# nuclia/nucliadb

Hardware: NVIDIA H100
Metric: k-NN QPS @ recall@10 (higher is better)
Workload: dtype f32

## Files before the change

### include/nidx_b200.h

```cpp
#ifndef NIDX_B200_H
#define NIDX_B200_H

#include <stdint.h>

#ifdef __cplusplus
extern "C" {
#endif

#define NIDX_OK 0
#define NIDX_EINVAL (-1)
#define NIDX_ENODEVICE (-2)
#define NIDX_ECUDA (-3)
#define NIDX_EIO (-4)
#define NIDX_ESTATE (-5)
#define NIDX_EOVERFLOW (-6)

#define NIDX_MEM_HOST 0
#define NIDX_MEM_DEVICE 1

#define NIDX_SIM_DOT 0
#define NIDX_SIM_COSINE 1
#define NIDX_SIM_L2 2

#define NIDX_METHOD_AUTO 0
#define NIDX_METHOD_HNSW 1
#define NIDX_METHOD_BRUTE 2
#define NIDX_METHOD_BRUTE_RABITQ 3
#define NIDX_METHOD_HNSW_RABITQ 4

#define NIDX_NIL 0xFFFFFFFFu

const char* nidx_last_error(void);
int nidx_device_count(void);
uint64_t nidx_launch_count(void);

typedef struct nidx_vec_segment nidx_vec_segment;

typedef struct nidx_vec_config {
    int32_t dimension;
    int32_t similarity;
    int32_t multi_vector;
    int32_t m;
    int32_t m0;
    int32_t ef_construction;
    int32_t ef_search;
    int32_t device;
} nidx_vec_config;

int nidx_vec_create(const nidx_vec_config* cfg, const float* vectors, uint64_t n, int32_t ld, int mem, const uint32_t* paragraph_of,
                    nidx_vec_segment** out);

int nidx_vec_open(const nidx_vec_config* cfg, const char* dir, nidx_vec_segment** out);
int nidx_vec_save(nidx_vec_segment* seg, const char* dir);
void nidx_vec_close(nidx_vec_segment* seg);

uint64_t nidx_vec_len(const nidx_vec_segment* seg);
const float* nidx_vec_device_vectors(const nidx_vec_segment* seg, int32_t* ld_out);

int nidx_vec_build_hnsw(nidx_vec_segment* seg, uint64_t seed, int32_t max_batch, void* stream);

int nidx_hnsw_levels(uint64_t n, int32_t m, uint64_t seed, uint8_t* out_level);

int nidx_normalize_vectors(int32_t device, float* vectors, uint64_t n, int32_t d, int32_t ld, int mem, void* stream);

int nidx_use_hnsw(uint64_t total_nodes, uint64_t matching_nodes, uint64_t top_k, int has_rabitq, int m);

int nidx_vec_extend_hnsw(nidx_vec_segment* seg, uint64_t n_existing, const uint8_t* level_existing, const uint32_t* adj0, const float* w0,
                         const uint32_t* adjU, const float* wU, uint32_t entry_node, uint32_t entry_layer, uint64_t seed, int32_t max_batch,
                         void* stream);

int nidx_vec_graph_dims(const nidx_vec_segment* seg, int32_t* s0, int32_t* su, uint64_t* upper_rows, uint32_t* entry_node,
                        uint32_t* entry_layer);
int nidx_vec_set_graph(nidx_vec_segment* seg, const uint8_t* level, const uint32_t* adj0, const float* w0, const uint32_t* adjU,
                       const float* wU);
int nidx_vec_get_graph(const nidx_vec_segment* seg, uint8_t* level, uint32_t* adj0, float* w0, uint32_t* adjU, float* wU);

int nidx_vec_set_alive(nidx_vec_segment* seg, const uint64_t* alive_bits, int mem);

typedef struct nidx_vec_search_params {
    int32_t k;
    int32_t ef;
    float min_score;
    int32_t with_duplicates;
    int32_t method;
    const uint64_t* filter_bits;
    uint64_t filter_matching;
} nidx_vec_search_params;

int nidx_vec_search(nidx_vec_segment* seg, const float* queries, int32_t nq, int32_t ldq, int mem, const nidx_vec_search_params* p,
                    uint32_t* out_ids, float* out_scores, int32_t* out_counts, void* stream);

#define NIDX_INV_LABELS 0
#define NIDX_INV_FIELDS 1
int nidx_vec_set_inverted_index(nidx_vec_segment* seg, int32_t which, uint32_t n_keys, const uint8_t* key_bytes, const uint64_t* key_off,
                                const uint64_t* post_off, const uint32_t* postings);

#define NIDX_F_LABEL 0
#define NIDX_F_KEYS 1
#define NIDX_F_AND 2
#define NIDX_F_OR 3
#define NIDX_F_NOT 4
typedef struct nidx_filter_node {
    int32_t kind;
    int32_t n;
    const uint8_t* const* keys;
    const uint32_t* key_len;
} nidx_filter_node;

int nidx_vec_filter(nidx_vec_segment* seg, const nidx_filter_node* nodes, int32_t n_nodes, uint64_t* out_bits, int mem, uint64_t* out_matching, void* stream);

int nidx_vec_search_formula(nidx_vec_segment* seg, const float* queries, int32_t nq, int32_t ldq, int mem, const nidx_vec_search_params* p,
                            const nidx_filter_node* nodes, int32_t n_nodes, uint32_t* out_ids, float* out_scores, int32_t* out_counts, void* stream);

int nidx_merge_topk(int32_t device, const uint32_t* ids, const float* scores, int32_t n_parts, int64_t part_stride, int32_t nq, int32_t k,
                    uint32_t* out_ids, float* out_scores, int32_t* out_part, void* stream);
int nidx_merge_vector_parts(int32_t device, const uint32_t* ids, const float* scores, int32_t n_parts, int64_t part_stride, int32_t nq, int32_t k,
                            uint32_t* out_ids, float* out_scores, int32_t* out_part, void* stream);

int nidx_vec_counters(nidx_vec_segment* seg, uint64_t out[3]);
int nidx_vec_counters_ex(nidx_vec_segment* seg, uint64_t out[6]);
int nidx_vec_exact_rows(nidx_vec_segment* seg, uint64_t* out);
int nidx_vec_scan_counters(nidx_vec_segment* seg, uint64_t out[2]);

int nidx_vec_rabitq_encode(nidx_vec_segment* seg, void* stream);
int nidx_vec_rabitq_codes(const nidx_vec_segment* seg, uint8_t* out_codes);
int nidx_vec_rabitq_estimate(nidx_vec_segment* seg, const float* queries, int32_t nq, int32_t ldq, int mem, float* out_estimate, float* out_error,
                             void* stream);

int nidx_vec_last_kernel_ms(nidx_vec_segment* seg, float* ms);

typedef struct nidx_txt_segment nidx_txt_segment;

#define NIDX_BM25_OR 0
#define NIDX_BM25_AND 1

int nidx_txt_create(int32_t device, uint32_t n_docs, uint32_t n_terms, const uint64_t* term_off, const uint32_t* post_doc,
                    const uint32_t* post_tf, const uint8_t* fieldnorm_id, nidx_txt_segment** out);
int nidx_txt_set_stats(nidx_txt_segment* seg, uint64_t total_docs, uint64_t total_tokens, const uint64_t* doc_freq);
int nidx_txt_set_alive(nidx_txt_segment* seg, const uint64_t* alive_bits);
void nidx_txt_close(nidx_txt_segment* seg);

typedef struct nidx_txt_search_params {
    int32_t k;
    int32_t mode;
    int32_t use_tf;
    float min_score;
    int32_t after_mode;
    float after_score;
    uint64_t after_docaddr;
    uint64_t docaddr_base;
} nidx_txt_search_params;

int nidx_txt_search(nidx_txt_segment* seg, const uint32_t* query_terms, const uint32_t* query_off, int32_t nq, int mem,
                    const nidx_txt_search_params* p, uint32_t* out_docs, float* out_scores, int32_t* out_counts, uint64_t* out_total,
                    void* stream);

int nidx_txt_last_kernel_ms(nidx_txt_segment* seg, float* ms);


int nidx_txt_set_facets(nidx_txt_segment* seg, uint32_t n_facets, const uint8_t* key_bytes, const uint64_t* key_off, const uint64_t* doc_off,
                        const uint32_t* doc_ords);

typedef struct nidx_txt_facet_request {
    int32_t n;
    const uint8_t* key_bytes;
    const uint64_t* key_off;
} nidx_txt_facet_request;

int nidx_txt_facet_buckets(nidx_txt_segment* seg, const nidx_txt_facet_request* facets, uint32_t* out_bucket_req, uint32_t* out_bucket_ord,
                           uint32_t cap, uint32_t* out_n_buckets);

int nidx_txt_search_faceted(nidx_txt_segment* seg, const uint32_t* query_terms, const uint32_t* query_off, int32_t nq, int mem,
                            const nidx_txt_search_params* p, const nidx_txt_facet_request* facets, uint32_t* out_docs, float* out_scores,
                            int32_t* out_counts, uint64_t* out_total, uint32_t* out_facet_counts, void* stream);

int nidx_txt_facet_count_all(nidx_txt_segment* seg, const nidx_txt_facet_request* facets, int mem, uint32_t* out_facet_counts, void* stream);

#define NIDX_DATE_NONE INT64_MIN
#define NIDX_ORDER_CREATED 0
#define NIDX_ORDER_MODIFIED 1
#define NIDX_ORDER_DESC 0
#define NIDX_ORDER_ASC 1

typedef struct nidx_txt_order {
    int32_t field;
    int32_t type;
} nidx_txt_order;

int nidx_txt_set_dates(nidx_txt_segment* seg, const int64_t* created, const int64_t* modified);

int nidx_txt_search_ordered(nidx_txt_segment* seg, const uint32_t* query_terms, const uint32_t* query_off, int32_t nq, int mem,
                            const nidx_txt_search_params* p, const nidx_txt_order* order, const nidx_txt_facet_request* facets, uint32_t* out_docs,
                            int64_t* out_dates, int32_t* out_counts, uint64_t* out_total, uint32_t* out_facet_counts, void* stream);


int nidx_txt_set_positions(nidx_txt_segment* seg, const uint32_t* positions, uint64_t n_positions);

typedef struct nidx_txt_phrases {
    const uint32_t* terms;
    const uint32_t* off;
    const uint32_t* query;
    int32_t n;
} nidx_txt_phrases;

int nidx_txt_search_phrases(nidx_txt_segment* seg, const uint32_t* query_terms, const uint32_t* query_off, int32_t nq, int mem,
                            const nidx_txt_search_params* p, const nidx_txt_phrases* phrases, const nidx_txt_order* order,
                            const nidx_txt_facet_request* facets, uint32_t* out_docs, float* out_scores, int64_t* out_dates, int32_t* out_counts,
                            uint64_t* out_total, uint32_t* out_facet_counts, void* stream);

int nidx_txt_list_ordered(nidx_txt_segment* seg, const nidx_txt_order* order, int32_t k, int mem, uint32_t* out_docs, int64_t* out_dates,
                          int32_t* out_count, uint64_t* out_total, void* stream);


int nidx_txt_set_doc_columns(nidx_txt_segment* seg, const uint32_t* resource_ord, const uint32_t* field_ord);

#define NIDX_P_FACET 0
#define NIDX_P_FIELD 1
#define NIDX_P_RESOURCE 2
#define NIDX_P_DATE 3
#define NIDX_P_KEYWORD 4
#define NIDX_P_ALL 5
#define NIDX_P_AND 6
#define NIDX_P_OR 7
#define NIDX_P_NOT 8
#define NIDX_PREFILTER_MAX_DEPTH 64
typedef struct nidx_prefilter_node {
    int32_t kind;
    int32_t n;
    int64_t lo, hi;
    const uint32_t* terms;
} nidx_prefilter_node;

int nidx_txt_prefilter(nidx_txt_segment* seg, const nidx_prefilter_node* nodes, int32_t n_nodes, uint64_t* out_bits, int mem, uint64_t* out_matching,
                       void* stream);

int nidx_vec_prefilter_bits(nidx_vec_segment* seg, const uint64_t* doc_bits, uint64_t n_docs, const uint32_t* join, const nidx_filter_node* nodes,
                            int32_t n_nodes, int32_t op, uint64_t* out_bits, int mem, uint64_t* out_matching, void* stream);

typedef struct nidx_shard_comm nidx_shard_comm;

int nidx_shard_unique_id(uint8_t out_id[128]);
int nidx_shard_init(const uint8_t unique_id[128], int32_t rank, int32_t world, int32_t device, nidx_shard_comm** out);
void nidx_shard_destroy(nidx_shard_comm* comm);

int nidx_vec_set_paragraph_keys(nidx_vec_segment* seg, const uint64_t* keys);

int nidx_vec_search_sharded(nidx_shard_comm* comm, nidx_vec_segment* seg, const float* queries, int32_t nq, int32_t ldq, int mem,
                            const nidx_vec_search_params* p, int32_t dedup, uint32_t* out_ids, float* out_scores, int32_t* out_part, int32_t* out_counts,
                            void* stream);

int nidx_vec_shard_record(nidx_vec_segment* seg, const float* queries, int32_t nq, int32_t ldq, int mem, const nidx_vec_search_params* p, int32_t rank,
                          int32_t dedup, uint32_t* out_record, void* stream);
int nidx_shard_merge(int32_t device, const uint32_t* records, int32_t n_parts, int32_t nq, int32_t k, int32_t dedup, int32_t with_duplicates, int mem,
                     uint32_t* out_ids, float* out_scores, int32_t* out_part, int32_t* out_counts, void* stream);
int nidx_txt_search_sharded(nidx_shard_comm* comm, nidx_txt_segment* seg, const uint32_t* query_terms, const uint32_t* query_off, int32_t nq, int mem,
                            const nidx_txt_search_params* p, uint32_t* out_docs, float* out_scores, int32_t* out_part, int32_t* out_counts, uint64_t* out_total,
                            void* stream);

int nidx_txt_set_doc_keys(nidx_txt_segment* seg, const uint64_t* keys);

typedef struct nidx_rrf_source {
    const uint64_t* keys;
    const float* scores;
    const int32_t* counts;
    int32_t k;
    double weight;
} nidx_rrf_source;

int nidx_rank_fusion_rrf(int32_t device, const nidx_rrf_source* sources, int32_t n_sources, int32_t nq, double k, int mem, uint64_t* out_keys,
                         double* out_scores, uint32_t* out_refs, int32_t* out_counts, void* stream);

typedef struct nidx_shard_search_request {
    int32_t nq;
    nidx_vec_segment* vec; const float* queries; int32_t ldq; const nidx_vec_search_params* vec_params;
    const nidx_filter_node* formula; int32_t n_formula;
    nidx_txt_segment* par; const uint32_t* par_terms; const uint32_t* par_off; const nidx_txt_search_params* par_params;
    nidx_txt_segment* doc; const uint32_t* doc_terms; const uint32_t* doc_off; const nidx_txt_search_params* doc_params;
    double rrf_k, weight_keyword, weight_semantic;
    int32_t semantic_first;
} nidx_shard_search_request;

typedef struct nidx_shard_search_response {
    uint32_t* vec_ids; float* vec_scores; int32_t* vec_counts;
    uint32_t* par_docs; float* par_scores; int32_t* par_counts; uint64_t* par_total;
    uint32_t* doc_docs; float* doc_scores; int32_t* doc_counts; uint64_t* doc_total;
    uint64_t* fused_keys; double* fused_scores; uint32_t* fused_refs; int32_t* fused_counts;
} nidx_shard_search_response;

int nidx_shard_search(const nidx_shard_search_request* req, nidx_shard_search_response* resp, int mem, void* stream);

#ifdef __cplusplus
}
#endif
#endif
```

### nucliadb_b200/_lib.py

```python
from __future__ import annotations

import ctypes as C
import os

_HERE = os.path.dirname(os.path.abspath(__file__))
LIB_PATH = os.path.join(_HERE, os.path.basename(os.environ.get("NIDX_B200_LIB", "libnidx_b200.so")))

NIDX_MEM_HOST, NIDX_MEM_DEVICE = 0, 1
NIDX_SIM_DOT, NIDX_SIM_COSINE, NIDX_SIM_L2 = 0, 1, 2
NIDX_METHOD_AUTO, NIDX_METHOD_HNSW, NIDX_METHOD_BRUTE, NIDX_METHOD_BRUTE_RABITQ, NIDX_METHOD_HNSW_RABITQ = 0, 1, 2, 3, 4
NIDX_BM25_OR, NIDX_BM25_AND = 0, 1
NIDX_ORDER_CREATED, NIDX_ORDER_MODIFIED = 0, 1
NIDX_ORDER_DESC, NIDX_ORDER_ASC = 0, 1
NIDX_DATE_NONE = -(1 << 63)
NIL = 0xFFFFFFFF


class NidxError(RuntimeError):

    def __init__(self, code: int, message: str):
        super().__init__(f"nidx_b200 error {code}: {message}")
        self.code = code


class VecConfig(C.Structure):
    _fields_ = [("dimension", C.c_int32), ("similarity", C.c_int32), ("multi_vector", C.c_int32), ("m", C.c_int32), ("m0", C.c_int32),
                ("ef_construction", C.c_int32), ("ef_search", C.c_int32), ("device", C.c_int32)]


class VecSearchParams(C.Structure):
    _fields_ = [("k", C.c_int32), ("ef", C.c_int32), ("min_score", C.c_float), ("with_duplicates", C.c_int32), ("method", C.c_int32),
                ("filter_bits", C.c_void_p), ("filter_matching", C.c_uint64)]


class FilterNode(C.Structure):
    _fields_ = [("kind", C.c_int32), ("n", C.c_int32), ("keys", C.POINTER(C.c_void_p)), ("key_len", C.POINTER(C.c_uint32))]


NIDX_INV_LABELS, NIDX_INV_FIELDS = 0, 1
NIDX_F_LABEL, NIDX_F_KEYS, NIDX_F_AND, NIDX_F_OR, NIDX_F_NOT = 0, 1, 2, 3, 4


class PrefilterNode(C.Structure):
    _fields_ = [("kind", C.c_int32), ("n", C.c_int32), ("lo", C.c_int64), ("hi", C.c_int64), ("terms", C.c_void_p)]


NIDX_P_FACET, NIDX_P_FIELD, NIDX_P_RESOURCE, NIDX_P_DATE, NIDX_P_KEYWORD, NIDX_P_ALL, NIDX_P_AND, NIDX_P_OR, NIDX_P_NOT = range(9)
NIDX_PREFILTER_MAX_DEPTH = 64


class TxtSearchParams(C.Structure):
    _fields_ = [("k", C.c_int32), ("mode", C.c_int32), ("use_tf", C.c_int32), ("min_score", C.c_float), ("after_mode", C.c_int32),
                ("after_score", C.c_float), ("after_docaddr", C.c_uint64), ("docaddr_base", C.c_uint64)]


class TxtFacetRequest(C.Structure):
    _fields_ = [("n", C.c_int32), ("key_bytes", C.c_void_p), ("key_off", C.c_void_p)]


class TxtOrder(C.Structure):
    _fields_ = [("field", C.c_int32), ("type", C.c_int32)]


class TxtPhrases(C.Structure):
    _fields_ = [("terms", C.c_void_p), ("off", C.c_void_p), ("query", C.c_void_p), ("n", C.c_int32)]


class RrfSource(C.Structure):
    _fields_ = [("keys", C.c_void_p), ("scores", C.c_void_p), ("counts", C.c_void_p), ("k", C.c_int32), ("weight", C.c_double)]


class ShardSearchRequest(C.Structure):
    _fields_ = [("nq", C.c_int32),
                ("vec", C.c_void_p), ("queries", C.c_void_p), ("ldq", C.c_int32), ("vec_params", C.POINTER(VecSearchParams)),
                ("formula", C.POINTER(FilterNode)), ("n_formula", C.c_int32),
                ("par", C.c_void_p), ("par_terms", C.c_void_p), ("par_off", C.c_void_p), ("par_params", C.POINTER(TxtSearchParams)),
                ("doc", C.c_void_p), ("doc_terms", C.c_void_p), ("doc_off", C.c_void_p), ("doc_params", C.POINTER(TxtSearchParams)),
                ("rrf_k", C.c_double), ("weight_keyword", C.c_double), ("weight_semantic", C.c_double), ("semantic_first", C.c_int32)]


class ShardSearchResponse(C.Structure):
    _fields_ = [(n, C.c_void_p) for n in ("vec_ids", "vec_scores", "vec_counts", "par_docs", "par_scores", "par_counts", "par_total",
                                           "doc_docs", "doc_scores", "doc_counts", "doc_total", "fused_keys", "fused_scores", "fused_refs", "fused_counts")]


i32, u32, i64, u64, f64, P = C.c_int32, C.c_uint32, C.c_int64, C.c_uint64, C.c_double, C.c_void_p
CFG, VSP, NODES, TSP = C.POINTER(VecConfig), C.POINTER(VecSearchParams), C.POINTER(FilterNode), C.POINTER(TxtSearchParams)
REQ, ORDER, RRF = C.POINTER(TxtFacetRequest), C.POINTER(TxtOrder), C.POINTER(RrfSource)
SIGNATURES = {
    "nidx_last_error": (C.c_char_p, []),
    "nidx_device_count": (i32, []),
    "nidx_launch_count": (u64, []),
    "nidx_vec_create": (i32, [CFG, P, u64, i32, i32, P, P]),
    "nidx_vec_open": (i32, [CFG, C.c_char_p, P]),
    "nidx_vec_save": (i32, [P, C.c_char_p]),
    "nidx_vec_close": (None, [P]),
    "nidx_vec_len": (u64, [P]),
    "nidx_vec_device_vectors": (P, [P, P]),
    "nidx_vec_build_hnsw": (i32, [P, u64, i32, P]),
    "nidx_hnsw_levels": (i32, [u64, i32, u64, P]),
    "nidx_normalize_vectors": (i32, [i32, P, u64, i32, i32, i32, P]),
    "nidx_use_hnsw": (i32, [u64, u64, u64, i32, i32]),
    "nidx_vec_extend_hnsw": (i32, [P, u64, P, P, P, P, P, u32, u32, u64, i32, P]),
    "nidx_vec_graph_dims": (i32, [P, P, P, P, P, P]),
    "nidx_vec_set_graph": (i32, [P, P, P, P, P, P]),
    "nidx_vec_get_graph": (i32, [P, P, P, P, P, P]),
    "nidx_vec_set_alive": (i32, [P, P, i32]),
    "nidx_vec_search": (i32, [P, P, i32, i32, i32, VSP, P, P, P, P]),
    "nidx_vec_set_inverted_index": (i32, [P, i32, u32, P, P, P, P]),
    "nidx_vec_filter": (i32, [P, NODES, i32, P, i32, P, P]),
    "nidx_vec_search_formula": (i32, [P, P, i32, i32, i32, VSP, NODES, i32, P, P, P, P]),
    "nidx_merge_topk": (i32, [i32, P, P, i32, i64, i32, i32, P, P, P, P]),
    "nidx_merge_vector_parts": (i32, [i32, P, P, i32, i64, i32, i32, P, P, P, P]),
    "nidx_vec_counters": (i32, [P, P]),
    "nidx_vec_counters_ex": (i32, [P, P]),
    "nidx_vec_exact_rows": (i32, [P, P]),
    "nidx_vec_scan_counters": (i32, [P, P]),
    "nidx_vec_rabitq_encode": (i32, [P, P]),
    "nidx_vec_rabitq_codes": (i32, [P, P]),
    "nidx_vec_rabitq_estimate": (i32, [P, P, i32, i32, i32, P, P, P]),
    "nidx_vec_last_kernel_ms": (i32, [P, P]),
    "nidx_txt_create": (i32, [i32, u32, u32, P, P, P, P, P]),
    "nidx_txt_set_stats": (i32, [P, u64, u64, P]),
    "nidx_txt_set_alive": (i32, [P, P]),
    "nidx_txt_close": (None, [P]),
    "nidx_txt_search": (i32, [P, P, P, i32, i32, TSP, P, P, P, P, P]),
    "nidx_txt_last_kernel_ms": (i32, [P, P]),
    "nidx_txt_set_facets": (i32, [P, u32, P, P, P, P]),
    "nidx_txt_facet_buckets": (i32, [P, REQ, P, P, u32, P]),
    "nidx_txt_search_faceted": (i32, [P, P, P, i32, i32, TSP, REQ, P, P, P, P, P, P]),
    "nidx_txt_facet_count_all": (i32, [P, REQ, i32, P, P]),
    "nidx_txt_set_dates": (i32, [P, P, P]),
    "nidx_txt_search_ordered": (i32, [P, P, P, i32, i32, TSP, ORDER, REQ, P, P, P, P, P, P]),
    "nidx_txt_list_ordered": (i32, [P, ORDER, i32, i32, P, P, P, P, P]),
    "nidx_txt_set_positions": (i32, [P, P, u64]),
    "nidx_txt_search_phrases": (i32, [P, P, P, i32, i32, TSP, P, ORDER, REQ, P, P, P, P, P, P, P]),
    "nidx_txt_set_doc_columns": (i32, [P, P, P]),
    "nidx_txt_prefilter": (i32, [P, P, i32, P, i32, P, P]),
    "nidx_vec_prefilter_bits": (i32, [P, P, u64, P, NODES, i32, i32, P, i32, P, P]),
    "nidx_shard_unique_id": (i32, [P]),
    "nidx_shard_init": (i32, [P, i32, i32, i32, P]),
    "nidx_shard_destroy": (None, [P]),
    "nidx_vec_set_paragraph_keys": (i32, [P, P]),
    "nidx_vec_search_sharded": (i32, [P, P, P, i32, i32, i32, VSP, i32, P, P, P, P, P]),
    "nidx_vec_shard_record": (i32, [P, P, i32, i32, i32, VSP, i32, i32, P, P]),
    "nidx_shard_merge": (i32, [i32, P, i32, i32, i32, i32, i32, i32, P, P, P, P, P]),
    "nidx_txt_search_sharded": (i32, [P, P, P, P, i32, i32, TSP, P, P, P, P, P, P]),
    "nidx_txt_set_doc_keys": (i32, [P, P]),
    "nidx_rank_fusion_rrf": (i32, [i32, RRF, i32, i32, f64, i32, P, P, P, P, P]),
    "nidx_shard_search": (i32, [C.POINTER(ShardSearchRequest), C.POINTER(ShardSearchResponse), i32, P]),
}
SYMBOLS = list(SIGNATURES)

_lib = None


def load():
    global _lib
    if _lib is not None:
        return _lib
    if not os.path.exists(LIB_PATH):
        raise ImportError(f"{LIB_PATH} is missing: build it with `python -c 'import __graft_entry__ as g; g.build()'` "
                          "(nvcc, sm_90a). nucliadb_b200 has no CPU fallback.")
    L = C.CDLL(LIB_PATH)
    for name, (restype, argtypes) in SIGNATURES.items():
        fn = getattr(L, name)
        fn.restype, fn.argtypes = restype, argtypes
    _lib = L
    return L


def check(rc: int):
    if rc != 0:
        raise NidxError(rc, load().nidx_last_error().decode("utf-8", "replace"))


def require_device():
    L = load()
    if L.nidx_device_count() <= 0:
        raise NidxError(-2, "no CUDA device available; nucliadb_b200 has no CPU fallback")
    return L


def ptr(a):
    if a is None:
        return None
    if isinstance(a, int):
        return C.c_void_p(a)
    if hasattr(a, "data_ptr"):
        return C.c_void_p(a.data_ptr())
    return a.ctypes.data_as(C.c_void_p)
```

### nucliadb_b200/csrc/api.cu

```cuda
#include <cub/device/device_radix_sort.cuh>
#include <cub/device/device_scan.cuh>

#include <algorithm>
#include <atomic>
#include <cmath>
#include <cfloat>
#include <cstdarg>
#include <cstdio>
#include <cstring>
#include <memory>
#include <mutex>
#include <string>
#include <vector>

#include "../../include/nidx_b200.h"
#include "bm25.cuh"
#include "phrase.cuh"
#include "prefilter.cuh"
#include "common.cuh"
#include "hnsw_build.cuh"
#include "hnsw_search.cuh"
#include "hnsw_rabitq.cuh"
#include "rabitq.cuh"
#include "rank_fusion.cuh"
#include "scan.cu"
#include "scan_tc2.cuh"
#include "segment_io.hpp"
#include "shard.cuh"
#include "topk.cuh"

using namespace nidx;

static thread_local std::string g_err;
static std::atomic<uint64_t> g_launches{0};

static int fail(int code, const char* fmt, ...) {
    char buf[512];
    va_list ap;
    va_start(ap, fmt);
    vsnprintf(buf, sizeof(buf), fmt, ap);
    va_end(ap);
    g_err = buf;
    return code;
}
#define CU(expr)                                                                                              \
    do {                                                                                                      \
        cudaError_t e__ = (expr);                                                                             \
        if (e__ != cudaSuccess) return fail(NIDX_ECUDA, "%s failed: %s (%s:%d)", #expr, cudaGetErrorString(e__), __FILE__, __LINE__); \
    } while (0)
#define LAUNCHED() (g_launches.fetch_add(1, std::memory_order_relaxed))

static int next_pow2(int x) { int p = 1; while (p < x) p <<= 1; return p; }
static int ilog2(int x) { int b = 0; while ((1 << b) < x) ++b; return b; }

template <class T>
struct DevArray {
    T* p = nullptr;
    size_t cap = 0;
    DevArray() = default;
    DevArray(DevArray&& o) noexcept : p(o.p), cap(o.cap) { o.p = nullptr; o.cap = 0; }
    DevArray& operator=(DevArray&& o) noexcept {
        if (this != &o) { release(); p = o.p; cap = o.cap; o.p = nullptr; o.cap = 0; }
        return *this;
    }
    ~DevArray() { release(); }
    operator T*() const { return p; }
    template <class U> U* as() const { return reinterpret_cast<U*>(p); }
    void release() { if (p) cudaFree(p); p = nullptr; cap = 0; }
    cudaError_t try_alloc(size_t bytes) {
        release();
        cudaError_t e = cudaMalloc(&p, bytes);
        if (e == cudaSuccess) cap = bytes;
        else { p = nullptr; (void)cudaGetLastError(); }
        return e;
    }
    int alloc(size_t bytes) {
        cudaError_t e = try_alloc(bytes);
        return e == cudaSuccess ? 0 : fail(NIDX_ECUDA, "cudaMalloc(%zu) failed: %s", bytes, cudaGetErrorString(e));
    }
    int ensure(size_t bytes) {
        if (bytes <= cap || try_alloc(bytes + bytes / 4 + 256) == cudaSuccess) return 0;
        return alloc(bytes);
    }
};
using DevBuf = DevArray<unsigned char>;
#define ENSURE(buf, bytes) do { int r__ = (buf).ensure(bytes); if (r__) return r__; } while (0)
#define ALLOC(buf, bytes) do { int r__ = (buf).alloc(bytes); if (r__) return r__; } while (0)

struct Workspace {
    DevBuf queries, qnorms, stage, scores, partial, filter, misc, sched, facets, phrases, prefilter;
    cudaEvent_t done = nullptr;
    cudaStream_t last_stream = nullptr;
    bool busy = false;
    ~Workspace() { if (done) cudaEventDestroy(done); }
};

struct WorkspacePool {
    std::mutex mu;
    std::vector<Workspace*> all;
    static constexpr size_t MAX_POOL = 8;
    Workspace* acquire(cudaStream_t stream) {
        std::lock_guard<std::mutex> g(mu);
        Workspace* pick = nullptr;
        for (Workspace* w : all)
            if (!w->busy && w->last_stream == stream) { pick = w; break; }
        if (!pick) {
            for (Workspace* w : all)
                if (!w->busy && (!w->done || cudaEventQuery(w->done) == cudaSuccess)) { pick = w; break; }
            (void)cudaGetLastError();
        }
        if (!pick && all.size() >= MAX_POOL)
            for (Workspace* w : all)
                if (!w->busy) { cudaEventSynchronize(w->done); pick = w; break; }
        if (!pick) {
            pick = new Workspace();
            cudaEventCreateWithFlags(&pick->done, cudaEventDisableTiming);
            all.push_back(pick);
        }
        pick->busy = true;
        return pick;
    }
    void release(Workspace* w, cudaStream_t stream) {
        cudaEventRecord(w->done, stream);
        std::lock_guard<std::mutex> g(mu);
        w->last_stream = stream;
        w->busy = false;
    }
    ~WorkspacePool() { for (Workspace* w : all) delete w; }
};
struct WsGuard {
    WorkspacePool& pool; Workspace* w; cudaStream_t s;
    WsGuard(WorkspacePool& p, cudaStream_t st) : pool(p), w(p.acquire(st)), s(st) {}
    ~WsGuard() { pool.release(w, s); }
};

static WorkspacePool* plan_pool(int device) {
    static std::mutex mu;
    static WorkspacePool* pools[64] = {nullptr};
    std::lock_guard<std::mutex> g(mu);
    if (device < 0 || device >= 64) return nullptr;
    if (!pools[device]) pools[device] = new WorkspacePool();
    return pools[device];
}

struct Stage {
    cudaStream_t stream;
    bool qhost, ohost;
    struct Slot { void* var; const void* in; void* out; size_t bytes; void* dev; };
    std::vector<Slot> slots;
    size_t total = 0;
    Stage(cudaStream_t s, bool qh, bool oh) : stream(s), qhost(qh), ohost(oh) {}
    void add(void* var, const void* in, void* out, size_t bytes) {
        slots.push_back({var, in, out, bytes, nullptr});
        total += (bytes + 15) / 16 * 16;
    }
    template <class T> void in(const T* src, size_t n, const T** dev) {
        *dev = src;
        if (qhost && src) add(dev, src, nullptr, n * sizeof(T));
    }
    template <class T> void out(T* dst, size_t n, T** dev) {
        *dev = dst;
        if (ohost || !dst) add(dev, nullptr, ohost ? dst : nullptr, n * sizeof(T));
    }
    int place(DevBuf& buf) {
        ENSURE(buf, total);
        unsigned char* p = buf.as<unsigned char>();
        for (Slot& s : slots) {
            s.dev = p;
            p += (s.bytes + 15) / 16 * 16;
            memcpy(s.var, &s.dev, sizeof(void*));
            if (s.in && s.bytes) CU(cudaMemcpyAsync(s.dev, s.in, s.bytes, cudaMemcpyHostToDevice, stream));
        }
        return 0;
    }
    int finish(bool sync = false) {
        if (ohost)
            for (const Slot& s : slots)
                if (s.out && s.bytes) CU(cudaMemcpyAsync(s.out, s.dev, s.bytes, cudaMemcpyDeviceToHost, stream));
        if (ohost || sync) CU(cudaStreamSynchronize(stream));
        return 0;
    }
};

struct nidx_vec_segment {
    nidx_vec_config cfg;
    uint64_t n = 0;
    int d = 0, ld = 0;
    int sm_count = 0;
    DevArray<float> d_vecs;
    DevArray<float> d_norms;
    DevArray<uint32_t> d_par_of;
    DevArray<uint32_t> d_par_first;
    uint32_t n_par = 0;
    DevArray<uint64_t> d_alive;
    uint64_t alive_count = 0;
    DevArray<uint64_t> d_par_keys;
    struct InvIndex {
        std::vector<unsigned char> key_bytes;
        std::vector<uint64_t> key_off, post_off;
        DevArray<uint32_t> d_post;
        DevArray<uint64_t> d_post_off;
        uint32_t n_keys = 0;
    } inv[2];
    bool has_graph = false;
    std::vector<uint8_t> h_level;
    DevArray<uint8_t> d_level;
    uint32_t entry_node = 0, entry_layer = 0;
    int s0 = 0, su = 0;
    uint64_t upper_rows = 0;
    DevArray<uint32_t> d_adj0; DevArray<float> d_w0;
    DevArray<uint64_t> d_upper_off;
    DevArray<uint32_t> d_adjU; DevArray<float> d_wU;
    float max_norm = 0.0f;
    bool tc_rows_ok = false;
    CUtensorMap map_v;
    bool map_v_ready = false;
    std::mutex map_mu;
    DevArray<unsigned char> d_quant;
    int quant_stride = 0;
    DevArray<unsigned long long> d_counters;
    std::atomic<unsigned long long*> last_counters{nullptr};
    DevArray<unsigned int> d_work_counter;
    cudaEvent_t ev_k0 = nullptr, ev_k1 = nullptr;
    WorkspacePool pool;
    DevArray<__half> d_hvecs;
    DevArray<float4> d_hrec;
    int ldh = 0;
    bool half_decided = false;
    std::mutex half_mu;

    ~nidx_vec_segment() {
        if (ev_k0) cudaEventDestroy(ev_k0);
        if (ev_k1) cudaEventDestroy(ev_k1);
    }

    VecDev vdev() const {
        VecDev v;
        v.vecs = d_vecs; v.norms = d_norms; v.paragraph_of = d_par_of; v.n = (uint32_t)n; v.d = d; v.ld = ld; v.sim = cfg.similarity;
        v.hvecs = nullptr; v.hrec = nullptr; v.ldh = 0;
        return v;
    }
    GraphDev gdev() const {
        GraphDev g;
        g.n = (uint32_t)n; g.M = cfg.m; g.M0 = cfg.m0; g.s0 = s0; g.su = su; g.level = d_level;
        g.entry_node = entry_node; g.entry_layer = entry_layer;
        g.adj0 = d_adj0; g.w0 = d_w0; g.upper_off = d_upper_off; g.adjU = d_adjU; g.wU = d_wU;
        return g;
    }
};

static int stride0_for(int M0) { return (M0 + 31) / 32 * 32; }
static int strideU_for(int M) { return (M + 15) / 16 * 16; }

static void free_graph(nidx_vec_segment* s) {
    s->d_level.release(); s->d_adj0.release(); s->d_w0.release(); s->d_upper_off.release(); s->d_adjU.release(); s->d_wU.release();
    s->has_graph = false;
}

static int alloc_graph(nidx_vec_segment* s, const uint8_t* level) {
    free_graph(s);
    uint64_t n = s->n;
    s->h_level.assign(level, level + n);
    std::vector<uint64_t> off(n ? n : 1);
    uint64_t rows = 0;
    uint32_t top = 0;
    for (uint64_t i = 0; i < n; ++i) { off[i] = rows; rows += level[i]; top = std::max<uint32_t>(top, level[i]); }
    s->upper_rows = rows;
    s->entry_layer = top;
    s->entry_node = 0;
    for (uint64_t i = 0; i < n; ++i) if (level[i] == top) { s->entry_node = (uint32_t)i; break; }
    s->s0 = stride0_for(s->cfg.m0);
    s->su = strideU_for(s->cfg.m);
    size_t n0 = (size_t)n * s->s0, nu = (size_t)std::max<uint64_t>(rows, 1) * s->su;
    ALLOC(s->d_level, std::max<uint64_t>(n, 1));
    ALLOC(s->d_adj0, n0 * 4 + 16);
    ALLOC(s->d_w0, n0 * 4 + 16);
    ALLOC(s->d_upper_off, std::max<uint64_t>(n, 1) * 8);
    ALLOC(s->d_adjU, nu * 4);
    ALLOC(s->d_wU, nu * 4);
    CU(cudaMemcpy(s->d_level, level, n, cudaMemcpyHostToDevice));
    CU(cudaMemcpy(s->d_upper_off, off.data(), n * 8, cudaMemcpyHostToDevice));
    CU(cudaMemset(s->d_adj0, 0xFF, n0 * 4));
    CU(cudaMemset(s->d_w0, 0, n0 * 4));
    CU(cudaMemset(s->d_adjU, 0xFF, nu * 4));
    CU(cudaMemset(s->d_wU, 0, nu * 4));
    return 0;
}

__global__ void max_norm_kernel(VecDev V, uint64_t n, unsigned int* __restrict__ out) {
    float m = 0.0f;
    bool bad = false;
    for (uint64_t i = blockIdx.x * (uint64_t)blockDim.x + threadIdx.x; i < n; i += (uint64_t)gridDim.x * blockDim.x) {
        const float nv = V.norms[i];
        m = fmaxf(m, nv);
        if (!(nv <= FLT_MAX)) bad = true;
        else if (V.sim == SIM_COSINE && nv < TC2_MIN_NORM)
            for (int j = 0; j < V.ld && !bad; ++j) bad = V.vecs[i * V.ld + j] != 0.0f;
    }
    for (int off = 16; off >= 1; off >>= 1) m = fmaxf(m, __shfl_xor_sync(0xFFFFFFFFu, m, off));
    if ((threadIdx.x & 31) == 0) atomicMax(out, __float_as_uint(m));
    if (__any_sync(0xFFFFFFFFu, bad) && (threadIdx.x & 31) == 0) atomicOr(out + 1, 1u);
}

__global__ void hs_half_kernel(VecDev V, uint64_t n, int ldh, __half* __restrict__ hv, float4* __restrict__ rec) {
    const int lane = threadIdx.x & 31;
    const double slack = 1.0 + 0x1p-20, mu = dot_depth(V.ld) * 0x1p-24, gm = mu / (1.0 - mu);
    for (uint64_t i = (blockIdx.x * (uint64_t)blockDim.x + threadIdx.x) >> 5; i < n; i += ((uint64_t)gridDim.x * blockDim.x) >> 5) {
        const float* v = V.vecs + i * V.ld;
        float m = 0.0f;
        bool finite = true;
        for (int k = lane; k < V.ld; k += 32) { float x = v[k]; finite = finite && isfinite(x); m = fmaxf(m, fabsf(x)); }
        for (int off = 16; off >= 1; off >>= 1) m = fmaxf(m, __shfl_xor_sync(0xFFFFFFFFu, m, off));
        finite = __all_sync(0xFFFFFFFFu, finite);
        int e = 0;
        if (finite && m > 0.0f) { int ex; frexpf(m, &ex); e = min(15 - ex, 126); }
        const float up = ldexpf(1.0f, e), down = ldexpf(1.0f, -e);
        double r2 = 0.0, v2 = 0.0;
        for (int k = lane; k < ldh; k += 32) {
            float x = k < V.ld ? v[k] : 0.0f;
            __half h = __float2half_rn(__fmul_rn(x, up));
            hv[i * ldh + k] = h;
            double dd = (double)__half2float(h) * (double)down - (double)x;
            r2 = fma(dd, dd, r2);
            v2 = fma((double)x, (double)x, v2);
        }
        for (int off = 16; off >= 1; off >>= 1) { r2 += __shfl_xor_sync(0xFFFFFFFFu, r2, off); v2 += __shfl_xor_sync(0xFFFFFFFFu, v2, off); }
        if (lane == 0) {
            double rho = sqrt(r2 * slack), vn = sqrt(v2 * slack);
            double eq = (rho + gm * (2.0 * vn + rho)) * slack;
            double ea = 0x1p-149 * ((double)V.ld * (1.0 + (double)down) + 1.0) * slack;
            rec[i] = make_float4(V.norms[i], down, finite ? __double2float_ru(eq) : INFINITY, __double2float_ru(ea));
        }
    }
}

constexpr size_t HS_HALF_MARGIN = (size_t)4 << 30;
static int attach_half_copy(nidx_vec_segment* s, VecDev* V) {
    const char* e = getenv("NIDX_B200_HS_F16");
    if (e && !strcmp(e, "0")) return 0;
    std::lock_guard<std::mutex> g(s->half_mu);
    if (!s->half_decided && s->n) {
        s->half_decided = true;
        const int ldh = (s->ld + 7) / 8 * 8;
        const size_t hbytes = (size_t)s->n * ldh * 2, rbytes = (size_t)s->n * 16;
        size_t free_b = 0, total_b = 0;
        CU(cudaMemGetInfo(&free_b, &total_b));
        if (free_b < hbytes + rbytes + HS_HALF_MARGIN) return 0;
        if (s->d_hvecs.try_alloc(hbytes) != cudaSuccess || s->d_hrec.try_alloc(rbytes) != cudaSuccess) {
            s->d_hvecs.release();
            return 0;
        }
        hs_half_kernel<<<s->sm_count * 8, 256>>>(s->vdev(), s->n, ldh, s->d_hvecs, s->d_hrec);
        LAUNCHED();
        CU(cudaGetLastError());
        CU(cudaDeviceSynchronize());
        s->ldh = ldh;
    }
    if (s->ldh) { V->hvecs = s->d_hvecs; V->hrec = s->d_hrec; V->ldh = s->ldh; }
    return 0;
}

typedef CUresult (*tmap_encode_fn)(CUtensorMap*, CUtensorMapDataType, cuuint32_t, void*, const cuuint64_t*, const cuuint64_t*, const cuuint32_t*, const cuuint32_t*,
                                   CUtensorMapInterleave, CUtensorMapSwizzle, CUtensorMapL2promotion, CUtensorMapFloatOOBfill);
static int make_row_tensor_map(CUtensorMap* map, const float* base, uint64_t rows, int ld, int box_rows) {
    static tmap_encode_fn encode = nullptr;
    static std::once_flag once;
    std::call_once(once, [] {
        void* fn = nullptr;
        cudaDriverEntryPointQueryResult qres;
        if (cudaGetDriverEntryPoint("cuTensorMapEncodeTiled", &fn, cudaEnableDefault, &qres) == cudaSuccess && qres == cudaDriverEntryPointSuccess)
            encode = reinterpret_cast<tmap_encode_fn>(fn);
    });
    if (!encode) return fail(NIDX_ECUDA, "cuTensorMapEncodeTiled is not available from this driver");
    cuuint64_t dims[2] = {(cuuint64_t)ld, (cuuint64_t)rows};
    cuuint64_t strides[1] = {(cuuint64_t)ld * 4};
    cuuint32_t box[2] = {(cuuint32_t)TC2_KB, (cuuint32_t)box_rows};
    cuuint32_t estr[2] = {1, 1};
    CUresult r = encode(map, CU_TENSOR_MAP_DATA_TYPE_FLOAT32, 2, const_cast<float*>(base), dims, strides, box, estr, CU_TENSOR_MAP_INTERLEAVE_NONE,
                        CU_TENSOR_MAP_SWIZZLE_128B, CU_TENSOR_MAP_L2_PROMOTION_L2_256B, CU_TENSOR_MAP_FLOAT_OOB_FILL_NONE);
    if (r != CUDA_SUCCESS) return fail(NIDX_ECUDA, "cuTensorMapEncodeTiled failed (%d)", (int)r);
    return 0;
}

template <class T>
static int set_rows(int device, DevArray<T>& dev, const T* host, size_t n) {
    CU(cudaSetDevice(device));
    if (!host) { dev.release(); return 0; }
    if (!dev) ALLOC(dev, std::max<size_t>(n, 1) * sizeof(T));
    CU(cudaMemcpy(dev, host, n * sizeof(T), cudaMemcpyHostToDevice));
    return 0;
}

extern "C" {

const char* nidx_last_error(void) { return g_err.c_str(); }
int nidx_device_count(void) {
    int n = 0;
    if (cudaGetDeviceCount(&n) != cudaSuccess) { cudaGetLastError(); return 0; }
    return n;
}
uint64_t nidx_launch_count(void) { return g_launches.load(); }

static int check_device(int device) {
    int n = nidx_device_count();
    if (n <= 0) return fail(NIDX_ENODEVICE, "no CUDA device available (nidx_b200 has no CPU fallback)");
    if (device < 0 || device >= n) return fail(NIDX_EINVAL, "device %d out of range (have %d)", device, n);
    CU(cudaSetDevice(device));
    return 0;
}

static int fill_defaults(nidx_vec_config* c) {
    if (c->dimension <= 0) return fail(NIDX_EINVAL, "dimension must be positive");
    if (c->similarity != NIDX_SIM_DOT && c->similarity != NIDX_SIM_COSINE && c->similarity != NIDX_SIM_L2) return fail(NIDX_EINVAL, "unknown similarity %d", c->similarity);
    if (c->m <= 0) c->m = 30;
    if (c->m0 <= 0) c->m0 = 60;
    if (c->ef_construction <= 0) c->ef_construction = 100;
    if (c->ef_search <= 0) c->ef_search = 30;
    if (c->m0 > HS_MAX_ROW || c->m > HS_MAX_ROW) return fail(NIDX_EINVAL, "M / M0 above %d not supported", HS_MAX_ROW);
    if (c->ef_construction > HB_MAX_CAND) return fail(NIDX_EINVAL, "ef_construction above %d not supported", HB_MAX_CAND);
    return 0;
}

static int finish_create(nidx_vec_segment* s, const uint32_t* paragraph_of_host) {
    uint64_t n = s->n;
    ALLOC(s->d_norms, std::max<uint64_t>(n, 1) * 4);
    if (n) {
        int blocks = (int)std::min<uint64_t>((n + 7) / 8, (uint64_t)s->sm_count * 16);
        row_norms_kernel<<<blocks, 256>>>(s->d_vecs, s->ld, n, s->d_norms);
        LAUNCHED();
        CU(cudaGetLastError());
    }
    s->n_par = (uint32_t)n;
    if (paragraph_of_host) {
        std::vector<uint32_t> first;
        uint32_t prev = NIDX_NIL;
        for (uint64_t i = 0; i < n; ++i) {
            uint32_t p = paragraph_of_host[i];
            if (i == 0 || p != prev) {
                if (p != (uint32_t)first.size()) return fail(NIDX_EINVAL, "paragraph_of must be contiguous and ascending from 0 (vector %llu -> %u)", (unsigned long long)i, p);
                first.push_back((uint32_t)i);
                prev = p;
            }
        }
        first.push_back((uint32_t)n);
        s->n_par = (uint32_t)first.size() - 1;
        if (s->n_par != n) {
            ALLOC(s->d_par_of, n * 4);
            CU(cudaMemcpy(s->d_par_of, paragraph_of_host, n * 4, cudaMemcpyHostToDevice));
            ALLOC(s->d_par_first, first.size() * 4);
            CU(cudaMemcpy(s->d_par_first, first.data(), first.size() * 4, cudaMemcpyHostToDevice));
        }
    }
    if (n) {
        DevArray<unsigned int> d_bits;
        ALLOC(d_bits, 8);
        CU(cudaMemset(d_bits, 0, 8));
        max_norm_kernel<<<std::min<uint64_t>((n + 255) / 256, (uint64_t)s->sm_count * 8), 256>>>(s->vdev(), n, d_bits);
        LAUNCHED();
        unsigned int hb[2] = {0, 0};
        CU(cudaMemcpy(hb, d_bits, 8, cudaMemcpyDeviceToHost));
        memcpy(&s->max_norm, &hb[0], 4);
        s->tc_rows_ok = hb[1] == 0;
    }
    ALLOC(s->d_counters, 8 * sizeof(unsigned long long));
    CU(cudaMemset(s->d_counters, 0, 8 * sizeof(unsigned long long)));
    ALLOC(s->d_work_counter, 64);
    CU(cudaEventCreate(&s->ev_k0));
    CU(cudaEventCreate(&s->ev_k1));
    CU(cudaDeviceSynchronize());
    return 0;
}

static int new_segment(const nidx_vec_config* cfg, std::unique_ptr<nidx_vec_segment>& out) {
    if (!cfg) return fail(NIDX_EINVAL, "null argument");
    nidx_vec_config c = *cfg;
    int r = fill_defaults(&c);
    if (r) return r;
    r = check_device(c.device);
    if (r) return r;
    out.reset(new nidx_vec_segment());
    nidx_vec_segment* s = out.get();
    s->cfg = c;
    s->d = c.dimension;
    s->ld = (c.dimension + 3) / 4 * 4;
    cudaDeviceProp prop;
    cudaGetDeviceProperties(&prop, c.device);
    s->sm_count = prop.multiProcessorCount;
    return 0;
}

static int upload_rows(nidx_vec_segment* s, const void* rows, size_t row_bytes, bool host, bool whole) {
    const uint64_t n = s->n;
    ALLOC(s->d_vecs, std::max<size_t>((size_t)n * s->ld * 4, 16));
    if (n == 0) return 0;
    if (whole) {
        CU(cudaMemcpy(s->d_vecs, rows, (size_t)n * row_bytes, host ? cudaMemcpyHostToDevice : cudaMemcpyDeviceToDevice));
        return 0;
    }
    const unsigned char* src = static_cast<const unsigned char*>(rows);
    DevBuf staged;
    if (host) {
        ALLOC(staged, (size_t)n * row_bytes);
        CU(cudaMemcpy(staged, rows, (size_t)n * row_bytes, cudaMemcpyHostToDevice));
        src = staged;
    }
    pad_rows_kernel<<<s->sm_count * 8, 256>>>(src, row_bytes, s->d, s->d_vecs, s->ld, n);
    LAUNCHED();
    CU(cudaGetLastError());
    CU(cudaDeviceSynchronize());
    return 0;
}

int nidx_vec_create(const nidx_vec_config* cfg, const float* vectors, uint64_t n, int32_t ld, int mem, const uint32_t* paragraph_of,
                    nidx_vec_segment** out) {
    if (!out) return fail(NIDX_EINVAL, "null argument");
    std::unique_ptr<nidx_vec_segment> s;
    int r = new_segment(cfg, s);
    if (r) return r;
    if (n >= (1ull << 31)) return fail(NIDX_EINVAL, "at most 2^31-1 vectors per segment");
    if (ld < s->d) return fail(NIDX_EINVAL, "ld %d < dimension %d (VectorErr::InconsistentDimensions)", ld, s->d);
    s->n = n;
    r = upload_rows(s.get(), vectors, (size_t)ld * 4, mem == NIDX_MEM_HOST, ld == s->ld);
    if (!r) r = finish_create(s.get(), paragraph_of);
    if (r) return r;
    *out = s.release();
    return 0;
}

constexpr int NRM_WARPS = 4;
__global__ void __launch_bounds__(NRM_WARPS * 32) normalize_rows_kernel(float* __restrict__ v, uint64_t n, int d, int ld) {
    extern __shared__ float nrm_row[];
    const int lane = threadIdx.x & 31, warp = threadIdx.x >> 5;
    float* row = nrm_row + (size_t)warp * d;
    for (uint64_t i = (uint64_t)blockIdx.x * NRM_WARPS + warp; i < n; i += (uint64_t)gridDim.x * NRM_WARPS) {
        float* src = v + i * (uint64_t)ld;
        for (int j = lane; j < d; j += 32) row[j] = src[j];
        __syncwarp();
        float acc = 0.0f;
        if (lane == 0)
            for (int j = 0; j < d; ++j) acc = __fadd_rn(acc, __fmul_rn(row[j], row[j]));
        float mag = __fsqrt_rn(__shfl_sync(0xFFFFFFFFu, acc, 0));
        for (int j = lane; j < d; j += 32) src[j] = __fdiv_rn(row[j], mag);
        __syncwarp();
    }
}

int nidx_normalize_vectors(int32_t device, float* vectors, uint64_t n, int32_t d, int32_t ld, int mem, void* stream_) {
    int r = check_device(device);
    if (r) return r;
    if (d <= 0 || ld < d || !vectors) return fail(NIDX_EINVAL, "normalize: d %d, ld %d", d, ld);
    if ((size_t)d * 4 * NRM_WARPS > 200 * 1024) return fail(NIDX_EINVAL, "normalize: dimension %d too large", d);
    if (n == 0) return 0;
    cudaStream_t st = static_cast<cudaStream_t>(stream_);
    float* dv = vectors;
    DevArray<float> staged;
    size_t bytes = (size_t)n * ld * 4;
    if (mem == NIDX_MEM_HOST) {
        ALLOC(staged, bytes);
        dv = staged;
        cudaError_t e = cudaMemcpyAsync(dv, vectors, bytes, cudaMemcpyHostToDevice, st);
        if (e != cudaSuccess) return fail(NIDX_ECUDA, "normalize: H2D failed: %s", cudaGetErrorString(e));
    }
    int sm = 0;
    cudaDeviceGetAttribute(&sm, cudaDevAttrMultiProcessorCount, device);
    size_t smem = (size_t)d * 4 * NRM_WARPS;
    cudaFuncSetAttribute(normalize_rows_kernel, cudaFuncAttributeMaxDynamicSharedMemorySize, (int)smem);
    uint64_t want = (n + NRM_WARPS - 1) / NRM_WARPS;
    int grid = (int)std::min<uint64_t>(want, (uint64_t)sm * 16);
    normalize_rows_kernel<<<grid, NRM_WARPS * 32, smem, st>>>(dv, n, d, ld);
    LAUNCHED();
    cudaError_t e = cudaGetLastError();
    if (e == cudaSuccess && staged) e = cudaMemcpyAsync(vectors, dv, bytes, cudaMemcpyDeviceToHost, st);
    if (e == cudaSuccess && staged) e = cudaStreamSynchronize(st);
    if (e != cudaSuccess) return fail(NIDX_ECUDA, "normalize failed: %s", cudaGetErrorString(e));
    return 0;
}

void nidx_vec_close(nidx_vec_segment* s) {
    if (!s) return;
    cudaSetDevice(s->cfg.device);
    cudaDeviceSynchronize();
    delete s;
}

uint64_t nidx_vec_len(const nidx_vec_segment* s) { return s ? s->n : 0; }
const float* nidx_vec_device_vectors(const nidx_vec_segment* s, int32_t* ld_out) {
    if (!s) return nullptr;
    if (ld_out) *ld_out = s->ld;
    return s->d_vecs;
}

int nidx_vec_set_alive(nidx_vec_segment* s, const uint64_t* alive_bits, int mem) {
    if (!s) return fail(NIDX_EINVAL, "null segment");
    CU(cudaSetDevice(s->cfg.device));
    if (!alive_bits) { s->d_alive.release(); return 0; }
    size_t words = ((size_t)s->n_par + 63) / 64;
    if (!s->d_alive) ALLOC(s->d_alive, std::max<size_t>(words, 1) * 8 + 8);
    CU(cudaMemcpy(s->d_alive, alive_bits, words * 8, mem == NIDX_MEM_DEVICE ? cudaMemcpyDeviceToDevice : cudaMemcpyHostToDevice));
    std::vector<uint64_t> h(words);
    if (words) CU(cudaMemcpy(h.data(), s->d_alive, words * 8, cudaMemcpyDeviceToHost));
    uint64_t cnt = 0;
    for (size_t i = 0; i < words; ++i) {
        uint64_t v = h[i];
        if ((i + 1) * 64 > s->n_par) v &= s->n_par > i * 64 ? (~0ull >> (64 - (s->n_par - i * 64))) : 0ull;
        cnt += (uint64_t)__builtin_popcountll(v);
    }
    s->alive_count = cnt;
    return 0;
}

static bool use_hnsw_cost(size_t total_nodes, size_t matching_nodes, size_t top_k, size_t M, bool has_rabitq);
int nidx_use_hnsw(uint64_t total_nodes, uint64_t matching_nodes, uint64_t top_k, int has_rabitq, int m) {
    if (matching_nodes == 0 || top_k == 0 || m <= 0) return 0;
    return use_hnsw_cost((size_t)total_nodes, (size_t)matching_nodes, (size_t)top_k, (size_t)m, has_rabitq != 0) ? 1 : 0;
}

int nidx_vec_graph_dims(const nidx_vec_segment* s, int32_t* s0, int32_t* su, uint64_t* upper_rows, uint32_t* entry_node, uint32_t* entry_layer) {
    if (!s) return fail(NIDX_EINVAL, "null segment");
    if (!s->has_graph) return fail(NIDX_ESTATE, "segment has no HNSW graph");
    if (s0) *s0 = s->s0;
    if (su) *su = s->su;
    if (upper_rows) *upper_rows = s->upper_rows;
    if (entry_node) *entry_node = s->entry_node;
    if (entry_layer) *entry_layer = s->entry_layer;
    return 0;
}

int nidx_vec_set_graph(nidx_vec_segment* s, const uint8_t* level, const uint32_t* adj0, const float* w0, const uint32_t* adjU, const float* wU) {
    if (!s || !level || !adj0) return fail(NIDX_EINVAL, "null argument");
    CU(cudaSetDevice(s->cfg.device));
    for (uint64_t i = 0; i < s->n; ++i)
        if (level[i] >= HS_MAX_LAYERS) return fail(NIDX_EINVAL, "node %llu has level %d >= %d", (unsigned long long)i, level[i], HS_MAX_LAYERS);
    int r = alloc_graph(s, level);
    if (r) return r;
    size_t n0 = (size_t)s->n * s->s0, nu = (size_t)s->upper_rows * s->su;
    CU(cudaMemcpy(s->d_adj0, adj0, n0 * 4, cudaMemcpyHostToDevice));
    if (w0) CU(cudaMemcpy(s->d_w0, w0, n0 * 4, cudaMemcpyHostToDevice));
    if (nu && adjU) CU(cudaMemcpy(s->d_adjU, adjU, nu * 4, cudaMemcpyHostToDevice));
    if (nu && wU) CU(cudaMemcpy(s->d_wU, wU, nu * 4, cudaMemcpyHostToDevice));
    s->has_graph = true;
    return 0;
}

int nidx_vec_get_graph(const nidx_vec_segment* s, uint8_t* level, uint32_t* adj0, float* w0, uint32_t* adjU, float* wU) {
    if (!s) return fail(NIDX_EINVAL, "null segment");
    if (!s->has_graph) return fail(NIDX_ESTATE, "segment has no HNSW graph");
    CU(cudaSetDevice(s->cfg.device));
    CU(cudaDeviceSynchronize());
    size_t n0 = (size_t)s->n * s->s0, nu = (size_t)s->upper_rows * s->su;
    if (level) memcpy(level, s->h_level.data(), s->n);
    if (adj0) CU(cudaMemcpy(adj0, s->d_adj0, n0 * 4, cudaMemcpyDeviceToHost));
    if (w0) CU(cudaMemcpy(w0, s->d_w0, n0 * 4, cudaMemcpyDeviceToHost));
    if (adjU && nu) CU(cudaMemcpy(adjU, s->d_adjU, nu * 4, cudaMemcpyDeviceToHost));
    if (wU && nu) CU(cudaMemcpy(wU, s->d_wU, nu * 4, cudaMemcpyDeviceToHost));
    return 0;
}

static int read_counters(nidx_vec_segment* s, uint64_t* out, std::initializer_list<int> pick) {
    if (!s || !out) return fail(NIDX_EINVAL, "null argument");
    CU(cudaSetDevice(s->cfg.device));
    unsigned long long h[8];
    unsigned long long* src = s->last_counters.load();
    CU(cudaMemcpy(h, src ? src : s->d_counters, sizeof(h), cudaMemcpyDeviceToHost));
    for (int i : pick) *out++ = i < 0 ? h[2] + h[3] : h[i];
    return 0;
}
int nidx_vec_counters_ex(nidx_vec_segment* s, uint64_t out[6]) { return read_counters(s, out, {0, 1, 2, 3, 4, 5}); }
int nidx_vec_counters(nidx_vec_segment* s, uint64_t out[3]) { return read_counters(s, out, {0, 1, -1}); }
int nidx_vec_exact_rows(nidx_vec_segment* s, uint64_t* out) { return read_counters(s, out, {6}); }
int nidx_vec_scan_counters(nidx_vec_segment* s, uint64_t out[2]) { return read_counters(s, out, {6, 7}); }

static int rabitq_check(const nidx_vec_segment* s) {
    if (s->cfg.similarity != NIDX_SIM_DOT || s->d % 64 != 0) return fail(NIDX_EINVAL, "RaBitQ needs Dot similarity and dimension %% 64 == 0 (config.rs:170-173)");
    if (s->d / 32 > RQ_MAX_WORDS32) return fail(NIDX_EINVAL, "RaBitQ: dimension above %d not supported", RQ_MAX_WORDS32 * 32);
    return 0;
}

int nidx_vec_rabitq_encode(nidx_vec_segment* s, void* stream_) {
    if (!s) return fail(NIDX_EINVAL, "null segment");
    int r = rabitq_check(s);
    if (r) return r;
    CU(cudaSetDevice(s->cfg.device));
    cudaStream_t stream = reinterpret_cast<cudaStream_t>(stream_);
    s->quant_stride = rabitq_stride(s->d);
    if (!s->d_quant) ALLOC(s->d_quant, std::max<size_t>((size_t)s->n * s->quant_stride, 16));
    if (s->n) {
        rabitq_encode_kernel<<<(unsigned)((s->n + 7) / 8), 256, 0, stream>>>(s->vdev(), s->d_quant, s->quant_stride);
        LAUNCHED();
        CU(cudaGetLastError());
    }
    CU(cudaStreamSynchronize(stream));
    return 0;
}

int nidx_vec_rabitq_codes(const nidx_vec_segment* s, uint8_t* out) {
    if (!s || !out) return fail(NIDX_EINVAL, "null argument");
    if (!s->d_quant) return fail(NIDX_ESTATE, "segment has no RaBitQ codes (call nidx_vec_rabitq_encode)");
    CU(cudaSetDevice(s->cfg.device));
    size_t rec = (size_t)s->d / 8 + 8;
    CU(cudaMemcpy2D(out, rec, s->d_quant, (size_t)s->quant_stride, rec, (size_t)s->n, cudaMemcpyDeviceToHost));
    return 0;
}

static int rabitq_ready(const nidx_vec_segment* s) {
    int r = rabitq_check(s);
    if (r) return r;
    if (!s->d_quant) return fail(NIDX_ESTATE, "segment has no RaBitQ codes (call nidx_vec_rabitq_encode)");
    return 0;
}

static int upload_queries(nidx_vec_segment* s, Workspace& w, const float* queries, int nq, int ldq, bool staged, cudaStream_t stream, const float** dq) {
    *dq = queries;
    if (ldq == s->ld && staged) return 0;
    ENSURE(w.queries, (size_t)nq * s->ld * 4);
    *dq = w.queries.as<float>();
    if (ldq == s->ld) {
        CU(cudaMemcpyAsync(w.queries.p, queries, (size_t)nq * ldq * 4, cudaMemcpyDeviceToDevice, stream));
    } else {
        pad_rows_kernel<<<std::min(nq, 1024), 256, 0, stream>>>(reinterpret_cast<const unsigned char*>(queries), (size_t)ldq * 4, s->d, w.queries.as<float>(),
                                                               s->ld, (uint64_t)nq);
        LAUNCHED();
    }
    return 0;
}

static int rabitq_query_planes(nidx_vec_segment* s, Workspace& w, const float* dq, int nq, cudaStream_t stream, uint32_t** planes, RabitqQueryParams** params) {
    size_t plane_bytes = ((size_t)nq * 4 * (s->d / 32) * 4 + 15) / 16 * 16;
    ENSURE(w.misc, plane_bytes + (size_t)nq * sizeof(RabitqQueryParams) + 64);
    *planes = w.misc.as<uint32_t>();
    *params = reinterpret_cast<RabitqQueryParams*>(w.misc.as<unsigned char>() + plane_bytes);
    rabitq_query_kernel<<<(nq + 7) / 8, 256, 0, stream>>>(dq, s->ld, s->d, nq, *planes, *params);
    LAUNCHED();
    return 0;
}

int nidx_vec_rabitq_estimate(nidx_vec_segment* s, const float* queries, int32_t nq, int32_t ldq, int mem, float* out_est, float* out_err, void* stream_) {
    if (!s || !queries || !out_est || !out_err || nq <= 0) return fail(NIDX_EINVAL, "bad argument");
    if (!s->d_quant) return fail(NIDX_ESTATE, "segment has no RaBitQ codes (call nidx_vec_rabitq_encode)");
    if (ldq < s->d) return fail(NIDX_EINVAL, "query dimension %d != index dimension %d", ldq, s->d);
    CU(cudaSetDevice(s->cfg.device));
    cudaStream_t stream = reinterpret_cast<cudaStream_t>(stream_);
    WsGuard g(s->pool, stream);
    Workspace& w = *g.w;
    const bool host = mem == NIDX_MEM_HOST;
    Stage st(stream, host, host);
    const float* d_q;
    float *d_est, *d_err;
    st.in(queries, (size_t)nq * ldq, &d_q);
    st.out(out_est, (size_t)nq * s->n, &d_est);
    st.out(out_err, (size_t)nq * s->n, &d_err);
    int r = st.place(w.stage);
    const float* dq;
    if (!r) r = upload_queries(s, w, d_q, nq, ldq, host, stream, &dq);
    uint32_t* planes; RabitqQueryParams* params;
    if (!r) r = rabitq_query_planes(s, w, dq, nq, stream, &planes, &params);
    if (r) return r;
    if (s->n) {
        rabitq_estimate_kernel<<<dim3((unsigned)((s->n + 255) / 256), nq), 256, 0, stream>>>(s->d_quant, s->quant_stride, (uint32_t)s->n, s->d, planes, params, d_est, d_err);
        LAUNCHED();
        CU(cudaGetLastError());
    }
    return st.finish();
}

int nidx_vec_last_kernel_ms(nidx_vec_segment* s, float* ms) {
    if (!s || !ms) return fail(NIDX_EINVAL, "null argument");
    CU(cudaSetDevice(s->cfg.device));
    CU(cudaEventSynchronize(s->ev_k1));
    CU(cudaEventElapsedTime(ms, s->ev_k0, s->ev_k1));
    return 0;
}

static bool use_hnsw_cost(size_t total_nodes, size_t matching_nodes, size_t top_k, size_t M, bool has_rabitq) {
    const size_t RERANKING_FACTOR = 100;
    size_t full_cost = has_rabitq ? 16 : 1, search_mult = has_rabitq ? RERANKING_FACTOR * 3 / 4 : 1, rerank_mult = has_rabitq ? RERANKING_FACTOR / 2 : 0;
    float l = logf((float)total_nodes) - 2.0f;
    float hnsw_rq = l * l * logf((float)top_k) * (float)search_mult;
    size_t hnsw_full = top_k * rerank_mult + top_k * M * total_nodes / std::max<size_t>(matching_nodes, 1);
    size_t hnsw_cost = (size_t)(hnsw_rq < 0 ? 0 : hnsw_rq) + hnsw_full * full_cost;
    size_t bf_cost = matching_nodes + top_k * rerank_mult * full_cost;
    return hnsw_cost < bf_cost;
}

__global__ void and_bits_kernel(const uint64_t* a, const uint64_t* b, uint64_t* out, size_t words, unsigned long long* count) {
    unsigned long long local = 0;
    for (size_t i = blockIdx.x * (size_t)blockDim.x + threadIdx.x; i < words; i += (size_t)gridDim.x * blockDim.x) {
        uint64_t v = a[i] & (b ? b[i] : ~0ull);
        out[i] = v;
        local += __popcll(v);
    }
    for (int off = 16; off >= 1; off >>= 1) local += __shfl_xor_sync(0xFFFFFFFFu, local, off);
    if ((threadIdx.x & 31) == 0 && local) atomicAdd(count, local);
}

static bool hnsw_search_smem(const nidx_vec_segment* s, int ef0, int k, int* list_cap, int* cu_cap, int* hash_bits, size_t* bytes) {
    int cu = std::min(std::max(ef0 + k * s->s0, 2 * ef0), 4096);
    int lc = std::max(ef0, cu);
    int slots = next_pow2(std::max(4096, (ef0 * s->s0 * 3) / 2));
    slots = std::max(slots, next_pow2(4 * lc));
    *list_cap = lc; *cu_cap = cu; *hash_bits = ilog2(slots);
    *bytes = hs_smem_bytes(s->ld, lc, *hash_bits);
    return *bytes <= 200 * 1024;
}

static bool rq_walk_smem(const nidx_vec_segment* s, int k, int* last_k, int* cu_cap, int* list_cap, int* hash_bits, size_t* bytes) {
    *last_k = (int)std::min<size_t>((size_t)k * 100, 2000);
    *cu_cap = std::min(std::max(k + k * s->s0, 2 * k), 4096);
    *list_cap = std::max(*last_k, *cu_cap);
    *hash_bits = ilog2(next_pow2(std::max(2048, 4 * *cu_cap)));
    *bytes = rq_smem_bytes(s->ld, s->d, *list_cap, *hash_bits, k);
    return *bytes <= 200 * 1024;
}

}

template <int... NGs, typename F>
static auto pick_ng(int ld, F inst) {
    auto k = inst(std::integral_constant<int, 0>());
    auto match = [&](auto ng) { if (ld == ng * 128) k = inst(ng); };
    (match(std::integral_constant<int, NGs>()), ...);
    return k;
}

typedef void (*hs_kernel_t)(VecDev, GraphDev, SearchArgs);
static hs_kernel_t pick_search_kernel(int ld) {
    return pick_ng<1, 2, 3, 4, 6, 8>(ld, [](auto ng) -> hs_kernel_t { return hnsw_search_kernel<ng>; });
}

static hs_kernel_t pick_rabitq_walk_kernel(int ld, bool w4) {
    return pick_ng<2, 3, 4, 6, 8>(ld, [w4](auto ng) -> hs_kernel_t { return w4 ? hnsw_rabitq_kernel<ng, 4> : hnsw_rabitq_kernel<ng>; });
}

typedef void (*scan_kernel_t)(VecDev, const float*, const float*, int, int, float*);
static scan_kernel_t pick_scan_kernel(int ld) {
    return pick_ng<1, 2, 3, 4, 6, 8>(ld, [](auto ng) -> scan_kernel_t {
        if constexpr (ng == 0) return scan_scores_kernel;
        else return scan_scores_kernel_t<ng, ng <= 3 ? 4 : 2>;
    });
}

__global__ void bits_scatter_kernel(const uint32_t* __restrict__ postings, const uint64_t* __restrict__ ranges, uint64_t* __restrict__ out) {
    uint64_t b = ranges[2 * blockIdx.x], e = ranges[2 * blockIdx.x + 1];
    for (uint64_t i = b + threadIdx.x; i < e; i += blockDim.x) {
        uint32_t p = postings[i];
        atomicOr(reinterpret_cast<unsigned long long*>(out) + (p >> 6), 1ull << (p & 63));
    }
}
__global__ void bits_combine_kernel(uint64_t* __restrict__ a, const uint64_t* __restrict__ b, size_t words, uint64_t n_bits, int op) {
    for (size_t i = blockIdx.x * (size_t)blockDim.x + threadIdx.x; i < words; i += (size_t)gridDim.x * blockDim.x) {
        uint64_t v = a[i];
        if (op == 0) v &= b[i];
        else if (op == 1) v |= b[i];
        else {
            v = ~v;
            if ((i + 1) * 64 > n_bits) v &= n_bits > i * 64 ? (~0ull >> (64 - (n_bits - i * 64))) : 0ull;
        }
        a[i] = v;
    }
}

struct FilterEval {
    nidx_vec_segment* s;
    const nidx_filter_node* nodes;
    int n_nodes;
    uint64_t* bufs;
    size_t words;
    cudaStream_t stream;
    std::vector<uint64_t> ranges;
    std::vector<std::pair<size_t, size_t>> atom_ranges;
    uint64_t* d_ranges = nullptr;
    int next_buf = 0;

    static int cmp_key(const unsigned char* a, size_t la, const unsigned char* b, size_t lb) {
        int c = memcmp(a, b, std::min(la, lb));
        return c ? c : (la < lb ? -1 : (la > lb ? 1 : 0));
    }
    static uint32_t lower_bound(const nidx_vec_segment::InvIndex& ix, const unsigned char* q, size_t lq) {
        uint32_t lo = 0, hi = ix.n_keys;
        while (lo < hi) {
            uint32_t mid = (lo + hi) / 2;
            if (cmp_key(ix.key_bytes.data() + ix.key_off[mid], ix.key_off[mid + 1] - ix.key_off[mid], q, lq) < 0) lo = mid + 1; else hi = mid;
        }
        return lo;
    }
    int collect(int i) {
        const nidx_filter_node& nd = nodes[i];
        if (nd.kind == NIDX_F_LABEL || nd.kind == NIDX_F_KEYS) {
            const nidx_vec_segment::InvIndex& ix = s->inv[nd.kind == NIDX_F_LABEL ? NIDX_INV_LABELS : NIDX_INV_FIELDS];
            size_t first = ranges.size() / 2;
            for (int j = 0; j < nd.n; ++j) {
                const unsigned char* q = nd.keys[j];
                size_t lq = nd.key_len[j];
                uint32_t lo = lower_bound(ix, q, lq), hi = lo;
                if (nd.kind == NIDX_F_LABEL) {
                    uint32_t a = lo, b = ix.n_keys;
                    while (a < b) {
                        uint32_t mid = (a + b) / 2;
                        size_t lk = ix.key_off[mid + 1] - ix.key_off[mid];
                        bool starts = lk >= lq && memcmp(ix.key_bytes.data() + ix.key_off[mid], q, lq) == 0;
                        if (starts) a = mid + 1; else b = mid;
                    }
                    hi = a;
                } else if (lo < ix.n_keys && cmp_key(ix.key_bytes.data() + ix.key_off[lo], ix.key_off[lo + 1] - ix.key_off[lo], q, lq) == 0) {
                    hi = lo + 1;
                }
                if (hi > lo && ix.post_off[hi] > ix.post_off[lo]) { ranges.push_back(ix.post_off[lo]); ranges.push_back(ix.post_off[hi]); }
            }
            atom_ranges[i] = {first, ranges.size() / 2 - first};
            return i + 1;
        }
        int j = i + 1;
        for (int c = 0; c < nd.n; ++c) { if (j >= n_nodes) return -1; j = collect(j); if (j < 0) return -1; }
        return j;
    }
    uint64_t* eval(int i, int* next) {
        const nidx_filter_node& nd = nodes[i];
        uint64_t* out = bufs + (size_t)(next_buf++) * words;
        if (nd.kind == NIDX_F_LABEL || nd.kind == NIDX_F_KEYS) {
            cudaMemsetAsync(out, 0, words * 8, stream);
            auto ar = atom_ranges[i];
            if (ar.second) {
                const nidx_vec_segment::InvIndex& ix = s->inv[nd.kind == NIDX_F_LABEL ? NIDX_INV_LABELS : NIDX_INV_FIELDS];
                bits_scatter_kernel<<<(unsigned)ar.second, 128, 0, stream>>>(ix.d_post, d_ranges + 2 * ar.first, out);
                LAUNCHED();
            }
            *next = i + 1;
            return out;
        }
        int j = i + 1;
        uint64_t* acc = nullptr;
        unsigned blocks = (unsigned)std::min<size_t>((words + 255) / 256, 1024);
        for (int c = 0; c < nd.n; ++c) {
            int nx;
            uint64_t* child = eval(j, &nx);
            j = nx;
            if (!acc) { cudaMemcpyAsync(out, child, words * 8, cudaMemcpyDeviceToDevice, stream); acc = out; }
            else {
                bits_combine_kernel<<<blocks, 256, 0, stream>>>(acc, child, words, s->n_par, nd.kind == NIDX_F_OR ? 1 : 0);
                LAUNCHED();
            }
        }
        if (nd.kind == NIDX_F_NOT) { bits_combine_kernel<<<blocks, 256, 0, stream>>>(acc, nullptr, words, s->n_par, 2); LAUNCHED(); }
        *next = j;
        return acc;
    }
};

struct FilterBufs {
    size_t words;
    uint64_t* bits;
    unsigned long long* count;
    uint64_t* nodes;
    uint64_t* ranges;
};
static int filter_bufs(const nidx_vec_segment* s, Workspace& w, int n_nodes, size_t range_bytes, FilterBufs& f) {
    f.words = ((size_t)s->n_par + 63) / 64;
    const size_t node_words = n_nodes ? ((size_t)n_nodes + 1) * f.words : 0;
    ENSURE(w.filter, (f.words + 8 + node_words) * 8 + range_bytes);
    f.bits = w.filter.as<uint64_t>();
    f.count = reinterpret_cast<unsigned long long*>(f.bits + f.words);
    f.nodes = f.bits + f.words + 8;
    f.ranges = f.nodes + node_words;
    return 0;
}

static int filter_and_alive(nidx_vec_segment* s, Workspace& w, const uint64_t* filter, uint64_t* out, unsigned long long* h_count, cudaStream_t stream,
                            const uint64_t** bits) {
    FilterBufs f;
    int r = filter_bufs(s, w, 0, 0, f);
    if (r) return r;
    if (!out) out = f.bits;
    CU(cudaMemsetAsync(f.count, 0, 8, stream));
    and_bits_kernel<<<std::min<size_t>((f.words + 255) / 256, 1024), 256, 0, stream>>>(filter, s->d_alive, out, f.words, f.count);
    LAUNCHED();
    if (h_count) CU(cudaMemcpyAsync(h_count, f.count, 8, cudaMemcpyDeviceToHost, stream));
    *bits = out;
    return 0;
}

static int filter_formula_device(nidx_vec_segment* s, Workspace& w, const nidx_filter_node* nodes, int n_nodes, cudaStream_t stream, uint64_t** out) {
    if (!nodes || n_nodes <= 0) return fail(NIDX_EINVAL, "empty filter formula");
    size_t words = ((size_t)s->n_par + 63) / 64;
    for (int i = 0; i < n_nodes; ++i) {
        int kd = nodes[i].kind;
        if (kd < NIDX_F_LABEL || kd > NIDX_F_NOT || nodes[i].n < 0) return fail(NIDX_EINVAL, "filter node %d: bad kind / count", i);
        if ((kd == NIDX_F_LABEL || kd == NIDX_F_KEYS) && nodes[i].n > 0 && (!nodes[i].keys || !nodes[i].key_len)) return fail(NIDX_EINVAL, "filter node %d: null keys", i);
        if ((kd == NIDX_F_AND || kd == NIDX_F_OR || kd == NIDX_F_NOT) && nodes[i].n < 1) return fail(NIDX_EINVAL, "filter node %d: a compound clause needs operands", i);
    }
    FilterEval ev;
    ev.s = s; ev.nodes = nodes; ev.n_nodes = n_nodes; ev.words = words; ev.stream = stream;
    ev.atom_ranges.assign(n_nodes, {0, 0});
    if (ev.collect(0) != n_nodes) return fail(NIDX_EINVAL, "malformed filter formula (operand counts do not add up to %d nodes)", n_nodes);
    size_t range_bytes = ev.ranges.size() * 8;
    FilterBufs f;
    int r = filter_bufs(s, w, n_nodes, range_bytes, f);
    if (r) return r;
    ev.bufs = f.nodes;
    ev.d_ranges = f.ranges;
    if (range_bytes) CU(cudaMemcpyAsync(ev.d_ranges, ev.ranges.data(), range_bytes, cudaMemcpyHostToDevice, stream));
    int next = 0;
    uint64_t* res = ev.eval(0, &next);
    CU(cudaGetLastError());
    if (range_bytes) CU(cudaStreamSynchronize(stream));
    *out = res;
    return 0;
}

static bool use_tc_filter(const nidx_vec_segment* s, int nq, int k) {
    if (k > TC2_KMAX || s->ld % TC2_KB != 0 || s->d_par_first || s->n < (uint64_t)TC2_N || s->cfg.similarity == NIDX_SIM_L2 || !s->tc_rows_ok) return false;
    const char* e = getenv("NIDX_B200_SCAN");
    if (e && !strcmp(e, "exact")) return false;
    if (e && !strcmp(e, "tensor")) return true;
    return nq >= 64;
}

struct VecCall {
    nidx_vec_segment* s;
    Workspace& w;
    cudaStream_t stream;
    const nidx_vec_search_params* p;
    VecDev V;
    int nq, k;
    const float* dq;
    float* qnorms;
    const uint64_t* bits;
    uint32_t* ids;
    float* scores;
    int* counts;
    unsigned long long* counters;

    int write_empty() const {
        CU(cudaMemsetAsync(ids, 0xFF, (size_t)nq * k * 4, stream));
        CU(cudaMemsetAsync(scores, 0, (size_t)nq * k * 4, stream));
        CU(cudaMemsetAsync(counts, 0, (size_t)nq * 4, stream));
        return 0;
    }

    int rabitq_scan() {
        int r = rabitq_ready(s);
        if (r) return r;
        if (s->d_par_first) return fail(NIDX_EINVAL, "RaBitQ scan of multi-vector paragraphs is not implemented");
        if (k > 1024) return fail(NIDX_EINVAL, "k above 1024 not supported");
        uint32_t* planes; RabitqQueryParams* params;
        r = rabitq_query_planes(s, w, dq, nq, stream, &planes, &params);
        if (r) return r;
        int qgroup = (int)std::max<size_t>(1, std::min<size_t>((size_t)nq, ((size_t)4 << 30) / ((size_t)s->n * 8)));
        ENSURE(w.scores, (size_t)qgroup * s->n * 8);
        size_t smem_rr = rr_smem_bytes(s->ld, k);
        CU(cudaFuncSetAttribute(rabitq_rerank_kernel, cudaFuncAttributeMaxDynamicSharedMemorySize, (int)smem_rr));
        for (int q0 = 0; q0 < nq; q0 += qgroup) {
            int nqg = std::min(qgroup, nq - q0);
            float* d_est = w.scores.as<float>();
            float* d_err = d_est + (size_t)nqg * s->n;
            if (q0 == 0) CU(cudaEventRecord(s->ev_k0, stream));
            const uint32_t* qplanes = planes + (size_t)q0 * 4 * (s->d / 32);
            rabitq_estimate_kernel<<<dim3((unsigned)((s->n + 255) / 256), nqg), 256, 0, stream>>>(s->d_quant, s->quant_stride, (uint32_t)s->n, s->d, qplanes,
                                                                                                     params + q0, d_est, d_err);
            if (q0 == 0) CU(cudaEventRecord(s->ev_k1, stream));
            LAUNCHED();
            rabitq_rerank_kernel<<<nqg, RR_THREADS, smem_rr, stream>>>(V, dq + (size_t)q0 * s->ld, d_est, d_err, bits, p->min_score, k,
                                                                         ids + (size_t)q0 * k, scores + (size_t)q0 * k, counts + q0, nullptr);
            LAUNCHED();
        }
        CU(cudaGetLastError());
        return 0;
    }

    int tc_filter_scan() {
        int n_chunks = (int)((s->n + TC2_CHUNK - 1) / TC2_CHUNK), n_qblocks = (nq + TC2_M - 1) / TC2_M;
        {
            std::lock_guard<std::mutex> lk(s->map_mu);
            if (!s->map_v_ready) {
                int mr = make_row_tensor_map(&s->map_v, s->d_vecs, s->n, s->ld, TC2_N);
                if (mr) return mr;
                s->map_v_ready = true;
            }
        }
        CUtensorMap map_q;
        int mr = make_row_tensor_map(&map_q, dq, (uint64_t)nq, s->ld, TC2_M);
        if (mr) return mr;
        int grid = std::min(n_chunks * n_qblocks, s->sm_count);
        int slots = std::max(1, std::min(grid / n_qblocks, n_chunks));
        size_t cand_n = (size_t)nq * slots * TC2_LISTS * TC2_L;
        ENSURE(w.scores, cand_n * 8 + 64);
        Tc2Args ta;
        ta.nq = nq; ta.n_qblocks = n_qblocks; ta.n_chunks = n_chunks; ta.slots = slots; ta.qnorms = qnorms; ta.bits = bits;
        ta.cand_score = w.scores.as<float>(); ta.cand_id = reinterpret_cast<uint32_t*>(w.scores.as<float>() + cand_n);
        ta.work_counter = w.sched.as<unsigned int>();
        CU(cudaFuncSetAttribute(scan_tc_filter_kernel, cudaFuncAttributeMaxDynamicSharedMemorySize, (int)TC2_SMEM_BYTES));
        grid = n_qblocks <= grid ? n_qblocks * slots : grid;
        CU(cudaEventRecord(s->ev_k0, stream));
        scan_tc_filter_kernel<<<grid, TC2_THREADS, TC2_SMEM_BYTES, stream>>>(map_q, s->map_v, V, ta);
        CU(cudaEventRecord(s->ev_k1, stream));
        LAUNCHED();
        int cap = topk_cap(k, 256);
        size_t smem_rf = tc2_refine_smem(s->ld, cap);
        if (smem_rf > 48 * 1024) CU(cudaFuncSetAttribute(scan_tc_refine_kernel, cudaFuncAttributeMaxDynamicSharedMemorySize, (int)smem_rf));
        scan_tc_refine_kernel<<<nq, 256, smem_rf, stream>>>(V, dq, qnorms, slots * TC2_LISTS, ta.cand_score, ta.cand_id, bits, s->max_norm,
                                                              p->min_score, k, cap, ids, scores, counts, counters + 6);
        LAUNCHED();
        CU(cudaGetLastError());
        return 0;
    }

    int exact_scan() {
        if (k > 1024) return fail(NIDX_EINVAL, "brute-force k above 1024 not supported");
        int cap = topk_cap(k, 256);
        int n_chunks = (int)std::min<uint64_t>(std::max<uint64_t>(1, ((uint64_t)s->sm_count * 4 + nq - 1) / nq), (s->n_par + 4095) / 4096);
        n_chunks = std::max(n_chunks, 1);
        size_t max_score_bytes = (size_t)4 << 30;
        int qgroup = (int)std::max<size_t>(1, std::min<size_t>((size_t)nq, max_score_bytes / ((size_t)s->n * 4)));
        qgroup = std::max(SCAN_QT, qgroup / SCAN_QT * SCAN_QT);
        qgroup = std::min(qgroup, (nq + SCAN_QT - 1) / SCAN_QT * SCAN_QT);
        ENSURE(w.scores, (size_t)qgroup * s->n * 4);
        ENSURE(w.partial, (size_t)qgroup * n_chunks * k * 8);
        size_t smem_scan = (size_t)SCAN_QT * s->ld * 4;
        scan_kernel_t scan_kern = pick_scan_kernel(s->ld);
        if (smem_scan > 48 * 1024) CU(cudaFuncSetAttribute(scan_kern, cudaFuncAttributeMaxDynamicSharedMemorySize, (int)smem_scan));
        if ((size_t)cap * 8 > 48 * 1024) {
            CU(cudaFuncSetAttribute(scan_select_kernel, cudaFuncAttributeMaxDynamicSharedMemorySize, cap * 8));
            CU(cudaFuncSetAttribute(topk_merge_kernel, cudaFuncAttributeMaxDynamicSharedMemorySize, cap * 8));
        }
        for (int q0 = 0; q0 < nq; q0 += qgroup) {
            int nqg = std::min(qgroup, nq - q0);
            int n_qtiles = (nqg + SCAN_QT - 1) / SCAN_QT;
            uint64_t n_vchunks = (s->n + SCAN_WARPS * SCAN_VPW - 1) / (SCAN_WARPS * SCAN_VPW);
            uint64_t grid = n_vchunks * n_qtiles;
            if (grid > 0x7FFFFFFFull) return fail(NIDX_EINVAL, "scan grid too large");
            if (q0 == 0) CU(cudaEventRecord(s->ev_k0, stream));
            scan_kern<<<(unsigned)grid, SCAN_WARPS * 32, smem_scan, stream>>>(V, dq + (size_t)q0 * s->ld, qnorms + q0, nqg, n_qtiles, w.scores.as<float>());
            if (q0 == 0) CU(cudaEventRecord(s->ev_k1, stream));
            LAUNCHED();
            scan_select_kernel<<<dim3(n_chunks, nqg), 256, (size_t)cap * 8, stream>>>(w.scores.as<float>(), (uint32_t)s->n, s->n_par, s->d_par_first, nullptr,
                                                                                        bits, p->min_score, k, cap, n_chunks, w.partial.as<uint64_t>());
            LAUNCHED();
            topk_merge_kernel<<<nqg, 256, (size_t)cap * 8, stream>>>(w.partial.as<uint64_t>(), n_chunks * k, k, cap, ids + (size_t)q0 * k,
                                                                       scores + (size_t)q0 * k, counts + q0);
            LAUNCHED();
        }
        CU(cudaGetLastError());
        return 0;
    }

    SearchArgs walk_args(int ef0, int list_cap, int cu_cap, int hash_bits) const {
        SearchArgs a;
        memset(&a, 0, sizeof(a));
        a.mode = 0; a.nq = nq; a.queries = dq; a.qnorms = qnorms; a.k = k; a.ef0 = ef0; a.min_score = p->min_score;
        a.with_duplicates = p->with_duplicates; a.multi_vector = s->cfg.multi_vector; a.filter = bits;
        a.out_ids = ids; a.out_scores = scores; a.out_counts = counts;
        a.hash_bits = hash_bits; a.list_cap = list_cap; a.cu_cap = cu_cap;
        a.work_counter = w.sched.as<unsigned int>();
        a.counters = counters;
        return a;
    }

    int walk_grid(hs_kernel_t kern, int threads, size_t smem, int* grid) const {
        CU(cudaFuncSetAttribute(kern, cudaFuncAttributeMaxDynamicSharedMemorySize, (int)smem));
        int occ = 0;
        CU(cudaOccupancyMaxActiveBlocksPerMultiprocessor(&occ, kern, threads, smem));
        *grid = std::min(nq, std::max(1, occ) * s->sm_count);
        return 0;
    }

    int launch_walk(hs_kernel_t kern, int grid, int threads, size_t smem, const VecDev& Vw, const SearchArgs& a) const {
        CU(cudaEventRecord(s->ev_k0, stream));
        kern<<<grid, threads, smem, stream>>>(Vw, s->gdev(), a);
        CU(cudaEventRecord(s->ev_k1, stream));
        LAUNCHED();
        CU(cudaGetLastError());
        return 0;
    }

    int quantised_walk() {
        int r = rabitq_ready(s);
        if (r) return r;
        uint32_t* planes; RabitqQueryParams* params;
        r = rabitq_query_planes(s, w, dq, nq, stream, &planes, &params);
        if (r) return r;
        int last_k, cu_cap, list_cap, hash_bits;
        size_t smem;
        if (!rq_walk_smem(s, k, &last_k, &cu_cap, &list_cap, &hash_bits, &smem))
            return fail(NIDX_EINVAL, "quantised HNSW search needs %zu bytes of shared memory (k=%d, dim=%d): too large", smem, k, s->d);
        int gv_bits = 16;
        while ((1 << gv_bits) < 24 * last_k) ++gv_bits;
        hs_kernel_t kern = pick_rabitq_walk_kernel(s->ld, false);
        int threads = HS_THREADS, grid = 0;
        r = walk_grid(kern, threads, smem, &grid);
        const char* ew = getenv("NIDX_B200_RQ_W");
        const int force = ew ? atoi(ew) : 0;
        if (!r && (force == 4 || (force != 8 && nq > grid))) {
            kern = pick_rabitq_walk_kernel(s->ld, true);
            threads = 128;
            r = walk_grid(kern, threads, smem, &grid);
        }
        if (r) return r;
        ENSURE(w.scores, ((size_t)grid << gv_bits) * 4);
        SearchArgs a = walk_args(last_k, list_cap, cu_cap, hash_bits);
        a.codes = s->d_quant; a.code_stride = s->quant_stride; a.planes = planes; a.qparams = params;
        a.gvisited = w.scores.as<uint32_t>(); a.gv_bits = gv_bits; a.last_k = last_k;
        return launch_walk(kern, grid, threads, smem, V, a);
    }

    int dense_walk() {
        int ef = p->ef > 0 ? p->ef : s->cfg.ef_search;
        int ef0 = std::max(k, ef);
        int list_cap, cu_cap, hash_bits;
        size_t smem;
        if (!hnsw_search_smem(s, ef0, k, &list_cap, &cu_cap, &hash_bits, &smem))
            return fail(NIDX_EINVAL, "HNSW search needs %zu bytes of shared memory (ef=%d, k=%d, dim=%d): too large", smem, ef0, k, s->d);
        VecDev Vh = V;
        int r = attach_half_copy(s, &Vh);
        hs_kernel_t kern = pick_search_kernel(s->ld);
        int grid = 0;
        if (!r) r = walk_grid(kern, HS_THREADS, smem, &grid);
        if (r) return r;
        return launch_walk(kern, grid, HS_THREADS, smem, Vh, walk_args(ef0, list_cap, cu_cap, hash_bits));
    }
};

static int choose_method(const nidx_vec_segment* s, uint64_t matching, int k, int ef) {
    if (!s->has_graph) return NIDX_METHOD_BRUTE;
    bool walk_ok = s->d_quant && s->cfg.similarity == NIDX_SIM_DOT;
    bool scan_ok = walk_ok && !s->d_par_first && k <= 1024;
    if (!use_hnsw_cost(s->n_par, matching, (size_t)k, (size_t)s->cfg.m, walk_ok)) return scan_ok ? NIDX_METHOD_BRUTE_RABITQ : NIDX_METHOD_BRUTE;
    int last_k, list_cap, cu_cap, hash_bits;
    size_t bytes;
    bool fits = walk_ok ? rq_walk_smem(s, k, &last_k, &cu_cap, &list_cap, &hash_bits, &bytes)
                        : hnsw_search_smem(s, std::max(k, ef > 0 ? ef : s->cfg.ef_search), k, &list_cap, &cu_cap, &hash_bits, &bytes);
    if (!fits && k <= 1024) return NIDX_METHOD_BRUTE;
    return walk_ok ? NIDX_METHOD_HNSW_RABITQ : NIDX_METHOD_HNSW;
}

static int vec_search_impl(nidx_vec_segment* s, const float* queries, int32_t nq, int32_t ldq, bool qhost, bool ohost, const nidx_vec_search_params* p,
                           uint32_t* out_ids, float* out_scores, int32_t* out_counts, cudaStream_t stream, const nidx_filter_node* formula = nullptr,
                           int32_t n_formula = 0) {
    if (!s || !p || (!queries && nq > 0) || !out_ids || !out_scores) return fail(NIDX_EINVAL, "null argument");
    if (nq <= 0) return 0;
    if (ldq < s->d) return fail(NIDX_EINVAL, "query dimension %d != index dimension %d (VectorErr::InconsistentDimensions)", ldq, s->d);
    const int k = p->k;
    if (k <= 0) return fail(NIDX_EINVAL, "k must be positive");
    CU(cudaSetDevice(s->cfg.device));
    WsGuard g(s->pool, stream);
    Workspace& w = *g.w;
    VecCall c{s, w, stream, p, s->vdev(), nq, k};
    Stage st(stream, qhost, ohost);
    const float* d_q;
    const uint64_t* d_filter;
    st.in(queries, (size_t)nq * ldq, &d_q);
    st.in(formula ? nullptr : p->filter_bits, ((size_t)s->n_par + 63) / 64, &d_filter);
    st.out(out_ids, (size_t)nq * k, &c.ids);
    st.out(out_scores, (size_t)nq * k, &c.scores);
    st.out(out_counts, (size_t)nq, &c.counts);
    int r = st.place(w.stage);
    if (r) return r;
    ENSURE(w.sched, 128);
    CU(cudaMemsetAsync(w.sched.p, 0, 128, stream));
    c.counters = reinterpret_cast<unsigned long long*>(w.sched.as<unsigned char>() + 64);
    s->last_counters.store(c.counters);

    r = upload_queries(s, w, d_q, nq, ldq, qhost, stream, &c.dq);
    if (r) return r;
    ENSURE(w.qnorms, (size_t)nq * 4);
    c.qnorms = w.qnorms.as<float>();
    if (s->cfg.similarity != NIDX_SIM_DOT) {
        row_norms_kernel<<<(nq + 7) / 8, 256, 0, stream>>>(c.dq, s->ld, (uint64_t)nq, c.qnorms);
        LAUNCHED();
    }

    c.bits = s->d_alive;
    uint64_t matching = s->d_alive ? s->alive_count : s->n_par;
    if (d_filter || formula) {
        if (formula) {
            uint64_t* fdev = nullptr;
            r = filter_formula_device(s, w, formula, n_formula, stream, &fdev);
            if (r) return r;
            d_filter = fdev;
        }
        matching = formula ? 0 : p->filter_matching;
        unsigned long long h = 0;
        r = filter_and_alive(s, w, d_filter, nullptr, matching ? nullptr : &h, stream, &c.bits);
        if (r) return r;
        if (matching == 0) {
            CU(cudaStreamSynchronize(stream));
            matching = h;
        }
    }

    const int method = p->method == NIDX_METHOD_AUTO ? choose_method(s, matching, k, p->ef) : p->method;
    const bool walk = method == NIDX_METHOD_HNSW || method == NIDX_METHOD_HNSW_RABITQ;
    if (matching == 0) r = c.write_empty();
    else if (walk && !s->has_graph) return fail(NIDX_ESTATE, "HNSW search requested but the segment has no graph");
    else if (s->n == 0) r = c.write_empty();
    else if (method == NIDX_METHOD_BRUTE_RABITQ) r = c.rabitq_scan();
    else if (method == NIDX_METHOD_BRUTE && use_tc_filter(s, nq, k)) r = c.tc_filter_scan();
    else if (method == NIDX_METHOD_BRUTE) r = c.exact_scan();
    else if (method == NIDX_METHOD_HNSW_RABITQ) r = c.quantised_walk();
    else r = c.dense_walk();
    if (r) return r;
    return st.finish();
}

extern "C" {

int nidx_vec_search(nidx_vec_segment* s, const float* queries, int32_t nq, int32_t ldq, int mem, const nidx_vec_search_params* p, uint32_t* out_ids,
                    float* out_scores, int32_t* out_counts, void* stream_) {
    bool host = mem == NIDX_MEM_HOST;
    return vec_search_impl(s, queries, nq, ldq, host, host, p, out_ids, out_scores, out_counts, reinterpret_cast<cudaStream_t>(stream_));
}

int nidx_vec_search_formula(nidx_vec_segment* s, const float* queries, int32_t nq, int32_t ldq, int mem, const nidx_vec_search_params* p,
                            const nidx_filter_node* nodes, int32_t n_nodes, uint32_t* out_ids, float* out_scores, int32_t* out_counts, void* stream_) {
    bool host = mem == NIDX_MEM_HOST;
    if (p && p->filter_bits) return fail(NIDX_EINVAL, "give either filter_bits or a formula");
    return vec_search_impl(s, queries, nq, ldq, host, host, p, out_ids, out_scores, out_counts, reinterpret_cast<cudaStream_t>(stream_), nodes, n_nodes);
}

int nidx_vec_set_inverted_index(nidx_vec_segment* s, int32_t which, uint32_t n_keys, const uint8_t* key_bytes, const uint64_t* key_off, const uint64_t* post_off,
                                const uint32_t* postings) {
    if (!s || (which != NIDX_INV_LABELS && which != NIDX_INV_FIELDS)) return fail(NIDX_EINVAL, "bad argument");
    if (n_keys && (!key_off || !post_off || (!key_bytes && key_off[n_keys]) || (!postings && post_off[n_keys]))) return fail(NIDX_EINVAL, "null argument");
    CU(cudaSetDevice(s->cfg.device));
    nidx_vec_segment::InvIndex ix;
    if (!n_keys) { ix.key_off.assign(1, 0); ix.post_off.assign(1, 0); s->inv[which] = std::move(ix); return 0; }
    for (uint32_t i = 0; i + 1 < n_keys; ++i)
        if (FilterEval::cmp_key(key_bytes + key_off[i], key_off[i + 1] - key_off[i], key_bytes + key_off[i + 1], key_off[i + 2] - key_off[i + 1]) >= 0)
            return fail(NIDX_EINVAL, "inverted index keys must be strictly ascending (key %u)", i + 1);
    uint64_t np = post_off[n_keys];
    for (uint64_t i = 0; i < np; ++i) if (postings[i] >= s->n_par) return fail(NIDX_EINVAL, "posting %llu: paragraph %u out of range", (unsigned long long)i, postings[i]);
    ix.key_bytes.assign(key_bytes, key_bytes + key_off[n_keys]);
    ix.key_off.assign(key_off, key_off + n_keys + 1);
    ix.post_off.assign(post_off, post_off + n_keys + 1);
    ALLOC(ix.d_post, std::max<uint64_t>(np, 1) * 4);
    if (np) CU(cudaMemcpy(ix.d_post, postings, np * 4, cudaMemcpyHostToDevice));
    ALLOC(ix.d_post_off, ((size_t)n_keys + 1) * 8);
    CU(cudaMemcpy(ix.d_post_off, post_off, ((size_t)n_keys + 1) * 8, cudaMemcpyHostToDevice));
    ix.n_keys = n_keys;
    s->inv[which] = std::move(ix);
    return 0;
}

int nidx_vec_filter(nidx_vec_segment* s, const nidx_filter_node* nodes, int32_t n_nodes, uint64_t* out_bits, int mem, uint64_t* out_matching, void* stream_) {
    if (!s) return fail(NIDX_EINVAL, "null segment");
    CU(cudaSetDevice(s->cfg.device));
    cudaStream_t stream = reinterpret_cast<cudaStream_t>(stream_);
    WsGuard g(s->pool, stream);
    Workspace& w = *g.w;
    const bool host = mem == NIDX_MEM_HOST;
    Stage st(stream, host, host);
    uint64_t* d_bits;
    st.out(out_bits, ((size_t)s->n_par + 63) / 64, &d_bits);
    int r = st.place(w.stage);
    uint64_t* fdev = nullptr;
    if (!r) r = filter_formula_device(s, w, nodes, n_nodes, stream, &fdev);
    unsigned long long h = 0;
    const uint64_t* bits;
    if (!r) r = filter_and_alive(s, w, fdev, d_bits, &h, stream, &bits);
    if (!r) r = st.finish(true);
    if (r) return r;
    if (out_matching) *out_matching = h;
    return 0;
}

static int launch_parts_merge(const uint32_t* ids, const float* scores, int n_parts, size_t part_stride, int nq, int k, uint32_t* out_ids, float* out_scores,
                              int* out_part, cudaStream_t stream) {
    if (k > 1024 || (long long)n_parts * k >= (1ll << 31)) return fail(NIDX_EINVAL, "k above 1024 not supported");
    int cap = topk_cap(k, 256);
    if ((size_t)cap * 8 > 48 * 1024) CU(cudaFuncSetAttribute(parts_merge_kernel, cudaFuncAttributeMaxDynamicSharedMemorySize, cap * 8));
    parts_merge_kernel<<<nq, 256, (size_t)cap * 8, stream>>>(ids, scores, n_parts, part_stride, nq, k, cap, out_ids, out_scores, out_part);
    LAUNCHED();
    return 0;
}

int nidx_merge_topk(int32_t device, const uint32_t* ids, const float* scores, int32_t n_parts, int64_t part_stride, int32_t nq, int32_t k,
                    uint32_t* out_ids, float* out_scores, int32_t* out_part, void* stream_) {
    int r = check_device(device);
    if (r) return r;
    if (!ids || !scores || !out_ids || !out_scores || n_parts <= 0 || nq <= 0 || k <= 0) return fail(NIDX_EINVAL, "bad argument");
    r = launch_parts_merge(ids, scores, n_parts, part_stride > 0 ? (size_t)part_stride : (size_t)nq * k, nq, k, out_ids, out_scores, out_part,
                           reinterpret_cast<cudaStream_t>(stream_));
    if (r) return r;
    CU(cudaGetLastError());
    return 0;
}

static int launch_kmerge(const uint32_t* ids, const float* scores, int n_parts, size_t part_stride, int nq, int k, uint32_t* out_ids, float* out_scores,
                         int* out_part, int* out_counts, cudaStream_t stream) {
    if ((long long)n_parts * k >= (1ll << 31)) return fail(NIDX_EINVAL, "n_parts * k must stay below 2^31");
    size_t per = (size_t)n_parts * 4;
    if (per > 96 * 1024) return fail(NIDX_EINVAL, "%d parts are too many for the vector merge", n_parts);
    int threads = (int)std::max<size_t>(1, std::min<size_t>(128, (size_t)(48 * 1024) / per));
    threads = std::min(threads, nq);
    size_t smem = per * threads;
    if (smem > 48 * 1024) CU(cudaFuncSetAttribute(kmerge_parts_kernel, cudaFuncAttributeMaxDynamicSharedMemorySize, (int)smem));
    kmerge_parts_kernel<<<(nq + threads - 1) / threads, threads, smem, stream>>>(ids, scores, n_parts, part_stride, nq, k, out_ids, out_scores, out_part,
                                                                                 out_counts);
    LAUNCHED();
    return 0;
}

int nidx_merge_vector_parts(int32_t device, const uint32_t* ids, const float* scores, int32_t n_parts, int64_t part_stride, int32_t nq, int32_t k,
                            uint32_t* out_ids, float* out_scores, int32_t* out_part, void* stream_) {
    int r = check_device(device);
    if (r) return r;
    if (!ids || !scores || !out_ids || !out_scores || n_parts <= 0 || nq <= 0 || k <= 0) return fail(NIDX_EINVAL, "bad argument");
    r = launch_kmerge(ids, scores, n_parts, part_stride > 0 ? (size_t)part_stride : (size_t)nq * k, nq, k, out_ids, out_scores, out_part, nullptr,
                      reinterpret_cast<cudaStream_t>(stream_));
    if (r) return r;
    CU(cudaGetLastError());
    return 0;
}

static void host_assign_levels(uint64_t n, int M, uint64_t seed, uint8_t* level) {
    uint64_t st[4], state = seed;
    for (int i = 0; i < 4; ++i) {
        state += 0x9e3779b97f4a7c15ull;
        uint64_t z = state;
        z = (z ^ (z >> 30)) * 0xbf58476d1ce4e5b9ull;
        z = (z ^ (z >> 27)) * 0x94d049bb133111ebull;
        st[i] = z ^ (z >> 31);
    }
    auto rotl = [](uint64_t x, int k) { return (x << k) | (x >> (64 - k)); };
    double level_factor = 1.0 / std::log((double)M);
    for (uint64_t i = 0; i < n; ++i) {
        uint64_t r = rotl(st[0] + st[3], 23) + st[0];
        uint64_t t = st[1] << 17;
        st[2] ^= st[0]; st[3] ^= st[1]; st[1] ^= st[2]; st[0] ^= st[3];
        st[2] ^= t;
        st[3] = rotl(st[3], 45);
        double u = (double)(r >> 12) * (1.0 / 4503599627370496.0);
        double lv = std::round(-std::log(u) * level_factor);
        if (!(lv < (double)(HS_MAX_LAYERS - 1))) lv = (double)(HS_MAX_LAYERS - 1);
        level[i] = (uint8_t)lv;
    }
}

}

static int insert_batches(nidx_vec_segment* s, const std::vector<uint8_t>& level, const std::vector<uint32_t>& order, const std::vector<uint32_t>& ends,
                          cudaStream_t stream, const uint32_t* entry_after_first) {
    uint64_t n = order.size();
    std::vector<uint64_t> wstart(n + 1);
    uint64_t W = 0;
    for (uint64_t i = 0; i < n; ++i) { wstart[i] = W; W += (uint64_t)level[order[i]] + 1; }
    wstart[n] = W;
    std::vector<uint32_t> w_pos(W);
    std::vector<unsigned char> w_layer(W);
    for (uint64_t i = 0; i < n; ++i)
        for (int l = 0; l <= level[order[i]]; ++l) { w_pos[wstart[i] + l] = (uint32_t)i; w_layer[wstart[i] + l] = (unsigned char)l; }
    uint64_t max_b = 0, max_w = 0;
    for (size_t b = 0, begin = 0; b < ends.size(); begin = ends[b], ++b) {
        max_b = std::max<uint64_t>(max_b, ends[b] - begin);
        max_w = std::max<uint64_t>(max_w, wstart[ends[b]] - wstart[begin]);
    }
    int efC = s->cfg.ef_construction, M = s->cfg.m;
    DevArray<uint32_t> d_order, d_wpos, d_rev_x, d_idx, d_idx_sorted, d_heads;
    DevArray<unsigned int> d_head_ctr;
    DevArray<unsigned char> d_wlayer;
    DevArray<uint64_t> d_found, d_rev_key, d_key_sorted;
    DevArray<int> d_found_count;
    DevArray<float> d_rev_sim;
    DevBuf d_cub;
    size_t cub_bytes = 0;
    size_t max_rev = (size_t)max_w * M;
    ALLOC(d_order, n * 4);
    ALLOC(d_wpos, W * 4);
    ALLOC(d_wlayer, W);
    ALLOC(d_found, (size_t)max_b * HS_MAX_LAYERS * efC * 8);
    ALLOC(d_found_count, (size_t)max_b * HS_MAX_LAYERS * 4);
    ALLOC(d_rev_key, max_rev * 8);
    ALLOC(d_key_sorted, max_rev * 8);
    ALLOC(d_rev_x, max_rev * 4);
    ALLOC(d_rev_sim, max_rev * 4);
    ALLOC(d_idx, max_rev * 4);
    ALLOC(d_idx_sorted, max_rev * 4);
    ALLOC(d_heads, max_rev * 4);
    ALLOC(d_head_ctr, 64);
    CU(cudaMemcpyAsync(d_order, order.data(), n * 4, cudaMemcpyHostToDevice, stream));
    CU(cudaMemcpyAsync(d_wpos, w_pos.data(), W * 4, cudaMemcpyHostToDevice, stream));
    CU(cudaMemcpyAsync(d_wlayer, w_layer.data(), W, cudaMemcpyHostToDevice, stream));
    {
        std::vector<uint32_t> iota(max_rev);
        for (size_t i = 0; i < max_rev; ++i) iota[i] = (uint32_t)i;
        CU(cudaMemcpyAsync(d_idx, iota.data(), max_rev * 4, cudaMemcpyHostToDevice, stream));
        CU(cudaStreamSynchronize(stream));
    }
    CU(cub::DeviceRadixSort::SortPairs(nullptr, cub_bytes, d_rev_key.p, d_key_sorted.p, d_idx.p, d_idx_sorted.p, (int)max_rev, 0, 40, stream));
    ALLOC(d_cub, cub_bytes);


    int list_cap = efC, hash_bits;
    int slots = next_pow2(std::max(2048, (efC * s->s0 * 3) / 2));
    slots = std::max(slots, next_pow2(4 * list_cap));
    hash_bits = ilog2(slots);
    size_t smem_search = hs_smem_bytes(s->ld, list_cap, hash_bits);
    if (smem_search > 200 * 1024) return fail(NIDX_EINVAL, "HNSW build search needs %zu bytes of shared memory", smem_search);
    hs_kernel_t kern = pick_search_kernel(s->ld);
    CU(cudaFuncSetAttribute(kern, cudaFuncAttributeMaxDynamicSharedMemorySize, (int)smem_search));
    int occ = 0;
    CU(cudaOccupancyMaxActiveBlocksPerMultiprocessor(&occ, kern, HS_THREADS, smem_search));
    size_t row_bytes = (size_t)s->ld * 4;
    size_t budget = 96 * 1024;
    int cache_sel = (int)std::min<size_t>(M, budget / row_bytes);
    int prune_max = std::max(s->cfg.m0, M) * 95 / 100;
    int cache_rev = (int)std::min<size_t>(prune_max, budget / row_bytes);
    size_t smem_sel = hb_smem_bytes(s->ld, cache_sel), smem_rev = hb_smem_bytes(s->ld, cache_rev);
    CU(cudaFuncSetAttribute(select_link_kernel, cudaFuncAttributeMaxDynamicSharedMemorySize, (int)smem_sel));
    CU(cudaFuncSetAttribute(reverse_link_kernel, cudaFuncAttributeMaxDynamicSharedMemorySize, (int)smem_rev));
    int occ_rev = 0;
    CU(cudaOccupancyMaxActiveBlocksPerMultiprocessor(&occ_rev, reverse_link_kernel, HB_THREADS, smem_rev));
    int rev_grid = std::max(1, occ_rev) * s->sm_count;
    CU(cudaMemsetAsync(s->d_counters, 0, 8 * sizeof(unsigned long long), stream));
    s->last_counters.store(nullptr);


    VecDev V = s->vdev();
    int hr = attach_half_copy(s, &V);
    if (hr) return hr;
    GraphDev G = s->gdev();
    uint32_t begin = 0;
    for (size_t b = 0; b < ends.size(); ++b) {
        uint32_t end = ends[b];
        int nb = (int)(end - begin);
        int nw = (int)(wstart[end] - wstart[begin]);
        SearchArgs a;
        memset(&a, 0, sizeof(a));
        a.mode = 1; a.nq = nb; a.nodes = d_order + begin; a.efC = efC; a.found = d_found; a.found_count = d_found_count;
        a.hash_bits = hash_bits; a.list_cap = list_cap; a.cu_cap = 0; a.work_counter = s->d_work_counter; a.counters = s->d_counters;
        CU(cudaMemsetAsync(s->d_work_counter, 0, 4, stream));
        int grid = std::min(nb, std::max(1, occ) * s->sm_count);
        kern<<<grid, HS_THREADS, smem_search, stream>>>(V, G, a);
        LAUNCHED();
        BuildArgs ba;
        ba.n_work = nw; ba.w_pos = d_wpos + wstart[begin]; ba.w_layer = d_wlayer + wstart[begin]; ba.order = d_order; ba.batch_begin = begin;
        ba.efC = efC; ba.M = M; ba.found = d_found; ba.found_count = d_found_count; ba.rev_key = d_rev_key; ba.rev_x = d_rev_x; ba.rev_sim = d_rev_sim;
        ba.cache_cap = cache_sel;
        select_link_kernel<<<nw, HB_THREADS, smem_sel, stream>>>(V, G, ba);
        LAUNCHED();
        int n_rev = nw * M;
        size_t tmp = cub_bytes;
        CU(cub::DeviceRadixSort::SortPairs(d_cub.p, tmp, d_rev_key.p, d_key_sorted.p, d_idx.p, d_idx_sorted.p, n_rev, 0, 40, stream));
        LAUNCHED();
        ReverseArgs ra;
        ra.n_rev = n_rev; ra.key_sorted = d_key_sorted; ra.idx_sorted = d_idx_sorted; ra.rev_x = d_rev_x; ra.rev_sim = d_rev_sim; ra.cache_cap = cache_rev;
        ra.heads = d_heads; ra.n_heads = d_head_ctr; ra.work_counter = d_head_ctr + 1;
        CU(cudaMemsetAsync(d_head_ctr, 0, 8, stream));
        collect_heads_kernel<<<(n_rev + 255) / 256, 256, 0, stream>>>(d_key_sorted, n_rev, d_heads, d_head_ctr);
        LAUNCHED();
        reverse_link_kernel<<<std::min(n_rev, rev_grid), HB_THREADS, smem_rev, stream>>>(V, G, ra);
        LAUNCHED();
        begin = end;
        if (b == 0 && entry_after_first) {
            s->entry_node = entry_after_first[0];
            s->entry_layer = entry_after_first[1];
            G = s->gdev();
        }
    }
    CU(cudaGetLastError());
    CU(cudaStreamSynchronize(stream));
    return 0;
}

static int run_insertions(nidx_vec_segment* s, const std::vector<uint8_t>& level, const std::vector<uint32_t>& order, const std::vector<uint32_t>& ends,
                          cudaStream_t stream, const uint32_t* entry_after_first = nullptr) {
    int r = insert_batches(s, level, order, ends, stream, entry_after_first);
    if (r) free_graph(s);
    return r;
}

static void batch_ends(uint64_t done, uint64_t n, uint64_t base, int max_batch, std::vector<uint32_t>& ends) {
    if (max_batch <= 0) max_batch = 4096;
    while (done < n) {
        done += std::min<uint64_t>({(uint64_t)max_batch, std::max<uint64_t>(1, done / 16), n - done});
        ends.push_back((uint32_t)(done - base));
    }
}

extern "C" {

int nidx_hnsw_levels(uint64_t n, int32_t m, uint64_t seed, uint8_t* out_level) {
    if (!out_level && n) return fail(NIDX_EINVAL, "null argument");
    if (m < 2) return fail(NIDX_EINVAL, "M must be at least 2");
    host_assign_levels(n, m, seed, out_level);
    return 0;
}

int nidx_vec_build_hnsw(nidx_vec_segment* s, uint64_t seed, int32_t max_batch, void* stream_) {
    if (!s) return fail(NIDX_EINVAL, "null segment");
    CU(cudaSetDevice(s->cfg.device));
    cudaStream_t stream = reinterpret_cast<cudaStream_t>(stream_);
    uint64_t n = s->n;
    std::vector<uint8_t> level(n ? n : 1);
    host_assign_levels(n, s->cfg.m, seed, level.data());
    int r = alloc_graph(s, level.data());
    if (r) return r;
    s->has_graph = true;
    if (n == 0) return 0;

    std::vector<uint32_t> order(n);
    order[0] = s->entry_node;
    for (uint64_t i = 0, j = 1; i < n; ++i) if (i != s->entry_node) order[j++] = (uint32_t)i;
    std::vector<uint32_t> ends;
    batch_ends(0, n, 0, max_batch, ends);
    return run_insertions(s, level, order, ends, stream);
}

int nidx_vec_extend_hnsw(nidx_vec_segment* s, uint64_t n_existing, const uint8_t* level_existing, const uint32_t* adj0, const float* w0,
                         const uint32_t* adjU, const float* wU, uint32_t entry_node, uint32_t entry_layer, uint64_t seed, int32_t max_batch, void* stream_) {
    if (!s || !level_existing || !adj0) return fail(NIDX_EINVAL, "null argument");
    if (!w0 || (adjU && !wU)) return fail(NIDX_EINVAL, "the existing edges' similarities are required (hnsw.edges): the reverse-link prune ranks by them");
    if (n_existing == 0 || n_existing > s->n) return fail(NIDX_EINVAL, "n_existing must be in 1..len");
    if (entry_node >= n_existing || level_existing[entry_node] < entry_layer) return fail(NIDX_EINVAL, "bad entry point");
    CU(cudaSetDevice(s->cfg.device));
    cudaStream_t stream = reinterpret_cast<cudaStream_t>(stream_);
    uint64_t n = s->n;
    std::vector<uint8_t> level(n);
    memcpy(level.data(), level_existing, n_existing);
    for (uint64_t i = 0; i < n_existing; ++i)
        if (level[i] >= HS_MAX_LAYERS) return fail(NIDX_EINVAL, "node %llu has level %d >= %d", (unsigned long long)i, level[i], HS_MAX_LAYERS);
    uint64_t rows_existing = 0;
    for (uint64_t i = 0; i < n_existing; ++i) rows_existing += level[i];
    if (rows_existing && !adjU) return fail(NIDX_EINVAL, "existing nodes have upper layers but adjU is null");
    host_assign_levels(n - n_existing, s->cfg.m, seed, level.data() + n_existing);
    int r = alloc_graph(s, level.data());
    if (r) return r;
    uint32_t raised[2] = {s->entry_node, s->entry_layer};
    bool raises = raised[1] > entry_layer && raised[0] >= n_existing;
    if (raised[1] > entry_layer && !raises) { entry_node = raised[0]; entry_layer = raised[1]; }
    s->entry_layer = entry_layer;
    s->entry_node = entry_node;
    CU(cudaMemcpy(s->d_adj0, adj0, (size_t)n_existing * s->s0 * 4, cudaMemcpyHostToDevice));
    CU(cudaMemcpy(s->d_w0, w0, (size_t)n_existing * s->s0 * 4, cudaMemcpyHostToDevice));
    if (rows_existing) {
        std::vector<uint32_t> fixed_adj;
        std::vector<float> fixed_w;
        uint64_t row = 0;
        for (uint64_t i = 0; i < n_existing; ++i)
            for (int layer = 1; layer <= level[i]; ++layer, ++row) {
                const uint32_t* r0 = adjU + row * s->su;
                bool broken = false;
                for (int j = 0; j < s->su && r0[j] != NIL; ++j)
                    if (r0[j] >= n_existing || level[r0[j]] < layer) { broken = true; break; }
                if (!broken) continue;
                if (fixed_adj.empty()) {
                    fixed_adj.assign(adjU, adjU + rows_existing * s->su);
                    if (wU) fixed_w.assign(wU, wU + rows_existing * s->su);
                }
                uint32_t* dst = fixed_adj.data() + row * s->su;
                float* dw = wU ? fixed_w.data() + row * s->su : nullptr;
                int kept = 0;
                for (int j = 0; j < s->su && r0[j] != NIL; ++j)
                    if (r0[j] < n_existing && level[r0[j]] >= layer) {
                        dst[kept] = r0[j];
                        if (dw) dw[kept] = wU[row * s->su + j];
                        ++kept;
                    }
                for (int j = kept; j < s->su; ++j) { dst[j] = NIL; if (dw) dw[j] = 0.0f; }
            }
        const uint32_t* srcA = fixed_adj.empty() ? adjU : fixed_adj.data();
        const float* srcW = fixed_adj.empty() ? wU : fixed_w.data();
        CU(cudaMemcpy(s->d_adjU, srcA, (size_t)rows_existing * s->su * 4, cudaMemcpyHostToDevice));
        if (wU) CU(cudaMemcpy(s->d_wU, srcW, (size_t)rows_existing * s->su * 4, cudaMemcpyHostToDevice));
    }
    s->has_graph = true;
    if (n == n_existing) return 0;
    std::vector<uint32_t> order;
    order.reserve(n - n_existing);
    if (raises) order.push_back(raised[0]);
    for (uint64_t i = n_existing; i < n; ++i)
        if (!raises || i != raised[0]) order.push_back((uint32_t)i);
    std::vector<uint32_t> ends;
    if (raises) ends.push_back(1);
    batch_ends(n_existing + (raises ? 1 : 0), n, n_existing, max_batch, ends);
    return run_insertions(s, level, order, ends, stream, raises ? raised : nullptr);
}

int nidx_vec_open(const nidx_vec_config* cfg, const char* dir, nidx_vec_segment** out) {
    if (!dir) return fail(NIDX_EINVAL, "null dir");
    if (!out) return fail(NIDX_EINVAL, "null argument");
    std::unique_ptr<nidx_vec_segment> s;
    int r = new_segment(cfg, s);
    if (r) return r;
    std::string err;
    std::vector<unsigned char> raw;
    if (!segio::read_file(std::string(dir) + "/vectors.bin", raw, err)) return fail(NIDX_EIO, "%s", err.c_str());
    size_t rec = (size_t)s->d * 4 + 4;
    if (raw.size() % rec) return fail(NIDX_EIO, "vectors.bin size %zu is not a multiple of the record length %zu", raw.size(), rec);
    uint64_t n = raw.size() / rec;
    s->n = n;
    std::vector<uint32_t> par(n);
    for (uint64_t i = 0; i < n; ++i) memcpy(&par[i], raw.data() + i * rec + (size_t)s->d * 4, 4);
    r = upload_rows(s.get(), raw.data(), rec, true, false);
    if (!r) r = finish_create(s.get(), n ? par.data() : nullptr);
    if (r) return r;
    std::vector<unsigned char> graph, edges;
    if (segio::read_file(std::string(dir) + "/hnsw.graph", graph, err) && !graph.empty()) {
        segio::read_file(std::string(dir) + "/hnsw.edges", edges, err);
        segio::FlatGraph fg;
        if (!segio::parse_graph_v2(graph, edges, n, stride0_for(s->cfg.m0), strideU_for(s->cfg.m), HS_MAX_LAYERS, fg, err))
            return fail(NIDX_EIO, "hnsw.graph: %s", err.c_str());
        r = nidx_vec_set_graph(s.get(), fg.level.data(), fg.adj0.data(), fg.w0.empty() ? nullptr : fg.w0.data(), fg.adjU.data(), fg.wU.empty() ? nullptr : fg.wU.data());
        if (r) return r;
        s->entry_node = fg.entry_node;
        s->entry_layer = fg.entry_layer;
    }
    std::vector<unsigned char> quant;
    if (s->cfg.similarity == NIDX_SIM_DOT && s->d % 64 == 0 && s->d / 32 <= RQ_MAX_WORDS32 && segio::read_file(std::string(dir) + "/vectors.quant", quant, err) && !quant.empty()) {
        size_t rec_q = (size_t)s->d / 8 + 8;
        if (quant.size() != rec_q * n) return fail(NIDX_EIO, "vectors.quant holds %zu bytes, expected %zu records of %zu", quant.size(), (size_t)n, rec_q);
        s->quant_stride = rabitq_stride(s->d);
        ALLOC(s->d_quant, std::max<size_t>((size_t)n * s->quant_stride, 16));
        CU(cudaMemset(s->d_quant, 0, std::max<size_t>((size_t)n * s->quant_stride, 16)));
        CU(cudaMemcpy2D(s->d_quant, (size_t)s->quant_stride, quant.data(), rec_q, rec_q, (size_t)n, cudaMemcpyHostToDevice));
    }
    *out = s.release();
    return 0;
}

int nidx_vec_save(nidx_vec_segment* s, const char* dir) {
    if (!s || !dir) return fail(NIDX_EINVAL, "null argument");
    CU(cudaSetDevice(s->cfg.device));
    CU(cudaDeviceSynchronize());
    uint64_t n = s->n;
    std::vector<float> vecs((size_t)n * s->ld);
    CU(cudaMemcpy(vecs.data(), s->d_vecs, vecs.size() * 4, cudaMemcpyDeviceToHost));
    std::vector<uint32_t> par(n);
    if (s->d_par_of) CU(cudaMemcpy(par.data(), s->d_par_of, n * 4, cudaMemcpyDeviceToHost));
    else for (uint64_t i = 0; i < n; ++i) par[i] = (uint32_t)i;
    std::string err;
    if (!segio::write_vectors_bin(std::string(dir) + "/vectors.bin", vecs.data(), n, s->d, s->ld, par.data(), err)) return fail(NIDX_EIO, "%s", err.c_str());
    if (s->has_graph) {
        segio::FlatGraph fg;
        fg.n = n; fg.s0 = s->s0; fg.su = s->su; fg.entry_node = s->entry_node; fg.entry_layer = s->entry_layer;
        fg.level = s->h_level;
        fg.upper_rows = s->upper_rows;
        fg.adj0.resize((size_t)n * s->s0); fg.w0.resize((size_t)n * s->s0);
        fg.adjU.resize((size_t)s->upper_rows * s->su); fg.wU.resize((size_t)s->upper_rows * s->su);
        int r = nidx_vec_get_graph(s, nullptr, fg.adj0.data(), fg.w0.data(), fg.adjU.data(), fg.wU.data());
        if (r) return r;
        if (!segio::write_graph_v2(std::string(dir) + "/hnsw.graph", std::string(dir) + "/hnsw.edges", fg, err)) return fail(NIDX_EIO, "%s", err.c_str());
    }
    if (s->d_quant) {
        size_t rec_q = (size_t)s->d / 8 + 8;
        std::vector<unsigned char> quant(rec_q * n);
        if (n) CU(cudaMemcpy2D(quant.data(), rec_q, s->d_quant, (size_t)s->quant_stride, rec_q, (size_t)n, cudaMemcpyDeviceToHost));
        FILE* f = fopen((std::string(dir) + "/vectors.quant").c_str(), "wb");
        if (!f) return fail(NIDX_EIO, "cannot write %s/vectors.quant", dir);
        size_t wr = quant.empty() ? 0 : fwrite(quant.data(), 1, quant.size(), f);
        fclose(f);
        if (wr != quant.size()) return fail(NIDX_EIO, "short write to %s/vectors.quant", dir);
    }
    return 0;
}

struct nidx_txt_segment {
    int device = 0, sm_count = 0;
    uint32_t n_docs = 0, n_terms = 0;
    uint64_t n_post = 0;
    DevArray<uint64_t> d_term_off;
    DevArray<uint2> d_post;
    DevArray<uint32_t> d_skip_row;
    DevArray<uint32_t> d_skip;
    uint32_t n_fine = 0;
    DevArray<uint64_t> d_alive;
    DevArray<float> d_weight;
    DevArray<float> d_norm_cache;
    DevArray<uint64_t> d_doc_keys;
    std::vector<uint64_t> own_df;
    uint64_t own_tokens = 0;
    cudaEvent_t ev_k0 = nullptr, ev_k1 = nullptr;
    std::vector<std::string> facet_keys;
    DevArray<uint32_t> d_fdoc_off;
    DevArray<uint32_t> d_ford;
    uint64_t n_facet_ords = 0;
    DevArray<int64_t> d_secs[2];
    DevArray<uint32_t> d_rank[2];
    uint32_t n_ranks[2] = {0, 0};
    DevArray<uint64_t> d_pos_off;
    DevArray<uint32_t> d_pos;
    std::vector<float> idf;
    DevArray<uint32_t> d_res_ord, d_field_ord;
    WorkspacePool pool;

    ~nidx_txt_segment() {
        if (ev_k0) cudaEventDestroy(ev_k0);
        if (ev_k1) cudaEventDestroy(ev_k1);
    }
};

static uint32_t fieldnorm_id_to_value(uint32_t id) {
    if (id < 24) return id;
    uint32_t j = id - 24, bits = j & 7, shift = j >> 3;
    return 24 + (shift == 0 ? bits : ((bits | 8u) << (shift - 1)));
}

static int txt_upload_stats(nidx_txt_segment* t, uint64_t total_docs, uint64_t total_tokens, const uint64_t* df) {
    const float K1 = 1.2f, B = 0.75f;
    float avg = (float)total_tokens / (float)total_docs;
    float cache[256];
    for (int i = 0; i < 256; ++i) cache[i] = K1 * (1.0f - B + B * (float)fieldnorm_id_to_value(i) / avg);
    std::vector<float> weight(t->n_terms), idf(t->n_terms);
    for (uint32_t i = 0; i < t->n_terms; ++i) {
        float x = ((float)(total_docs - df[i]) + 0.5f) / ((float)df[i] + 0.5f);
        idf[i] = logf(1.0f + x);
        weight[i] = idf[i] * (1.0f + K1);
    }
    CU(cudaMemcpy(t->d_norm_cache, cache, sizeof(cache), cudaMemcpyHostToDevice));
    if (t->n_terms) CU(cudaMemcpy(t->d_weight, weight.data(), (size_t)t->n_terms * 4, cudaMemcpyHostToDevice));
    t->idf = std::move(idf);
    return 0;
}

int nidx_txt_create(int32_t device, uint32_t n_docs, uint32_t n_terms, const uint64_t* term_off, const uint32_t* post_doc, const uint32_t* post_tf,
                    const uint8_t* fieldnorm_id, nidx_txt_segment** out) {
    if (!term_off || !fieldnorm_id || !out) return fail(NIDX_EINVAL, "null argument");
    int r = check_device(device);
    if (r) return r;
    if (n_docs >= (1u << 31)) return fail(NIDX_EINVAL, "at most 2^31-1 documents per segment");
    std::unique_ptr<nidx_txt_segment> t(new nidx_txt_segment());
    t->device = device; t->n_docs = n_docs; t->n_terms = n_terms; t->n_post = term_off[n_terms];
    cudaDeviceProp prop;
// ... 1173 lines not shown
```

### nucliadb_b200/csrc/common.cuh

```cuda
#pragma once
#include <cuda_fp16.h>
#include <cuda_runtime.h>
#include <stdint.h>

namespace nidx {

constexpr uint32_t NIL = 0xFFFFFFFFu;
constexpr int SIM_DOT = 0, SIM_COSINE = 1, SIM_L2 = 2;

struct VecDev {
    const float* vecs;
    const float* norms;
    const uint32_t* paragraph_of;
    uint32_t n;
    int d, ld, sim;
    const __half* hvecs;
    const float4* hrec;
    int ldh;
};

__host__ __device__ __forceinline__ int dot_depth(int ld) { return (ld / 4 + 31) / 32 + 7; }

struct GraphDev {
    uint32_t n;
    int M, M0, s0, su;
    const uint8_t* level;
    uint32_t entry_node, entry_layer;
    uint32_t* adj0; float* w0;
    const uint64_t* upper_off;
    uint32_t* adjU; float* wU;
    __device__ __forceinline__ uint32_t* row(uint32_t node, int layer) const {
        return layer == 0 ? adj0 + (size_t)node * s0 : adjU + (upper_off[node] + (uint64_t)(layer - 1)) * su;
    }
    __device__ __forceinline__ float* wrow(uint32_t node, int layer) const {
        return layer == 0 ? w0 + (size_t)node * s0 : wU + (upper_off[node] + (uint64_t)(layer - 1)) * su;
    }
    __device__ __forceinline__ int stride(int layer) const { return layer == 0 ? s0 : su; }
    __device__ __forceinline__ int mmax(int layer) const { return layer == 0 ? M0 : M; }
};

__device__ __forceinline__ uint32_t ordered_bits(float f) {
    uint32_t u = __float_as_uint(f);
    return (u & 0x80000000u) ? ~u : (u | 0x80000000u);
}
__device__ __forceinline__ float from_ordered_bits(uint32_t o) {
    uint32_t u = (o & 0x80000000u) ? (o & 0x7FFFFFFFu) : ~o;
    return __uint_as_float(u);
}
__device__ __forceinline__ uint64_t make_key(float score, uint32_t id, uint32_t flag) {
    return ((uint64_t)ordered_bits(score) << 32) | (uint64_t)(((0x7FFFFFFFu - id) << 1) | (flag & 1u));
}
__device__ __forceinline__ uint32_t key_id(uint64_t k) { return 0x7FFFFFFFu - ((uint32_t)k >> 1); }
__device__ __forceinline__ float key_score(uint64_t k) { return from_ordered_bits((uint32_t)(k >> 32)); }
__device__ __forceinline__ uint32_t key_flag(uint64_t k) { return (uint32_t)k & 1u; }

__device__ __forceinline__ float4 ldg_stream(const float4* p) {
    float4 r;
    asm volatile("ld.global.nc.L1::no_allocate.v4.f32 {%0, %1, %2, %3}, [%4];" : "=f"(r.x), "=f"(r.y), "=f"(r.z), "=f"(r.w) : "l"(p));
    return r;
}

__device__ __forceinline__ float butterfly_sum(float v) {
#pragma unroll
    for (int off = 16; off >= 1; off >>= 1) v = __fadd_rn(v, __shfl_xor_sync(0xFFFFFFFFu, v, off));
    return v;
}

__device__ __forceinline__ float warp_dot(const float4* __restrict__ a, const float4* __restrict__ b, int ngroups, int lane) {
    float ax = 0.f, ay = 0.f, az = 0.f, aw = 0.f;
    for (int base = 0; base < ngroups; base += 256) {
        float4 va[8];
#pragma unroll
        for (int j = 0; j < 8; ++j) {
            int g = base + j * 32 + lane;
            va[j] = g < ngroups ? ldg_stream(a + g) : make_float4(0.f, 0.f, 0.f, 0.f);
        }
#pragma unroll
        for (int j = 0; j < 8; ++j) {
            int g = base + j * 32 + lane;
            if (g < ngroups) {
                float4 vb = b[g];
                ax = __fmaf_rn(va[j].x, vb.x, ax);
                ay = __fmaf_rn(va[j].y, vb.y, ay);
                az = __fmaf_rn(va[j].z, vb.z, az);
                aw = __fmaf_rn(va[j].w, vb.w, aw);
            }
        }
    }
    return butterfly_sum(__fadd_rn(__fadd_rn(ax, ay), __fadd_rn(az, aw)));
}

template <int NG>
__device__ __forceinline__ float warp_dot_t(const float4* __restrict__ a, const float4* __restrict__ b, int ngroups, int lane) {
    if constexpr (NG == 0) {
        return warp_dot(a, b, ngroups, lane);
    } else {
        float4 va[NG];
#pragma unroll
        for (int j = 0; j < NG; ++j) va[j] = ldg_stream(a + j * 32 + lane);
        float ax = 0.f, ay = 0.f, az = 0.f, aw = 0.f;
#pragma unroll
        for (int j = 0; j < NG; ++j) {
            float4 vb = b[j * 32 + lane];
            ax = __fmaf_rn(va[j].x, vb.x, ax);
            ay = __fmaf_rn(va[j].y, vb.y, ay);
            az = __fmaf_rn(va[j].z, vb.z, az);
            aw = __fmaf_rn(va[j].w, vb.w, aw);
        }
        return butterfly_sum(__fadd_rn(__fadd_rn(ax, ay), __fadd_rn(az, aw)));
    }
}

__device__ __forceinline__ uint2 ldg_stream2(const uint2* p) {
    uint2 r;
    asm volatile("ld.global.nc.L1::no_allocate.v2.u32 {%0, %1}, [%2];" : "=r"(r.x), "=r"(r.y) : "l"(p));
    return r;
}

template <int NG>
__device__ __forceinline__ float warp_dot_h(const uint2* __restrict__ a, const float4* __restrict__ b, int ngroups, int lane) {
    float ax = 0.f, ay = 0.f, az = 0.f, aw = 0.f;
    auto acc = [&](uint2 h, float4 vb) {
        float2 lo = __half22float2(*reinterpret_cast<const __half2*>(&h.x)), hi = __half22float2(*reinterpret_cast<const __half2*>(&h.y));
        ax = __fmaf_rn(lo.x, vb.x, ax);
        ay = __fmaf_rn(lo.y, vb.y, ay);
        az = __fmaf_rn(hi.x, vb.z, az);
        aw = __fmaf_rn(hi.y, vb.w, aw);
    };
    if constexpr (NG == 0) {
        for (int g = lane; g < ngroups; g += 32) acc(ldg_stream2(a + g), b[g]);
    } else {
        uint2 va[NG];
#pragma unroll
        for (int j = 0; j < NG; ++j) va[j] = ldg_stream2(a + j * 32 + lane);
#pragma unroll
        for (int j = 0; j < NG; ++j) acc(va[j], b[j * 32 + lane]);
    }
    return butterfly_sum(__fadd_rn(__fadd_rn(ax, ay), __fadd_rn(az, aw)));
}

__device__ __forceinline__ void cp_async4(void* smem_dst, const void* gmem_src) {
    unsigned s = (unsigned)__cvta_generic_to_shared(smem_dst);
    asm volatile("cp.async.ca.shared.global [%0], [%1], 4;" ::"r"(s), "l"(gmem_src));
}
__device__ __forceinline__ void cp_async_commit_wait_all() {
    asm volatile("cp.async.commit_group;\n\tcp.async.wait_all;" ::: "memory");
}
__device__ __forceinline__ void prefetch_l2(const void* p) { asm volatile("prefetch.global.L2 [%0];" :: "l"(p)); }

__device__ __forceinline__ float cosine_from_parts(float ab, float na, float nb) {
    if (na == 0.0f && nb == 0.0f) return 1.0f;
    if (ab == 0.0f) return 0.0f;
    float c = __fdiv_rn(ab, __fmul_rn(na, nb));
    float dist = __fsub_rn(1.0f, c);
    if (!(dist > 0.0f)) dist = 0.0f;
    return __fsub_rn(1.0f, dist);
}

__device__ __forceinline__ float l2_from_parts(float ab, float na, float nb) {
    return __fsub_rn(__fmul_rn(2.0f, ab), __fadd_rn(__fmul_rn(na, na), __fmul_rn(nb, nb)));
}
__device__ __forceinline__ float sim_from_parts(int sim, float ab, float na, float nb) {
    return sim == SIM_COSINE ? cosine_from_parts(ab, na, nb) : (sim == SIM_L2 ? l2_from_parts(ab, na, nb) : ab);
}
__device__ __forceinline__ float finish_similarity(const VecDev& V, float ab, uint32_t x, float qnorm) {
    return V.sim == SIM_DOT ? ab : sim_from_parts(V.sim, ab, V.norms[x], qnorm);
}

}
```

### nucliadb_b200/csrc/hnsw_search.cuh

```cuda
#pragma once
#include <limits.h>

#include "common.cuh"

namespace nidx {

constexpr int HS_WARPS = 8;
constexpr int HS_THREADS = HS_WARPS * 32;
constexpr int HS_MAX_ROW = 64;
constexpr int HS_MAX_LAYERS = 8;

struct SearchArgs {
    int mode;
    int nq;
    const float* queries;
    const float* qnorms;
    int k, ef0;
    float min_score;
    int with_duplicates, multi_vector;
    const uint64_t* filter;
    uint32_t* out_ids; float* out_scores; int* out_counts;
    const uint32_t* nodes;
    int efC;
    uint64_t* found;
    int* found_count;
    int hash_bits;
    int list_cap;
    int cu_cap;
    unsigned int* work_counter;
    unsigned long long* counters;
    const unsigned char* codes;
    int code_stride;
    const uint32_t* planes;
    const void* qparams;
    uint32_t* gvisited;
    int gv_bits;
    int last_k;
};

struct VisitedSet {
    uint32_t* slots;
    uint32_t mask;
    int bits;
    int limit;

    __device__ void init(uint32_t* s, int b) {
        slots = s; bits = b; mask = (1u << b) - 1;
        limit = (int)((15u << b) >> 4) - HS_MAX_ROW;
    }
    __device__ uint32_t slot(uint32_t y) const { return (y * 2654435761u) >> (32 - bits); }
    __device__ void clear() const {
        const uint4 e4 = make_uint4(NIL, NIL, NIL, NIL);
        for (uint32_t i = threadIdx.x; i < (mask + 1) / 4; i += blockDim.x) reinterpret_cast<uint4*>(slots)[i] = e4;
    }
    __device__ bool insert(uint32_t y, int count, bool& overflow) const {
        if (count >= limit) { overflow = true; return false; }
        for (uint32_t h = slot(y);; h = (h + 1) & mask) {
            const uint32_t old = atomicCAS(&slots[h], NIL, y);
            if (old == NIL) return true;
            if (old == y) return false;
        }
    }
};

struct HopRec {
    unsigned long long maxtodo;
    int ntodo;
    int nadmit;
    int best_next;
    int pred;
    int nfresh;
    int overflow;

    __device__ void clear() { maxtodo = 0; nadmit = 0; best_next = INT_MAX; nfresh = 0; overflow = 0; }
};

struct SearchCtx {
    float* qvec;
    uint64_t *A, *B;
    VisitedSet vis;
    uint32_t* todo_id;
    uint64_t* todo_key;
    uint32_t* pref_row;
    uint32_t* pref_node;
    int *s_len, *s_best, *s_hash_count, *s_flag;
    HopRec* hops;
    unsigned hop;
    float qnorm;
    float qbound;
    unsigned long long n_dist, n_expand, n_overflow;
    unsigned long long n_skip;

    __device__ HopRec& last_hop() const { return hops[(hop & 1u) ^ 1u]; }
};

__device__ inline float hs_query_bound(const float* q, int ld) {
    double s = 0.0;
    for (int i = threadIdx.x & 31; i < ld; i += 32) s = fma((double)q[i], (double)q[i], s);
#pragma unroll
    for (int off = 16; off >= 1; off >>= 1) s += __shfl_xor_sync(0xFFFFFFFFu, s, off);
    return __double2float_ru(__dsqrt_ru(__dmul_ru(s, 1.0 + 0x1p-20)));
}

__device__ __forceinline__ bool hs_screened_out(const VecDev& V, const SearchCtx& c, uint32_t y, float ah, float4 r, uint64_t wkey) {
    float a = __fmul_rn(ah, r.y);
    float bnd = __fmaf_ru(c.qbound, r.z, r.w);
    if (!(fabsf(a) <= 0x1p120f && bnd <= 0x1p100f)) return false;
    float s_up = sim_from_parts(V.sim, __fadd_ru(a, bnd), r.x, c.qnorm);
    return make_key(s_up, y, 1) <= wkey;
}

__host__ __device__ __forceinline__ size_t hs_smem_bytes(int ld, int list_cap, int hash_bits) {
    return (size_t)ld * 4 + (size_t)list_cap * 16 + ((size_t)4 << hash_bits) + HS_MAX_ROW * 12 + HS_MAX_ROW * 8 + 16 + 64;
}

__device__ inline unsigned char* hs_setup(SearchCtx& c, const SearchArgs& a, unsigned char* p, int ld) {
    __shared__ int s_ints[4];
    __shared__ HopRec s_hops[2];
    c.qvec = reinterpret_cast<float*>(p); p += (size_t)ld * 4;
    c.A = reinterpret_cast<uint64_t*>(p); p += (size_t)a.list_cap * 8;
    c.B = reinterpret_cast<uint64_t*>(p); p += (size_t)a.list_cap * 8;
    c.todo_key = reinterpret_cast<uint64_t*>(p); p += HS_MAX_ROW * 8;
    c.vis.init(reinterpret_cast<uint32_t*>(p), a.hash_bits); p += (size_t)4 << a.hash_bits;
    c.todo_id = reinterpret_cast<uint32_t*>(p); p += HS_MAX_ROW * 4;
    c.pref_row = reinterpret_cast<uint32_t*>(p); p += 2 * HS_MAX_ROW * 4;
    c.pref_node = reinterpret_cast<uint32_t*>(p); p += 16;
    c.s_len = &s_ints[0]; c.s_best = &s_ints[1]; c.s_hash_count = &s_ints[2]; c.s_flag = &s_ints[3];
    c.hops = s_hops;
    c.hop = 0;
    c.qnorm = 0.0f;
    c.n_dist = c.n_expand = c.n_overflow = c.n_skip = 0;
    return p;
}

__device__ inline bool hs_next_query(const SearchArgs& a, unsigned* q) {
    __shared__ unsigned s_work;
    __syncthreads();
    if (threadIdx.x == 0) s_work = atomicAdd(a.work_counter, 1u);
    __syncthreads();
    *q = s_work;
    return *q < (unsigned)a.nq;
}

__device__ inline void hs_flush_counters(const SearchCtx& c, unsigned long long* counters) {
    if ((threadIdx.x & 31) == 0 && c.n_dist) atomicAdd(&counters[0], c.n_dist);
    if (threadIdx.x == 0) {
        if (c.n_expand) atomicAdd(&counters[1], c.n_expand);
        if (c.n_overflow & 0xFFFFFFFFull) atomicAdd(&counters[2], c.n_overflow & 0xFFFFFFFFull);
        if (c.n_overflow >> 32) atomicAdd(&counters[3], c.n_overflow >> 32);
    }
}

__device__ inline void hs_reseed(SearchCtx& c, const VisitedSet& vis) {
    __syncthreads();
    vis.clear();
    if (threadIdx.x == 0) {
        *c.s_hash_count = 0; *c.s_best = 0; c.pref_node[0] = NIL; c.pref_node[1] = NIL;
        c.hops[0].clear(); c.hops[1].clear();
    }
    __syncthreads();
    int len = *c.s_len;
    bool ov = false;
    for (int i = threadIdx.x; i < len; i += blockDim.x) {
        uint64_t key = c.A[i] | 1ull;
        c.A[i] = key;
        vis.insert(key_id(key), 0, ov);
    }
    __syncthreads();
    if (threadIdx.x == 0) *c.s_hash_count = len;
    __syncthreads();
}

template <bool CU>
__device__ inline int hs_prefetch_next(const GraphDev& G, SearchCtx& c, int layer, int best, int len) {
    const int lane = threadIdx.x & 31;
    const int stride = G.stride(layer);
    int pred = -1;
    if (CU) {
        pred = len > 1 ? 1 : -1;
    } else {
        for (int i0 = best + 1; i0 < len && pred < 0; i0 += 32) {
            int i = i0 + lane;
            unsigned m = __ballot_sync(0xFFFFFFFFu, i < len && (c.A[i] & 1ull));
            if (m) pred = i0 + __ffs(m) - 1;
        }
    }
    uint32_t pnode = NIL;
    if (pred >= 0) {
        pnode = key_id(c.A[pred]);
        const uint32_t* row = G.row(pnode, layer);
        uint32_t* dst = c.pref_row + ((c.hop & 1u) ^ 1u) * HS_MAX_ROW;
        for (int e = lane; e < stride; e += 32) cp_async4(dst + e, row + e);
    }
    if (lane == 0) c.pref_node[(c.hop & 1u) ^ 1u] = pnode;
    return pred;
}

template <bool CU, int NG, int W = HS_WARPS, bool LEAN = false>
__device__ inline void hs_expand(const VecDev& V, const GraphDev& G, SearchCtx& c, uint32_t node, int layer, int ef, float min_score, int best, int len_in = -1) {
    int lane = threadIdx.x & 31, warp = threadIdx.x >> 5;
    int stride = G.stride(layer);
    unsigned cur = c.hop & 1u;
    HopRec& h = c.hops[cur];
    if (warp == 0) {
        const uint32_t* prow = c.pref_row + cur * HS_MAX_ROW;
        bool hit = c.pref_node[cur] == node;
        const uint32_t* row = G.row(node, layer);
        const int visited = *c.s_hash_count;
        int ntodo = 0;
        bool ov = false;
        for (int e0 = 0; e0 < stride; e0 += 32) {
            uint32_t y = NIL;
            if (e0 + lane < stride) y = hit ? prow[e0 + lane] : __ldg(row + e0 + lane);
            bool fresh = (y != NIL) && c.vis.insert(y, visited, ov);
            unsigned mask = __ballot_sync(0xFFFFFFFFu, fresh);
            if (fresh) c.todo_id[ntodo + __popc(mask & ((1u << lane) - 1))] = y;
            ntodo += __popc(mask);
        }
        if (__any_sync(0xFFFFFFFFu, ov) && lane == 0) c.n_overflow++;
        if (lane == 0) {
            h.ntodo = ntodo;
            *c.s_hash_count = visited + ntodo;
            h.best_next = INT_MAX;
            h.nadmit = 0;
            h.maxtodo = 0;
            c.n_expand++;
        }
    } else if (warp == W - 1) {
        hs_prefetch_next<CU>(G, c, layer, best, LEAN ? len_in : *c.s_len);
    }
    __syncthreads();
    int ntodo = h.ntodo, len = LEAN ? len_in : *c.s_len;
    uint64_t wkey = (!CU && len >= ef) ? c.A[len - 1] : 0;
    int ng = V.ld >> 2;
    auto finish = [&](int j, uint32_t y, float ab, float vnorm) {
        float s = sim_from_parts(V.sim, ab, vnorm, c.qnorm);
        uint64_t key = make_key(s, y, 1);
        bool admit = CU ? (s >= min_score) : (wkey == 0 || s > key_score(wkey));
        c.todo_key[j] = admit ? key : 0;
        if (admit) { atomicAdd(&h.nadmit, 1); atomicMax(&h.maxtodo, (unsigned long long)key); }
        c.n_dist++;
    };
    const bool screen = !CU && wkey != 0 && V.hvecs != nullptr;
    auto skip = [&](int j) { c.todo_key[j] = 0; c.n_dist++; c.n_skip++; };
    const float4* qv = reinterpret_cast<const float4*>(c.qvec);
    auto frow = [&](uint32_t y) { return reinterpret_cast<const float4*>(V.vecs + (size_t)y * V.ld); };
    auto hrow = [&](uint32_t y) { return reinterpret_cast<const uint2*>(V.hvecs + (size_t)y * V.ldh); };
    const int lines = screen ? (V.ldh * 2 + 127) >> 7 : (V.ld * 4 + 127) >> 7;
    for (int j = warp + W; j < ntodo; j += W) {
        const char* rowp = screen ? reinterpret_cast<const char*>(hrow(c.todo_id[j])) : reinterpret_cast<const char*>(frow(c.todo_id[j]));
        for (int l = lane; l < lines; l += 32) prefetch_l2(rowp + (size_t)l * 128);
    }
    for (int j = warp; j < ntodo; j += W) {
        uint32_t y = c.todo_id[j];
        float vnorm;
        if (screen) {
            float4 r = __ldg(V.hrec + y);
            float ah = warp_dot_h<NG>(hrow(y), qv, ng, lane);
            if (hs_screened_out(V, c, y, ah, r, wkey)) { if (lane == 0) skip(j); continue; }
            vnorm = r.x;
        } else vnorm = V.sim != SIM_DOT ? __ldg(V.norms + y) : 0.0f;
        float ab = warp_dot_t<NG>(frow(y), qv, ng, lane);
        if (lane == 0) finish(j, y, ab, vnorm);
    }
    if (warp == W - 1) cp_async_commit_wait_all();
    c.hop++;
    __syncthreads();
}

template <bool CU, bool LEAN = false>
__device__ inline void hs_merge(SearchCtx& c, int cap, int best, int ntodo, int* len_io = nullptr, int* best_io = nullptr) {
    HopRec& h = c.last_hop();
    int len = LEAN ? *len_io : *c.s_len;
    int first = CU ? 1 : 0;
    int my_best = INT_MAX;
    const uint64_t maxtodo = h.maxtodo;
    const int nadmit = h.nadmit;
    int* const bn = &h.best_next;
    for (int t = threadIdx.x; t < len - first + ntodo; t += blockDim.x) {
        uint64_t key;
        int p;
        if (t < len - first) {
            int i = t + first;
            key = c.A[i];
            if (!CU && i == best) key &= ~1ull;
            int shift = 0;
            if (key < maxtodo)
                for (int j = 0; j < ntodo; ++j) shift += (c.todo_key[j] > key);
            p = t + shift;
        } else {
            int j = t - (len - first);
            key = c.todo_key[j];
            if (key == 0) continue;
            int r = 0;
            for (int jj = 0; jj < ntodo; ++jj) r += (c.todo_key[jj] > key);
            int lo = first, hi = len;
            while (lo < hi) {
                int mid = (lo + hi) >> 1;
                if (c.A[mid] > key) lo = mid + 1; else hi = mid;
            }
            p = r + (lo - first);
        }
        if (p < cap) {
            c.B[p] = key;
            if (key & 1ull) my_best = min(my_best, p);
        }
    }
    my_best = __reduce_min_sync(0xFFFFFFFFu, my_best);
    if ((threadIdx.x & 31) == 0 && my_best != INT_MAX) atomicMin(bn, my_best);
    __syncthreads();
    int nl = len - first + nadmit;
    const bool over = nl > cap;
    if (over) nl = cap;
    const int nb = *bn;
    if (threadIdx.x == 0) {
        if (over && CU) c.n_overflow += (1ull << 32);
        *c.s_len = nl;
        *c.s_best = nb;
    }
    uint64_t* t = c.A; c.A = c.B; c.B = t;
    if (LEAN) { *len_io = nl; *best_io = nb; }
    else __syncthreads();
}

template <int NG, int W = HS_WARPS>
__device__ inline void hs_layer_search(const VecDev& V, const GraphDev& G, SearchCtx& c, int layer, int ef) {
    int best = *c.s_best, len = *c.s_len;
    while (best < len) {
        uint64_t ckey = c.A[best];
        hs_expand<false, NG, W, true>(V, G, c, key_id(ckey), layer, ef, 0.0f, best, len);
        hs_merge<false, true>(c, ef, best, c.last_hop().ntodo, &len, &best);
    }
}

__device__ inline bool hs_passes(const VecDev& V, const SearchArgs& a, uint32_t node, float score, const uint32_t* acc_ids,
                                 const float* acc_scores, int nacc, int lane) {
    uint32_t p = V.paragraph_of ? V.paragraph_of[node] : node;
    if (a.filter && !((a.filter[p >> 6] >> (p & 63)) & 1)) return false;
    if (!a.with_duplicates) {
        const float4* x = reinterpret_cast<const float4*>(V.vecs + (size_t)node * V.ld);
        for (int i = 0; i < nacc; ++i) {
            if (__float_as_uint(acc_scores[i]) != __float_as_uint(score)) continue;
            const float4* y = reinterpret_cast<const float4*>(V.vecs + (size_t)acc_ids[i] * V.ld);
            bool same = true;
            for (int g = lane; g < (V.ld >> 2); g += 32) {
                float4 u = x[g], w = y[g];
                same = same && __float_as_uint(u.x) == __float_as_uint(w.x) && __float_as_uint(u.y) == __float_as_uint(w.y) &&
                       __float_as_uint(u.z) == __float_as_uint(w.z) && __float_as_uint(u.w) == __float_as_uint(w.w);
            }
            if (__all_sync(0xFFFFFFFFu, same)) return false;
        }
    }
    if (a.multi_vector) {
        for (int i = 0; i < nacc; ++i) {
            uint32_t ap = V.paragraph_of ? V.paragraph_of[acc_ids[i]] : acc_ids[i];
            if (ap == p) return false;
        }
    }
    return true;
}

template <int NG, int W = HS_WARPS>
__device__ inline int hs_closest_up(const VecDev& V, const GraphDev& G, SearchCtx& c, const SearchArgs& a, uint32_t* out_ids, float* out_scores) {
    int lane = threadIdx.x & 31, warp = threadIdx.x >> 5;
    hs_reseed(c, c.vis);
    int nacc = 0;
    while (true) {
        int len = *c.s_len;
        if (len == 0) break;
        uint64_t ckey = c.A[0];
        float score = key_score(ckey);
        uint32_t node = key_id(ckey);
        if (score < a.min_score) break;
        __syncthreads();
        if (warp == 0) {
            bool pass = !(score != score) && hs_passes(V, a, node, score, out_ids, out_scores, nacc, lane);
            if (lane == 0) {
                *c.s_flag = pass;
                if (pass) { out_ids[nacc] = node; out_scores[nacc] = score; }
            }
        }
        __syncthreads();
        nacc += *c.s_flag;
        if (nacc == a.k) break;
        hs_expand<true, NG, W>(V, G, c, node, 0, 0, a.min_score, 0);
        hs_merge<true>(c, a.cu_cap, 0, c.last_hop().ntodo);
    }
    return nacc;
}

template <int NG, int W = HS_WARPS>
__device__ inline void hs_emit_results(const VecDev& V, const GraphDev& G, SearchCtx& c, const SearchArgs& a, unsigned int q) {
    uint32_t* oi = a.out_ids + (size_t)q * a.k;
    float* os = a.out_scores + (size_t)q * a.k;
    int nacc = hs_closest_up<NG, W>(V, G, c, a, oi, os);
    __syncthreads();
    {
        uint32_t* tid = reinterpret_cast<uint32_t*>(c.B);
        float* tsc = reinterpret_cast<float*>(c.B) + a.k;
        for (int i = threadIdx.x; i < nacc; i += blockDim.x) { tid[i] = oi[i]; tsc[i] = os[i]; }
        __syncthreads();
        for (int i = threadIdx.x; i < nacc; i += blockDim.x) {
            uint32_t oi_bits = ordered_bits(tsc[i]);
            int r = 0;
            for (int j = 0; j < nacc; ++j) {
                uint32_t oj = ordered_bits(tsc[j]);
                r += (oj > oi_bits) || (oj == oi_bits && j < i);
            }
            oi[r] = tid[i];
            os[r] = tsc[i];
        }
        __syncthreads();
    }
    for (int i = nacc + threadIdx.x; i < a.k; i += blockDim.x) { oi[i] = NIL; os[i] = 0.0f; }
    if (threadIdx.x == 0) a.out_counts[q] = nacc;
}

template <int NG>
__global__ void __launch_bounds__(HS_THREADS, 4) hnsw_search_kernel(VecDev V, GraphDev G, SearchArgs a) {
    extern __shared__ __align__(16) unsigned char smem[];
    SearchCtx c;
    hs_setup(c, a, smem, V.ld);
    int lane = threadIdx.x & 31;
    int ng = V.ld >> 2;

    unsigned q;
    while (hs_next_query(a, &q)) {
        const float* qsrc;
        uint32_t self = NIL;
        if (a.mode == 0) { qsrc = a.queries + (size_t)q * V.ld; c.qnorm = V.sim != SIM_DOT ? a.qnorms[q] : 0.0f; }
        else { self = a.nodes[q]; qsrc = V.vecs + (size_t)self * V.ld; c.qnorm = V.sim != SIM_DOT ? V.norms[self] : 0.0f; }
        for (int i = threadIdx.x; i < ng; i += blockDim.x) reinterpret_cast<float4*>(c.qvec)[i] = reinterpret_cast<const float4*>(qsrc)[i];
        __syncthreads();
        if (V.hvecs) c.qbound = hs_query_bound(c.qvec, V.ld);

        if (threadIdx.x < 32) {
            uint32_t ep = G.entry_node;
            float ab = warp_dot_t<NG>(reinterpret_cast<const float4*>(V.vecs + (size_t)ep * V.ld), reinterpret_cast<const float4*>(c.qvec), ng, lane);
            if (lane == 0) {
                c.A[0] = make_key(finish_similarity(V, ab, ep, c.qnorm), ep, 1);
                *c.s_len = 1;
                c.n_dist++;
            }
        }
        __syncthreads();

        int top = a.mode == 1 ? (int)G.level[self] : -1;
        for (int layer = (int)G.entry_layer; layer >= 0; --layer) {
            int ef;
            if (a.mode == 0) ef = layer == 0 ? a.ef0 : 1;
            else ef = layer <= top ? a.efC : 1;
            hs_reseed(c, c.vis);
            hs_layer_search<NG>(V, G, c, layer, ef);
            __syncthreads();
            if (a.mode == 1 && layer <= top && layer < HS_MAX_LAYERS) {
                int len = *c.s_len;
                uint64_t* dst = a.found + ((size_t)q * HS_MAX_LAYERS + layer) * a.efC;
                for (int i = threadIdx.x; i < len; i += blockDim.x) dst[i] = c.A[i];
                if (threadIdx.x == 0) a.found_count[(size_t)q * HS_MAX_LAYERS + layer] = len;
            }
            __syncthreads();
        }

        if (a.mode == 1 && threadIdx.x == 0)
            for (int layer = (int)G.entry_layer + 1; layer <= top && layer < HS_MAX_LAYERS; ++layer) a.found_count[(size_t)q * HS_MAX_LAYERS + layer] = 0;

        if (a.mode == 0) hs_emit_results<NG>(V, G, c, a, q);
    }
    hs_flush_counters(c, a.counters);
    if (lane == 0 && c.n_dist) atomicAdd(&a.counters[6], c.n_dist - c.n_skip);
}

}
```

### nucliadb_b200/segment.py

```python
from __future__ import annotations

import ctypes as C
from typing import Optional

import numpy as np

from . import _lib
from ._lib import NIL, NidxError, TxtSearchParams, VecConfig, VecSearchParams, check, ptr


def _is_torch(x) -> bool:
    return hasattr(x, "data_ptr") and hasattr(x, "is_cuda")


def _torch_stream(device: int):
    import torch

    return C.c_void_p(torch.cuda.current_stream(device).cuda_stream)


_SIGNED = {"uint32": "int32", "uint64": "int64"}


def _stage(device: int, on_device: bool, stream: Optional[int] = None):
    if on_device:
        import torch

        def alloc(shape, dtype, zero=False):
            name = np.dtype(dtype).name
            return torch.empty(shape, dtype=getattr(torch, _SIGNED.get(name, name)), device=torch.device("cuda", device))

        return _lib.NIDX_MEM_DEVICE, _torch_stream(device), alloc
    return _lib.NIDX_MEM_HOST, C.c_void_p(stream) if stream else None, lambda shape, dtype, zero=False: (np.zeros if zero else np.empty)(shape, dtype)


def normalize(vectors: np.ndarray, device: int = 0) -> np.ndarray:
    assert vectors.dtype == np.float32 and vectors.flags.c_contiguous
    if vectors.size:
        rows = vectors.reshape(-1, vectors.shape[-1])
        check(_lib.require_device().nidx_normalize_vectors(device, ptr(rows), rows.shape[0], rows.shape[1], rows.shape[1], _lib.NIDX_MEM_HOST, None))
    return vectors


class VectorSegment:
    def __init__(self, handle, cfg: VecConfig):
        self._h, self.cfg = handle, cfg

    @classmethod
    def create(cls, vectors, dimension: int, similarity=_lib.NIDX_SIM_COSINE, m=30, m0=60, ef_construction=100, ef_search=30, device=0,
               multi_vector=False, paragraph_of: Optional[np.ndarray] = None) -> "VectorSegment":
        L = _lib.require_device()
        cfg = VecConfig(dimension, similarity, int(multi_vector), m, m0, ef_construction, ef_search, device)
        h = C.c_void_p()
        if _is_torch(vectors):
            assert vectors.is_cuda and vectors.is_contiguous() and vectors.dtype.is_floating_point
            n, ld = vectors.shape
            mem = _lib.NIDX_MEM_DEVICE
        else:
            vectors = np.ascontiguousarray(vectors, dtype=np.float32)
            n, ld = vectors.shape if vectors.ndim == 2 else (0, dimension)
            mem = _lib.NIDX_MEM_HOST
        par = None if paragraph_of is None else np.ascontiguousarray(paragraph_of, dtype=np.uint32)
        check(L.nidx_vec_create(C.byref(cfg), ptr(vectors) if n else None, n, ld, mem, ptr(par), C.byref(h)))
        return cls(h, cfg)

    @classmethod
    def open(cls, directory: str, dimension: int, similarity=_lib.NIDX_SIM_COSINE, m=30, m0=60, ef_construction=100, ef_search=30, device=0,
             multi_vector=False) -> "VectorSegment":
        L = _lib.require_device()
        cfg = VecConfig(dimension, similarity, int(multi_vector), m, m0, ef_construction, ef_search, device)
        h = C.c_void_p()
        check(L.nidx_vec_open(C.byref(cfg), directory.encode(), C.byref(h)))
        return cls(h, cfg)

    def save(self, directory: str):
        check(_lib.load().nidx_vec_save(self._h, directory.encode()))

    def close(self):
        if self._h is not None:
            _lib.load().nidx_vec_close(self._h)
            self._h = None

    def __del__(self):
        try:
            self.close()
        except Exception:
            pass

    def __len__(self):
        return int(_lib.load().nidx_vec_len(self._h))

    def build_hnsw(self, seed=2, max_batch=4096):
        check(_lib.load().nidx_vec_build_hnsw(self._h, seed, max_batch, None))

    def extend_hnsw(self, n_existing, level, adj0, adjU, w0, wU, entry_node, entry_layer, seed=2, max_batch=4096):
        level = np.ascontiguousarray(level, dtype=np.uint8)
        adj0 = np.ascontiguousarray(adj0, dtype=np.uint32)
        adjU = np.ascontiguousarray(adjU, dtype=np.uint32)
        w0 = np.ascontiguousarray(w0, dtype=np.float32)
        wU = np.ascontiguousarray(wU, dtype=np.float32)
        check(_lib.load().nidx_vec_extend_hnsw(self._h, n_existing, ptr(level), ptr(adj0), ptr(w0), ptr(adjU), ptr(wU), entry_node, entry_layer, seed,
                                               max_batch, None))

    def graph_dims(self):
        s0, su, rows, en, el = C.c_int32(), C.c_int32(), C.c_uint64(), C.c_uint32(), C.c_uint32()
        check(_lib.load().nidx_vec_graph_dims(self._h, C.byref(s0), C.byref(su), C.byref(rows), C.byref(en), C.byref(el)))
        return s0.value, su.value, rows.value, en.value, el.value

    def set_graph(self, level, adj0, adjU, w0=None, wU=None):
        level = np.ascontiguousarray(level, dtype=np.uint8)
        adj0 = np.ascontiguousarray(adj0, dtype=np.uint32)
        adjU = np.ascontiguousarray(adjU, dtype=np.uint32)
        w0 = None if w0 is None else np.ascontiguousarray(w0, dtype=np.float32)
        wU = None if wU is None else np.ascontiguousarray(wU, dtype=np.float32)
        check(_lib.load().nidx_vec_set_graph(self._h, ptr(level), ptr(adj0), ptr(w0), ptr(adjU), ptr(wU)))

    def get_graph(self):
        s0, su, rows, en, el = self.graph_dims()
        n = len(self)
        level = np.empty(n, dtype=np.uint8)
        adj0 = np.empty((n, s0), dtype=np.uint32)
        w0 = np.empty((n, s0), dtype=np.float32)
        adjU = np.full((max(rows, 1), su), NIL, dtype=np.uint32)
        wU = np.zeros((max(rows, 1), su), dtype=np.float32)
        check(_lib.load().nidx_vec_get_graph(self._h, ptr(level), ptr(adj0), ptr(w0), ptr(adjU), ptr(wU)))
        return dict(level=level, adj0=adj0, w0=w0, adjU=adjU, wU=wU, entry_node=en, entry_layer=el, s0=s0, su=su, upper_rows=rows)

    def set_alive(self, alive_bits: Optional[np.ndarray]):
        check(_lib.load().nidx_vec_set_alive(self._h, ptr(alive_bits), _lib.NIDX_MEM_HOST))

    def set_paragraph_keys(self, keys: Optional[np.ndarray]):
        keys = None if keys is None else np.ascontiguousarray(keys, dtype=np.uint64)
        check(_lib.load().nidx_vec_set_paragraph_keys(self._h, ptr(keys)))

    def set_inverted_index(self, which, keys, postings):
        key_bytes, key_off = _pack_keys(keys)
        post_off = np.zeros(len(keys) + 1, dtype=np.uint64)
        post_off[1:] = np.cumsum([len(p) for p in postings]) if len(keys) else []
        flat = np.asarray([p for ps in postings for p in ps] or [0], dtype=np.uint32)
        check(_lib.load().nidx_vec_set_inverted_index(self._h, which, len(keys), ptr(key_bytes), ptr(key_off), ptr(post_off), ptr(flat)))

    def filter(self, nodes, n, out_bits: Optional[np.ndarray] = None) -> int:
        matching = C.c_uint64()
        check(_lib.load().nidx_vec_filter(self._h, nodes, n, ptr(out_bits), _lib.NIDX_MEM_HOST, C.byref(matching), None))
        return matching.value

    def prefilter_bits(self, doc_bits, join, n_docs: int, n_paragraphs: int, formula=None, op=_lib.NIDX_F_AND):
        on_device = _is_torch(doc_bits)
        mem, stream, alloc = _stage(self.cfg.device, on_device)
        if not on_device:
            doc_bits = np.ascontiguousarray(doc_bits, dtype=np.uint64)
            join = np.ascontiguousarray(join, dtype=np.uint32)
        out = alloc((n_paragraphs + 63) // 64, np.uint64)
        matching = C.c_uint64()
        check(_lib.load().nidx_vec_prefilter_bits(self._h, ptr(doc_bits), n_docs, ptr(join), formula, 0 if formula is None else len(formula), op, ptr(out), mem,
                                                  C.byref(matching), stream))
        return out, matching.value

    def search(self, queries, k: int, ef: int = 0, min_score: float = -1.0, with_duplicates=True, method=_lib.NIDX_METHOD_AUTO,
               filter_bits=None, filter_matching: int = 0, formula=None, out=None, stream: Optional[int] = None):
        mem, stream, alloc = _stage(self.cfg.device, _is_torch(queries), stream)
        if mem == _lib.NIDX_MEM_DEVICE:
            import torch

            assert queries.is_cuda and queries.is_contiguous() and queries.dtype == torch.float32
        else:
            queries = np.ascontiguousarray(np.atleast_2d(queries), dtype=np.float32)
            filter_bits = None if filter_bits is None else np.ascontiguousarray(filter_bits, dtype=np.uint64)
        nq, ldq = queries.shape
        out = out or (alloc((nq, k), np.uint32), alloc((nq, k), np.float32), alloc(nq, np.int32))
        p = VecSearchParams(k, ef, min_score, int(with_duplicates), method, ptr(filter_bits), filter_matching)
        L = _lib.load()
        fn, by_formula = (L.nidx_vec_search, ()) if formula is None else (L.nidx_vec_search_formula, (formula, len(formula)))
        check(fn(self._h, ptr(queries), nq, ldq, mem, C.byref(p), *by_formula, ptr(out[0]), ptr(out[1]), ptr(out[2]), stream))
        return out

    def rabitq_encode(self):
        check(_lib.load().nidx_vec_rabitq_encode(self._h, None))

    def rabitq_codes(self) -> np.ndarray:
        out = np.empty((len(self), self.cfg.dimension // 8 + 8), dtype=np.uint8)
        check(_lib.load().nidx_vec_rabitq_codes(self._h, ptr(out)))
        return out

    def rabitq_estimate(self, queries):
        queries = np.ascontiguousarray(np.atleast_2d(queries), dtype=np.float32)
        nq = queries.shape[0]
        est = np.empty((nq, len(self)), dtype=np.float32)
        err = np.empty((nq, len(self)), dtype=np.float32)
        check(_lib.load().nidx_vec_rabitq_estimate(self._h, ptr(queries), nq, queries.shape[1], _lib.NIDX_MEM_HOST, ptr(est), ptr(err), None))
        return est, err

    def last_kernel_ms(self) -> float:
        ms = C.c_float()
        check(_lib.load().nidx_vec_last_kernel_ms(self._h, C.byref(ms)))
        return ms.value

    def counters_ex(self):
        out = (C.c_uint64 * 6)()
        check(_lib.load().nidx_vec_counters_ex(self._h, out))
        return dict(similarities=out[0], expansions=out[1], overflows=out[2] + out[3], estimates=out[4], rerank_needed=out[5])

    def counters(self):
        out = (C.c_uint64 * 3)()
        check(_lib.load().nidx_vec_counters(self._h, out))
        return dict(similarities=out[0], expansions=out[1], overflows=out[2])

    def exact_rows(self) -> int:
        out = C.c_uint64()
        check(_lib.load().nidx_vec_exact_rows(self._h, C.byref(out)))
        return out.value

    def scan_counters(self):
        out = (C.c_uint64 * 2)()
        check(_lib.load().nidx_vec_scan_counters(self._h, out))
        return dict(survivors=out[0], full_scans=out[1])


def _merge_parts(entry, ids, scores, device, part_stride, out):
    n_parts, nq, k = ids.shape
    _, stream, alloc = _stage(device, True)
    out = out or (alloc((nq, k), np.uint32), alloc((nq, k), np.float32), alloc((nq, k), np.int32))
    check(getattr(_lib.load(), entry)(device, ptr(ids), ptr(scores), n_parts, part_stride, nq, k, ptr(out[0]), ptr(out[1]), ptr(out[2]), stream))
    return out


def merge_topk(ids, scores, device=0, part_stride=0, out=None):
    return _merge_parts("nidx_merge_topk", ids, scores, device, part_stride, out)


def merge_vector_parts(ids, scores, device=0, part_stride=0, out=None):
    return _merge_parts("nidx_merge_vector_parts", ids, scores, device, part_stride, out)


def _pack_keys(keys):
    off = np.zeros(len(keys) + 1, dtype=np.uint64)
    off[1:] = np.cumsum([len(k) for k in keys]) if len(keys) else []
    return np.frombuffer(b"".join(keys) + b"\0", dtype=np.uint8).copy(), off


def _facet_request(facets):
    kb, ko = _pack_keys(list(facets))
    return _lib.TxtFacetRequest(len(facets), ptr(kb), ptr(ko)), (kb, ko)


def _txt_params(k, mode=_lib.NIDX_BM25_OR, use_tf=True, min_score=0.0, after=None, docaddr_base=0):
    p = TxtSearchParams(k, mode, int(use_tf), min_score, 0, 0.0, 0, docaddr_base)
    if after is not None:
        p.after_score, p.after_mode, p.after_docaddr = float(after[0]), int(after[1]), int(after[2])
    return p


class TextSegment:
    def __init__(self, handle, n_docs, n_terms, device):
        self._h, self.n_docs, self.n_terms, self.device = handle, n_docs, n_terms, device

    @classmethod
    def create(cls, n_docs, n_terms, term_off, post_doc, post_tf, fieldnorm_id, device=0) -> "TextSegment":
        L = _lib.require_device()
        term_off = np.ascontiguousarray(term_off, dtype=np.uint64)
        post_doc = np.ascontiguousarray(post_doc, dtype=np.uint32)
        post_tf = np.ascontiguousarray(post_tf, dtype=np.uint32)
        fieldnorm_id = np.ascontiguousarray(fieldnorm_id, dtype=np.uint8)
        h = C.c_void_p()
        check(L.nidx_txt_create(device, n_docs, n_terms, ptr(term_off), ptr(post_doc), ptr(post_tf), ptr(fieldnorm_id), C.byref(h)))
        return cls(h, n_docs, n_terms, device)

    def set_stats(self, total_docs: int, total_tokens: int, doc_freq: Optional[np.ndarray] = None):
        df = None if doc_freq is None else np.ascontiguousarray(doc_freq, dtype=np.uint64)
        check(_lib.load().nidx_txt_set_stats(self._h, total_docs, total_tokens, ptr(df)))

    def set_alive(self, alive_bits: Optional[np.ndarray]):
        check(_lib.load().nidx_txt_set_alive(self._h, ptr(alive_bits)))

    def _queries(self, query_terms, query_off):
        mem, stream, alloc = _stage(self.device, _is_torch(query_terms))
        if mem == _lib.NIDX_MEM_DEVICE:
            return mem, stream, alloc, query_terms, query_off, query_off.numel() - 1
        query_off = np.ascontiguousarray(query_off, dtype=np.uint32)
        return mem, stream, alloc, np.ascontiguousarray(query_terms, dtype=np.uint32), query_off, len(query_off) - 1

    def search(self, query_terms, query_off, k, mode=_lib.NIDX_BM25_OR, use_tf=True, min_score=0.0, out=None, after=None, docaddr_base=0):
        p = _txt_params(k, mode, use_tf, min_score, after, docaddr_base)
        mem, stream, alloc, query_terms, query_off, nq = self._queries(query_terms, query_off)
        out = out or (alloc((nq, k), np.uint32), alloc((nq, k), np.float32), alloc(nq, np.int32), alloc(nq, np.uint64))
        check(_lib.load().nidx_txt_search(self._h, ptr(query_terms), ptr(query_off), nq, mem, C.byref(p), *map(ptr, out), stream))
        return out

    def set_facets(self, keys, doc_off, doc_ords):
        kb, ko = _pack_keys(keys)
        doc_off = np.ascontiguousarray(doc_off, dtype=np.uint64)
        doc_ords = np.ascontiguousarray(doc_ords, dtype=np.uint32)
        check(_lib.load().nidx_txt_set_facets(self._h, len(keys), ptr(kb), ptr(ko), ptr(doc_off), ptr(doc_ords)))

    def facet_buckets(self, facets):
        req, _keep = _facet_request(facets)
        n = C.c_uint32()
        check(_lib.load().nidx_txt_facet_buckets(self._h, C.byref(req), None, None, 0, C.byref(n)))
        b_req, b_ord = np.empty(n.value, dtype=np.uint32), np.empty(n.value, dtype=np.uint32)
        check(_lib.load().nidx_txt_facet_buckets(self._h, C.byref(req), ptr(b_req), ptr(b_ord), n.value, C.byref(n)))
        return b_req, b_ord

    def search_faceted(self, query_terms, query_off, k, facets, mode=_lib.NIDX_BM25_OR, use_tf=True, min_score=0.0, after=None, docaddr_base=0):
        p = _txt_params(k, mode, use_tf, min_score, after, docaddr_base)
        nb = len(self.facet_buckets(facets)[0])
        req, _keep = _facet_request(facets)
        mem, stream, alloc, query_terms, query_off, nq = self._queries(query_terms, query_off)
        out = (alloc((nq, k), np.uint32), alloc((nq, k), np.float32), alloc(nq, np.int32), alloc(nq, np.uint64), alloc((nq, nb), np.uint32, zero=True))
        check(_lib.load().nidx_txt_search_faceted(self._h, ptr(query_terms), ptr(query_off), nq, mem, C.byref(p), C.byref(req), *map(ptr, out), stream))
        return out

    def facet_count_all(self, facets, device_out=False):
        nb = len(self.facet_buckets(facets)[0])
        req, _keep = _facet_request(facets)
        mem, stream, alloc = _stage(self.device, device_out)
        out = alloc(nb, np.uint32, zero=True)
        check(_lib.load().nidx_txt_facet_count_all(self._h, C.byref(req), mem, ptr(out), stream))
        return out

    def set_dates(self, created, modified):
        created = np.ascontiguousarray(created, dtype=np.int64)
        modified = np.ascontiguousarray(modified, dtype=np.int64)
        assert len(created) == self.n_docs and len(modified) == self.n_docs
        check(_lib.load().nidx_txt_set_dates(self._h, ptr(created), ptr(modified)))

    def search_ordered(self, query_terms, query_off, k, field=_lib.NIDX_ORDER_CREATED, order=_lib.NIDX_ORDER_DESC, mode=_lib.NIDX_BM25_OR, facets=None):
        p = TxtSearchParams(k, mode, 0, 0.0, 0, 0.0, 0, 0)
        o = _lib.TxtOrder(field, order)
        req, _keep = _facet_request(facets) if facets is not None else (None, None)
        mem, stream, alloc, query_terms, query_off, nq = self._queries(query_terms, query_off)
        out = (alloc((nq, k), np.uint32), alloc((nq, k), np.int64), alloc(nq, np.int32), alloc(nq, np.uint64))
        if facets is not None:
            out += (alloc((nq, len(self.facet_buckets(facets)[0])), np.uint32, zero=True),)
        check(_lib.load().nidx_txt_search_ordered(self._h, ptr(query_terms), ptr(query_off), nq, mem, C.byref(p), C.byref(o),
                                                  C.byref(req) if req is not None else None, *map(ptr, out[:4]), ptr(out[4]) if facets is not None else None,
                                                  stream))
        return out

    def set_positions(self, positions):
        positions = np.ascontiguousarray(positions, dtype=np.uint32)
        check(_lib.load().nidx_txt_set_positions(self._h, ptr(positions), len(positions)))

    def search_phrases(self, query_terms, query_off, phrases, k, mode=_lib.NIDX_BM25_OR, use_tf=True, min_score=0.0, after=None, docaddr_base=0,
                       order=None, facets=None):
        p = _txt_params(k, mode, use_tf, min_score, after, docaddr_base)
        terms = np.asarray([t for _, ts in phrases for t in ts], dtype=np.uint32)
        poff = np.zeros(len(phrases) + 1, dtype=np.uint32)
        poff[1:] = np.cumsum([len(ts) for _, ts in phrases])
        pq = np.asarray([q for q, _ in phrases], dtype=np.uint32)
        ph = _lib.TxtPhrases(ptr(terms), ptr(poff), ptr(pq), len(phrases))
        o = _lib.TxtOrder(*order) if order is not None else None
        req, _keep = _facet_request(facets) if facets is not None else (None, None)
        nb = len(self.facet_buckets(facets)[0]) if facets is not None else 0
        mem, stream, alloc, query_terms, query_off, nq = self._queries(query_terms, query_off)
        out = (alloc((nq, k), np.uint32), alloc((nq, k), np.int64 if order is not None else np.float32), alloc(nq, np.int32), alloc(nq, np.uint64))
        if facets is not None:
            out += (alloc((nq, nb), np.uint32, zero=True),)
        scores, dates = (None, out[1]) if order is not None else (out[1], None)
        check(_lib.load().nidx_txt_search_phrases(self._h, ptr(query_terms), ptr(query_off), nq, mem, C.byref(p), C.addressof(ph),
                                                  C.byref(o) if o is not None else None, C.byref(req) if req is not None else None,
                                                  ptr(out[0]), ptr(scores), ptr(dates), ptr(out[2]), ptr(out[3]),
                                                  ptr(out[4]) if facets is not None else None, stream))
        return out

    def list_ordered(self, k, field=_lib.NIDX_ORDER_CREATED, order=_lib.NIDX_ORDER_DESC, device_out=False):
        o = _lib.TxtOrder(field, order)
        mem, stream, alloc = _stage(self.device, device_out)
        out = (alloc(k, np.uint32), alloc(k, np.int64), alloc(1, np.int32, zero=True), alloc(1, np.uint64, zero=True))
        check(_lib.load().nidx_txt_list_ordered(self._h, C.byref(o), k, mem, *map(ptr, out), stream))
        return out if device_out else (out[0], out[1], int(out[2][0]), int(out[3][0]))

    def set_doc_columns(self, resource_ord, field_ord):
        resource_ord = np.ascontiguousarray(resource_ord, dtype=np.uint32)
        field_ord = np.ascontiguousarray(field_ord, dtype=np.uint32)
        assert len(resource_ord) == self.n_docs and len(field_ord) == self.n_docs
        check(_lib.load().nidx_txt_set_doc_columns(self._h, ptr(resource_ord), ptr(field_ord)))

    def prefilter(self, nodes, out=None):
        on_device = out is not None and _is_torch(out)
        mem, stream, alloc = _stage(self.device, on_device)
        if out is None:
            out = alloc((self.n_docs + 63) // 64, np.uint64)
        matching = C.c_uint64()
        check(_lib.load().nidx_txt_prefilter(self._h, C.addressof(nodes), len(nodes), ptr(out), mem, C.byref(matching), stream))
        return out, matching.value

    def set_doc_keys(self, keys: Optional[np.ndarray]):
        k = None if keys is None else np.ascontiguousarray(keys, dtype=np.uint64)
        check(_lib.load().nidx_txt_set_doc_keys(self._h, ptr(k)))

    def last_kernel_ms(self) -> float:
        ms = C.c_float()
        check(_lib.load().nidx_txt_last_kernel_ms(self._h, C.byref(ms)))
        return ms.value

    def close(self):
        if self._h is not None:
            _lib.load().nidx_txt_close(self._h)
            self._h = None

    def __del__(self):
        try:
            self.close()
        except Exception:
            pass
```

Measured before the change: 451,000.

## Add PCA-prefix projection screening to prune HNSW candidates before exact distance

Computes a low-dimensional orthonormal basis from a sampled covariance matrix using power iteration. Each vector is projected onto this basis and stored as half-precision codes with rigorous error bounds. During HNSW expansion, a cheap prefix dot plus those bounds screens out neighbours that provably cannot be admitted, so exact fp32 dots are computed only for survivors. This replaces the full fp16 screening copy when the basis captures enough energy, trading extra build-time work, per-query projection setup and a two-phase expand for fewer full-row reads.

```diff
diff --git a/include/nidx_b200.h b/include/nidx_b200.h
--- a/include/nidx_b200.h
+++ b/include/nidx_b200.h
@@ -120,6 +120,7 @@
 int nidx_vec_counters(nidx_vec_segment* seg, uint64_t out[3]);
 int nidx_vec_counters_ex(nidx_vec_segment* seg, uint64_t out[6]);
 int nidx_vec_exact_rows(nidx_vec_segment* seg, uint64_t* out);
+int nidx_vec_prefix_rows(nidx_vec_segment* seg, uint64_t* out);
 int nidx_vec_scan_counters(nidx_vec_segment* seg, uint64_t out[2]);
 
 int nidx_vec_rabitq_encode(nidx_vec_segment* seg, void* stream);
diff --git a/nucliadb_b200/_lib.py b/nucliadb_b200/_lib.py
--- a/nucliadb_b200/_lib.py
+++ b/nucliadb_b200/_lib.py
@@ -115,6 +115,7 @@
     "nidx_vec_counters": (i32, [P, P]),
     "nidx_vec_counters_ex": (i32, [P, P]),
     "nidx_vec_exact_rows": (i32, [P, P]),
+    "nidx_vec_prefix_rows": (i32, [P, P]),
     "nidx_vec_scan_counters": (i32, [P, P]),
     "nidx_vec_rabitq_encode": (i32, [P, P]),
     "nidx_vec_rabitq_codes": (i32, [P, P]),
diff --git a/nucliadb_b200/csrc/api.cu b/nucliadb_b200/csrc/api.cu
--- a/nucliadb_b200/csrc/api.cu
+++ b/nucliadb_b200/csrc/api.cu
@@ -226,6 +226,9 @@
     DevArray<__half> d_hvecs;
     DevArray<float4> d_hrec;
     int ldh = 0;
+    DevArray<uint4> d_pvecs;
+    DevArray<float> d_basis;
+    float basis_norm = 0.0f;
     bool half_decided = false;
     std::mutex half_mu;
 
@@ -238,6 +241,7 @@
         VecDev v;
         v.vecs = d_vecs; v.norms = d_norms; v.paragraph_of = d_par_of; v.n = (uint32_t)n; v.d = d; v.ld = ld; v.sim = cfg.similarity;
         v.hvecs = nullptr; v.hrec = nullptr; v.ldh = 0;
+        v.pvecs = nullptr; v.basis = nullptr; v.bnorm = 0.0f;
         return v;
     }
     GraphDev gdev() const {
@@ -302,7 +306,7 @@
     if (__any_sync(0xFFFFFFFFu, bad) && (threadIdx.x & 31) == 0) atomicOr(out + 1, 1u);
 }
 
-__global__ void hs_half_kernel(VecDev V, uint64_t n, int ldh, __half* __restrict__ hv, float4* __restrict__ rec) {
+__global__ void hs_half_kernel(VecDev V, uint64_t n, int ldh, __half* __restrict__ hv, float4* __restrict__ rec, int rstride) {
     const int lane = threadIdx.x & 31;
     const double slack = 1.0 + 0x1p-20, mu = dot_depth(V.ld) * 0x1p-24, gm = mu / (1.0 - mu);
     for (uint64_t i = (blockIdx.x * (uint64_t)blockDim.x + threadIdx.x) >> 5; i < n; i += ((uint64_t)gridDim.x * blockDim.x) >> 5) {
@@ -319,7 +323,7 @@
         for (int k = lane; k < ldh; k += 32) {
             float x = k < V.ld ? v[k] : 0.0f;
             __half h = __float2half_rn(__fmul_rn(x, up));
-            hv[i * ldh + k] = h;
+            if (hv) hv[i * ldh + k] = h;
             double dd = (double)__half2float(h) * (double)down - (double)x;
             r2 = fma(dd, dd, r2);
             v2 = fma((double)x, (double)x, v2);
@@ -329,12 +333,220 @@
             double rho = sqrt(r2 * slack), vn = sqrt(v2 * slack);
             double eq = (rho + gm * (2.0 * vn + rho)) * slack;
             double ea = 0x1p-149 * ((double)V.ld * (1.0 + (double)down) + 1.0) * slack;
-            rec[i] = make_float4(V.norms[i], down, finite ? __double2float_ru(eq) : INFINITY, __double2float_ru(ea));
-        }
+            rec[i * rstride] = make_float4(V.norms[i], down, finite ? __double2float_ru(eq) : INFINITY, __double2float_ru(ea));
+        }
+    }
+}
+
+constexpr int HS_PREFIX_SAMPLE = 32768;
+constexpr int HS_PREFIX_ROUNDS = 8;
+constexpr double HS_PREFIX_MIN_ENERGY = 0.9;
+
+__global__ void hs_cov_kernel(VecDev V, uint64_t stride, int S, float* __restrict__ C) {
+    __shared__ float xi[32][33], xj[32][33];
+    const int tx = threadIdx.x, ty = threadIdx.y, i0 = blockIdx.y * 32, j0 = blockIdx.x * 32;
+    float acc[4] = {0.f, 0.f, 0.f, 0.f};
+    for (int r0 = 0; r0 < S; r0 += 32) {
+        for (int rr = ty; rr < 32; rr += 8) {
+            float a = 0.f, b = 0.f;
+            if (r0 + rr < S) {
+                const uint64_t row = (uint64_t)(r0 + rr) * stride;
+                const float nv = V.norms[row];
+                if (nv > 0.0f && nv <= FLT_MAX) {
+                    const float sc = 1.0f / nv;
+                    if (i0 + tx < V.ld) a = V.vecs[row * V.ld + i0 + tx] * sc;
+                    if (j0 + tx < V.ld) b = V.vecs[row * V.ld + j0 + tx] * sc;
+                }
+            }
+            xi[rr][tx] = a;
+            xj[rr][tx] = b;
+        }
+        __syncthreads();
+        for (int rr = 0; rr < 32; ++rr)
+#pragma unroll
+            for (int e = 0; e < 4; ++e) acc[e] = __fmaf_rn(xi[rr][ty + 8 * e], xj[rr][tx], acc[e]);
+        __syncthreads();
+    }
+#pragma unroll
+    for (int e = 0; e < 4; ++e)
+        if (i0 + ty + 8 * e < V.ld && j0 + tx < V.ld) C[(size_t)(i0 + ty + 8 * e) * V.ld + j0 + tx] = acc[e];
+}
+
+__global__ void hs_cov_apply_kernel(const float* __restrict__ C, int ld, const double* __restrict__ Q, double* __restrict__ Z) {
+    const int i = blockIdx.x * blockDim.x + threadIdx.x, p = blockIdx.y;
+    if (i >= ld) return;
+    double z = 0.0;
+    for (int j = 0; j < ld; ++j) z = fma((double)C[(size_t)j * ld + i], Q[(size_t)p * ld + j], z);
+    Z[(size_t)p * ld + i] = z;
+}
+
+__global__ void __launch_bounds__(256) hs_prefix_kernel(VecDev V, uint64_t n, const double* __restrict__ G, uint4* __restrict__ pv,
+                                                        float4* __restrict__ rec) {
+    __shared__ float xs[32][33], bs[HS_P][33];
+    __shared__ double ps[32][HS_P];
+    const int t = threadIdx.x, rr = t >> 3, g = t & 7, ld = V.ld;
+    const double slack = 1.0 + 0x1p-20, gam = (double)(ld + 2 * HS_P + 8) * 0x1p-51, bF = (double)V.bnorm;
+    const double g12 = 12.0 * 0x1p-24 / (1.0 - 12.0 * 0x1p-24);
+    for (uint64_t r0 = (uint64_t)blockIdx.x * 32; r0 < n; r0 += (uint64_t)gridDim.x * 32) {
+        double acc[8] = {0, 0, 0, 0, 0, 0, 0, 0}, v2 = 0.0;
+        bool fin = true;
+        for (int k0 = 0; k0 < ld; k0 += 32) {
+            for (int e = t; e < 32 * 32; e += 256) {
+                const int a = e >> 5, k = k0 + (e & 31);
+                xs[a][e & 31] = (r0 + a < n && k < ld) ? V.vecs[(r0 + a) * ld + k] : 0.0f;
+            }
+            for (int e = t; e < HS_P * 32; e += 256) {
+                const int a = e >> 5, k = k0 + (e & 31);
+                bs[a][e & 31] = k < ld ? V.basis[(size_t)a * ld + k] : 0.0f;
+            }
+            __syncthreads();
+            for (int kk = 0; kk < 32; ++kk) {
+                const double x = (double)xs[rr][kk];
+#pragma unroll
+                for (int i = 0; i < 8; ++i) acc[i] = fma(x, (double)bs[8 * g + i][kk], acc[i]);
+                if (g == 0) { fin = fin && isfinite(x); v2 = fma(x, x, v2); }
+            }
+            __syncthreads();
+        }
+        const uint64_t row = r0 + rr;
+        v2 = __shfl_sync(0xFFFFFFFFu, v2, 0, 8);
+        fin = __shfl_sync(0xFFFFFFFFu, (int)fin, 0, 8) != 0;
+        double m = 0.0;
+#pragma unroll
+        for (int i = 0; i < 8; ++i) m = fmax(m, fabs(acc[i]));
+        for (int off = 4; off >= 1; off >>= 1) m = fmax(m, __shfl_xor_sync(0xFFFFFFFFu, m, off));
+        int ep = 0;
+        if (m > 0.0) { int ex; frexp(m, &ex); ep = min(15 - ex, 126); }
+        const bool ok = fin && m <= 0x1p1000 && ep >= -127;
+        const double up = ldexp(1.0, ep), down = ldexp(1.0, -ep);
+        __half h[8];
+        double pp = 0.0, yp = 0.0;
+#pragma unroll
+        for (int i = 0; i < 8; ++i) {
+            h[i] = ok ? __double2half(acc[i] * up) : __float2half(0.0f);
+            const double pt = (double)__half2float(h[i]) * down;
+            ps[rr][8 * g + i] = pt;
+            pp = fma(pt, pt, pp);
+            yp = fma(acc[i], pt, yp);
+        }
+        __syncwarp();
+        double pgp = 0.0, ss = 0.0;
+#pragma unroll
+        for (int i = 0; i < 8; ++i) {
+            const double* gr = G + (size_t)(8 * g + i) * HS_P;
+            double tq = 0.0;
+            for (int q = 0; q < HS_P; ++q) tq = fma(__ldg(gr + q), ps[rr][q], tq);
+            pgp = fma(ps[rr][8 * g + i], tq, pgp);
+            const double sp = acc[i] - tq;
+            ss = fma(sp, sp, ss);
+        }
+        for (int off = 4; off >= 1; off >>= 1) {
+            pp += __shfl_xor_sync(0xFFFFFFFFu, pp, off);
+            yp += __shfl_xor_sync(0xFFFFFFFFu, yp, off);
+            pgp += __shfl_xor_sync(0xFFFFFFFFu, pgp, off);
+            ss += __shfl_xor_sync(0xFFFFFFFFu, ss, off);
+        }
+        if (row < n) {
+            uint4 line;
+            memcpy(&line, h, 16);
+            pv[row * (HS_P / 8) + g] = line;
+            if (g == 0) {
+                const double vn = sqrt(v2 * slack) * slack, pn = sqrt(pp * slack) * slack;
+                const double r2 = fmax(v2 - 2.0 * yp + pgp, 0.0) + gam * (vn + 2.0 * bF * pn) * (vn + 2.0 * bF * pn);
+                const double tau = sqrt(r2 * slack) * slack;
+                const double sig = (sqrt(ss * slack) + 1.5 * gam * bF * (vn + bF * pn)) * slack + g12 * pn * slack;
+                rec[2 * row + 1] = ok ? make_float4((float)down, __double2float_ru(tau), __double2float_ru(sig), __double2float_ru(pn))
+                                      : make_float4(1.0f, INFINITY, 0.0f, 0.0f);
+            }
+        }
+        __syncthreads();
+    }
+}
+
+static void prefix_orthonormalise(std::vector<double>& Z, int ld) {
+    for (int p = 0; p < HS_P; ++p) {
+        double* zp = Z.data() + (size_t)p * ld;
+        double n0 = 0.0;
+        for (int k = 0; k < ld; ++k) n0 += zp[k] * zp[k];
+        for (int q = 0; q < p; ++q) {
+            const double* zq = Z.data() + (size_t)q * ld;
+            double d = 0.0;
+            for (int k = 0; k < ld; ++k) d += zp[k] * zq[k];
+            for (int k = 0; k < ld; ++k) zp[k] -= d * zq[k];
+        }
+        double n1 = 0.0;
+        for (int k = 0; k < ld; ++k) n1 += zp[k] * zp[k];
+        const double sc = n1 > 1e-24 * n0 && n1 > 0.0 ? 1.0 / sqrt(n1) : 0.0;
+        for (int k = 0; k < ld; ++k) zp[k] *= sc;
     }
 }
 
 constexpr size_t HS_HALF_MARGIN = (size_t)4 << 30;
+static int prefix_basis(nidx_vec_segment* s, DevArray<double>& dg, bool* selected) {
+    *selected = false;
+    const int ld = s->ld;
+    if (ld < 4 * HS_P || s->n < (uint64_t)HS_P) return 0;
+    const size_t pbytes = (size_t)s->n * (HS_P * 2 + 32), cbytes = (size_t)ld * ld * 4, qbytes = (size_t)HS_P * ld * 8;
+    size_t free_b = 0, total_b = 0;
+    CU(cudaMemGetInfo(&free_b, &total_b));
+    if (free_b < pbytes + cbytes + 2 * qbytes + HS_HALF_MARGIN) return 0;
+    DevArray<float> C;
+    DevArray<double> dq, dz;
+    if (C.try_alloc(cbytes) != cudaSuccess || dq.try_alloc(qbytes) != cudaSuccess || dz.try_alloc(qbytes) != cudaSuccess ||
+        dg.try_alloc((size_t)HS_P * HS_P * 8) != cudaSuccess)
+        return 0;
+    const int S = (int)std::min<uint64_t>(s->n, HS_PREFIX_SAMPLE);
+    const uint64_t stride = s->n / (uint64_t)S;
+    const VecDev V = s->vdev();
+    hs_cov_kernel<<<dim3((ld + 31) / 32, (ld + 31) / 32), dim3(32, 8)>>>(V, stride, S, C);
+    LAUNCHED();
+    CU(cudaGetLastError());
+    std::vector<double> Q((size_t)HS_P * ld, 0.0), Z((size_t)HS_P * ld);
+    uint64_t st = 0x9E3779B97F4A7C15ull;
+    auto next = [&st] {
+        uint64_t z = (st += 0x9E3779B97F4A7C15ull);
+        z = (z ^ (z >> 30)) * 0xBF58476D1CE4E5B9ull;
+        z = (z ^ (z >> 27)) * 0x94D049BB133111EBull;
+        return ((z ^ (z >> 31)) >> 11) * 0x1p-53 + 0x1p-54;
+    };
+    for (int p = 0; p < HS_P; ++p)
+        for (int k = 0; k < s->d; ++k) Q[(size_t)p * ld + k] = sqrt(-2.0 * log(next())) * cos(6.283185307179586 * next());
+    prefix_orthonormalise(Q, ld);
+    for (int round = 0; round <= HS_PREFIX_ROUNDS; ++round) {
+        CU(cudaMemcpy(dq, Q.data(), qbytes, cudaMemcpyHostToDevice));
+        hs_cov_apply_kernel<<<dim3((ld + 127) / 128, HS_P), 128>>>(C, ld, dq, dz);
+        LAUNCHED();
+        CU(cudaGetLastError());
+        CU(cudaMemcpy(Z.data(), dz, qbytes, cudaMemcpyDeviceToHost));
+        if (round == HS_PREFIX_ROUNDS) break;
+        Q.swap(Z);
+        prefix_orthonormalise(Q, ld);
+    }
+    std::vector<float> diag(ld);
+    CU(cudaMemcpy2D(diag.data(), 4, C.p, (size_t)(ld + 1) * 4, 4, ld, cudaMemcpyDeviceToHost));
+    double tr = 0.0, te = 0.0;
+    for (int k = 0; k < ld; ++k) tr += diag[k];
+    for (size_t i = 0; i < Q.size(); ++i) te += Q[i] * Z[i];
+    if (!(tr > 0.0 && te >= HS_PREFIX_MIN_ENERGY * tr)) return 0;
+    std::vector<float> B(Q.size());
+    double f2 = 0.0;
+    for (size_t i = 0; i < Q.size(); ++i) { B[i] = (float)Q[i]; f2 += (double)B[i] * B[i]; }
+    std::vector<double> Gh((size_t)HS_P * HS_P);
+    for (int p = 0; p < HS_P; ++p)
+        for (int q = 0; q <= p; ++q) {
+            double d = 0.0;
+            for (int k = 0; k < ld; ++k) d += (double)B[(size_t)p * ld + k] * B[(size_t)q * ld + k];
+            Gh[(size_t)p * HS_P + q] = Gh[(size_t)q * HS_P + p] = d;
+        }
+    const float bnorm = std::max(1.0f, std::nextafter((float)(sqrt(f2) * (1.0 + 0x1p-20)), INFINITY));
+    if (s->d_basis.try_alloc(B.size() * 4) != cudaSuccess) return 0;
+    CU(cudaMemcpy(s->d_basis, B.data(), B.size() * 4, cudaMemcpyHostToDevice));
+    CU(cudaMemcpy(dg, Gh.data(), Gh.size() * 8, cudaMemcpyHostToDevice));
+    s->basis_norm = bnorm;
+    *selected = true;
+    return 0;
+}
+
 static int attach_half_copy(nidx_vec_segment* s, VecDev* V) {
     const char* e = getenv("NIDX_B200_HS_F16");
     if (e && !strcmp(e, "0")) return 0;
@@ -342,21 +554,43 @@
     if (!s->half_decided && s->n) {
         s->half_decided = true;
         const int ldh = (s->ld + 7) / 8 * 8;
-        const size_t hbytes = (size_t)s->n * ldh * 2, rbytes = (size_t)s->n * 16;
-        size_t free_b = 0, total_b = 0;
-        CU(cudaMemGetInfo(&free_b, &total_b));
-        if (free_b < hbytes + rbytes + HS_HALF_MARGIN) return 0;
-        if (s->d_hvecs.try_alloc(hbytes) != cudaSuccess || s->d_hrec.try_alloc(rbytes) != cudaSuccess) {
-            s->d_hvecs.release();
-            return 0;
-        }
-        hs_half_kernel<<<s->sm_count * 8, 256>>>(s->vdev(), s->n, ldh, s->d_hvecs, s->d_hrec);
-        LAUNCHED();
-        CU(cudaGetLastError());
-        CU(cudaDeviceSynchronize());
-        s->ldh = ldh;
-    }
-    if (s->ldh) { V->hvecs = s->d_hvecs; V->hrec = s->d_hrec; V->ldh = s->ldh; }
+        DevArray<double> dg;
+        bool prefix = false;
+        int r = prefix_basis(s, dg, &prefix);
+        if (r) return r;
+        if (prefix) {
+            if (s->d_hrec.try_alloc((size_t)s->n * 32) != cudaSuccess || s->d_pvecs.try_alloc((size_t)s->n * HS_P * 2) != cudaSuccess) {
+                s->d_hrec.release();
+                s->d_basis.release();
+                return 0;
+            }
+            hs_half_kernel<<<s->sm_count * 8, 256>>>(s->vdev(), s->n, ldh, nullptr, s->d_hrec, 2);
+            LAUNCHED();
+            VecDev Vb = s->vdev();
+            Vb.basis = s->d_basis; Vb.bnorm = s->basis_norm;
+            hs_prefix_kernel<<<s->sm_count * 8, 256>>>(Vb, s->n, dg, s->d_pvecs, s->d_hrec);
+            LAUNCHED();
+            CU(cudaGetLastError());
+            CU(cudaDeviceSynchronize());
+        } else {
+            const size_t hbytes = (size_t)s->n * ldh * 2, rbytes = (size_t)s->n * 16;
+            size_t free_b = 0, total_b = 0;
+            CU(cudaMemGetInfo(&free_b, &total_b));
+            if (free_b < hbytes + rbytes + HS_HALF_MARGIN) return 0;
+            if (s->d_hvecs.try_alloc(hbytes) != cudaSuccess || s->d_hrec.try_alloc(rbytes) != cudaSuccess) {
+                s->d_hvecs.release();
+                return 0;
+            }
+            hs_half_kernel<<<s->sm_count * 8, 256>>>(s->vdev(), s->n, ldh, s->d_hvecs, s->d_hrec, 1);
+            LAUNCHED();
+            CU(cudaGetLastError());
+            CU(cudaDeviceSynchronize());
+            s->ldh = ldh;
+        }
+    }
+    if (s->d_hrec) V->hrec = s->d_hrec;
+    if (s->ldh) { V->hvecs = s->d_hvecs; V->ldh = s->ldh; }
+    if (s->d_pvecs) { V->pvecs = s->d_pvecs; V->basis = s->d_basis; V->bnorm = s->basis_norm; }
     return 0;
 }
 
@@ -668,6 +902,7 @@
 int nidx_vec_counters_ex(nidx_vec_segment* s, uint64_t out[6]) { return read_counters(s, out, {0, 1, 2, 3, 4, 5}); }
 int nidx_vec_counters(nidx_vec_segment* s, uint64_t out[3]) { return read_counters(s, out, {0, 1, -1}); }
 int nidx_vec_exact_rows(nidx_vec_segment* s, uint64_t* out) { return read_counters(s, out, {6}); }
+int nidx_vec_prefix_rows(nidx_vec_segment* s, uint64_t* out) { return read_counters(s, out, {7}); }
 int nidx_vec_scan_counters(nidx_vec_segment* s, uint64_t out[2]) { return read_counters(s, out, {6, 7}); }
 
 static int rabitq_check(const nidx_vec_segment* s) {
@@ -823,8 +1058,9 @@
 }
 
 typedef void (*hs_kernel_t)(VecDev, GraphDev, SearchArgs);
-static hs_kernel_t pick_search_kernel(int ld) {
-    return pick_ng<1, 2, 3, 4, 6, 8>(ld, [](auto ng) -> hs_kernel_t { return hnsw_search_kernel<ng>; });
+static hs_kernel_t pick_search_kernel(int ld, bool prefix) {
+    if (prefix) return pick_ng<2, 3, 4, 6, 8>(ld, [](auto ng) -> hs_kernel_t { return hnsw_search_kernel<ng, true>; });
+    return pick_ng<1, 2, 3, 4, 6, 8>(ld, [](auto ng) -> hs_kernel_t { return hnsw_search_kernel<ng, false>; });
 }
 
 static hs_kernel_t pick_rabitq_walk_kernel(int ld, bool w4) {
@@ -1210,7 +1446,7 @@
             return fail(NIDX_EINVAL, "HNSW search needs %zu bytes of shared memory (ef=%d, k=%d, dim=%d): too large", smem, ef0, k, s->d);
         VecDev Vh = V;
         int r = attach_half_copy(s, &Vh);
-        hs_kernel_t kern = pick_search_kernel(s->ld);
+        hs_kernel_t kern = pick_search_kernel(s->ld, Vh.pvecs != nullptr);
         int grid = 0;
         if (!r) r = walk_grid(kern, HS_THREADS, smem, &grid);
         if (r) return r;
@@ -1494,7 +1730,10 @@
     hash_bits = ilog2(slots);
     size_t smem_search = hs_smem_bytes(s->ld, list_cap, hash_bits);
     if (smem_search > 200 * 1024) return fail(NIDX_EINVAL, "HNSW build search needs %zu bytes of shared memory", smem_search);
-    hs_kernel_t kern = pick_search_kernel(s->ld);
+    VecDev V = s->vdev();
+    int hr = attach_half_copy(s, &V);
+    if (hr) return hr;
+    hs_kernel_t kern = pick_search_kernel(s->ld, V.pvecs != nullptr);
     CU(cudaFuncSetAttribute(kern, cudaFuncAttributeMaxDynamicSharedMemorySize, (int)smem_search));
     int occ = 0;
     CU(cudaOccupancyMaxActiveBlocksPerMultiprocessor(&occ, kern, HS_THREADS, smem_search));
@@ -1513,9 +1752,6 @@
     s->last_counters.store(nullptr);
 
 
-    VecDev V = s->vdev();
-    int hr = attach_half_copy(s, &V);
-    if (hr) return hr;
     GraphDev G = s->gdev();
     uint32_t begin = 0;
     for (size_t b = 0; b < ends.size(); ++b) {
diff --git a/nucliadb_b200/csrc/common.cuh b/nucliadb_b200/csrc/common.cuh
--- a/nucliadb_b200/csrc/common.cuh
+++ b/nucliadb_b200/csrc/common.cuh
@@ -17,7 +17,12 @@
     const __half* hvecs;
     const float4* hrec;
     int ldh;
+    const uint4* pvecs;
+    const float* basis;
+    float bnorm;
 };
+
+constexpr int HS_P = 64;
 
 __host__ __device__ __forceinline__ int dot_depth(int ld) { return (ld / 4 + 31) / 32 + 7; }
 
diff --git a/nucliadb_b200/csrc/hnsw_search.cuh b/nucliadb_b200/csrc/hnsw_search.cuh
--- a/nucliadb_b200/csrc/hnsw_search.cuh
+++ b/nucliadb_b200/csrc/hnsw_search.cuh
@@ -88,8 +88,11 @@
     unsigned hop;
     float qnorm;
     float qbound;
+    float* u;
+    float unorm, udelta, wnorm;
     unsigned long long n_dist, n_expand, n_overflow;
     unsigned long long n_skip;
+    unsigned long long n_pref;
 
     __device__ HopRec& last_hop() const { return hops[(hop & 1u) ^ 1u]; }
 };
@@ -110,8 +113,79 @@
     return make_key(s_up, y, 1) <= wkey;
 }
 
+__device__ __forceinline__ bool hs_prefix_out(const VecDev& V, const SearchCtx& c, uint32_t y, float dot, float4 r0, float4 r1, uint64_t wkey) {
+    float a = __fmul_rn(dot, r1.x);
+    float bnd = __fmaf_ru(r1.x, 0x1p-142f, __fadd_ru(r0.w, 0x1p-149f));
+    bnd = __fmaf_ru(__fmul_ru(0.5f, r0.z), c.qbound, bnd);
+    bnd = __fmaf_ru(r1.w, c.udelta, bnd);
+    bnd = __fmaf_ru(r1.z, c.unorm, bnd);
+    bnd = __fmaf_ru(r1.y, c.wnorm, bnd);
+    if (!(fabsf(a) <= 0x1p120f && bnd <= 0x1p100f)) return false;
+    float s_up = sim_from_parts(V.sim, __fadd_ru(a, bnd), r0.x, c.qnorm);
+    return make_key(s_up, y, 1) <= wkey;
+}
+
+__device__ __forceinline__ uint4 ldg_stream_u4(const uint4* p) {
+    uint4 r;
+    asm volatile("ld.global.nc.L1::no_allocate.v4.u32 {%0, %1, %2, %3}, [%4];" : "=r"(r.x), "=r"(r.y), "=r"(r.z), "=r"(r.w) : "l"(p));
+    return r;
+}
+
+__device__ __forceinline__ float hs_prefix_dot(uint4 h, const float* u, int g) {
+    const float4 u0 = reinterpret_cast<const float4*>(u)[2 * g], u1 = reinterpret_cast<const float4*>(u)[2 * g + 1];
+    const float2 a = __half22float2(*reinterpret_cast<const __half2*>(&h.x)), b = __half22float2(*reinterpret_cast<const __half2*>(&h.y));
+    const float2 e = __half22float2(*reinterpret_cast<const __half2*>(&h.z)), f = __half22float2(*reinterpret_cast<const __half2*>(&h.w));
+    float s = __fmul_rn(a.x, u0.x);
+    s = __fmaf_rn(a.y, u0.y, s);
+    s = __fmaf_rn(b.x, u0.z, s);
+    s = __fmaf_rn(b.y, u0.w, s);
+    s = __fmaf_rn(e.x, u1.x, s);
+    s = __fmaf_rn(e.y, u1.y, s);
+    s = __fmaf_rn(f.x, u1.z, s);
+    s = __fmaf_rn(f.y, u1.w, s);
+#pragma unroll
+    for (int off = 4; off >= 1; off >>= 1) s = __fadd_rn(s, __shfl_xor_sync(0xFFFFFFFFu, s, off));
+    return s;
+}
+
+__device__ inline void hs_query_prefix(const VecDev& V, SearchCtx& c, double* scratch) {
+    const int lane = threadIdx.x & 31, warp = threadIdx.x >> 5, ld = V.ld;
+    double d2 = 0.0, u2 = 0.0;
+    for (int p = warp; p < HS_P; p += HS_WARPS) {
+        const float* b = V.basis + (size_t)p * ld;
+        double s = 0.0;
+        for (int k = lane; k < ld; k += 32) s = fma((double)__ldg(b + k), (double)c.qvec[k], s);
+#pragma unroll
+        for (int off = 16; off >= 1; off >>= 1) s += __shfl_xor_sync(0xFFFFFFFFu, s, off);
+        const float u = __double2float_rn(s);
+        if (lane == 0) c.u[p] = u;
+        const double e = s - (double)u;
+        d2 = fma(e, e, d2);
+        u2 = fma((double)u, (double)u, u2);
+    }
+    __syncthreads();
+    double w2 = 0.0;
+    for (int k = threadIdx.x; k < ld; k += blockDim.x) {
+        double w = (double)c.qvec[k];
+        for (int p = 0; p < HS_P; ++p) w = fma(-(double)__ldg(V.basis + (size_t)p * ld + k), (double)c.u[p], w);
+        w2 = fma(w, w, w2);
+    }
+#pragma unroll
+    for (int off = 16; off >= 1; off >>= 1) w2 += __shfl_xor_sync(0xFFFFFFFFu, w2, off);
+    if (lane == 0) { scratch[warp] = d2; scratch[HS_WARPS + warp] = u2; scratch[2 * HS_WARPS + warp] = w2; }
+    __syncthreads();
+    double D2 = 0.0, U2 = 0.0, W2 = 0.0;
+    for (int i = 0; i < HS_WARPS; ++i) { D2 += scratch[i]; U2 += scratch[HS_WARPS + i]; W2 += scratch[2 * HS_WARPS + i]; }
+    const double slack = 1.0 + 0x1p-20, g = (double)(ld + HS_P + 2) * 0x1p-52 * (double)V.bnorm, qb = (double)c.qbound;
+    const double un = sqrt(U2 * slack) * slack;
+    c.unorm = __double2float_ru(un);
+    c.udelta = __double2float_ru((sqrt(D2 * slack) + g * qb) * slack);
+    c.wnorm = __double2float_ru((sqrt(W2 * slack) + g * (qb + un)) * slack);
+    __syncthreads();
+}
+
 __host__ __device__ __forceinline__ size_t hs_smem_bytes(int ld, int list_cap, int hash_bits) {
-    return (size_t)ld * 4 + (size_t)list_cap * 16 + ((size_t)4 << hash_bits) + HS_MAX_ROW * 12 + HS_MAX_ROW * 8 + 16 + 64;
+    return (size_t)ld * 4 + (size_t)list_cap * 16 + ((size_t)4 << hash_bits) + HS_MAX_ROW * 12 + HS_MAX_ROW * 8 + 16 + HS_P * 4 + 64;
 }
 
 __device__ inline unsigned char* hs_setup(SearchCtx& c, const SearchArgs& a, unsigned char* p, int ld) {
@@ -125,11 +199,12 @@
     c.todo_id = reinterpret_cast<uint32_t*>(p); p += HS_MAX_ROW * 4;
     c.pref_row = reinterpret_cast<uint32_t*>(p); p += 2 * HS_MAX_ROW * 4;
     c.pref_node = reinterpret_cast<uint32_t*>(p); p += 16;
+    c.u = reinterpret_cast<float*>(p); p += HS_P * 4;
     c.s_len = &s_ints[0]; c.s_best = &s_ints[1]; c.s_hash_count = &s_ints[2]; c.s_flag = &s_ints[3];
     c.hops = s_hops;
     c.hop = 0;
     c.qnorm = 0.0f;
-    c.n_dist = c.n_expand = c.n_overflow = c.n_skip = 0;
+    c.n_dist = c.n_expand = c.n_overflow = c.n_skip = c.n_pref = 0;
     return p;
 }
 
@@ -196,12 +271,13 @@
     return pred;
 }
 
-template <bool CU, int NG, int W = HS_WARPS, bool LEAN = false>
+template <bool CU, int NG, int W = HS_WARPS, bool LEAN = false, bool PF = false>
 __device__ inline void hs_expand(const VecDev& V, const GraphDev& G, SearchCtx& c, uint32_t node, int layer, int ef, float min_score, int best, int len_in = -1) {
     int lane = threadIdx.x & 31, warp = threadIdx.x >> 5;
     int stride = G.stride(layer);
     unsigned cur = c.hop & 1u;
     HopRec& h = c.hops[cur];
+    __shared__ unsigned long long s_surv[2];
     if (warp == 0) {
         const uint32_t* prow = c.pref_row + cur * HS_MAX_ROW;
         bool hit = c.pref_node[cur] == node;
@@ -224,6 +300,7 @@
             h.best_next = INT_MAX;
             h.nadmit = 0;
             h.maxtodo = 0;
+            if (PF) s_surv[cur] = 0;
             c.n_expand++;
         }
     } else if (warp == W - 1) {
@@ -241,11 +318,53 @@
         if (admit) { atomicAdd(&h.nadmit, 1); atomicMax(&h.maxtodo, (unsigned long long)key); }
         c.n_dist++;
     };
-    const bool screen = !CU && wkey != 0 && V.hvecs != nullptr;
+    const bool screen = !PF && !CU && wkey != 0 && V.hvecs != nullptr;
     auto skip = [&](int j) { c.todo_key[j] = 0; c.n_dist++; c.n_skip++; };
     const float4* qv = reinterpret_cast<const float4*>(c.qvec);
     auto frow = [&](uint32_t y) { return reinterpret_cast<const float4*>(V.vecs + (size_t)y * V.ld); };
     auto hrow = [&](uint32_t y) { return reinterpret_cast<const uint2*>(V.hvecs + (size_t)y * V.ldh); };
+    if (PF && !CU && wkey != 0) {
+        const int g = lane & 7;
+        const int flines = (V.ld * 4 + 127) >> 7;
+        for (int j0 = warp * 4; j0 < ntodo; j0 += W * 4) {
+            const int j = j0 + (lane >> 3);
+            const bool act = j < ntodo;
+            const uint32_t y = act ? c.todo_id[j] : 0u;
+            float4 r0 = make_float4(0.f, 0.f, 0.f, 0.f), r1 = r0;
+            uint4 hp = make_uint4(0u, 0u, 0u, 0u);
+            if (act) {
+                r0 = __ldg(V.hrec + 2 * (size_t)y);
+                r1 = __ldg(V.hrec + 2 * (size_t)y + 1);
+                hp = ldg_stream_u4(V.pvecs + (size_t)y * (HS_P / 8) + g);
+            }
+            const float dot = hs_prefix_dot(hp, c.u, g);
+            const bool out = act && hs_prefix_out(V, c, y, dot, r0, r1, wkey);
+            if (act && !out) {
+                const char* rowp = reinterpret_cast<const char*>(frow(y));
+                for (int l = g; l < flines; l += 8) prefetch_l2(rowp + (size_t)l * 128);
+            }
+            if (act && g == 0) {
+                if (out) c.todo_key[j] = 0;
+                else atomicOr(&s_surv[cur], 1ull << j);
+            }
+            const int nout = __popc(__ballot_sync(0xFFFFFFFFu, out && g == 0));
+            if (lane == 0) { c.n_dist += nout; c.n_skip += nout; c.n_pref += nout; }
+        }
+        __syncthreads();
+        unsigned long long m = s_surv[cur];
+        for (int s = 0; m; ++s, m &= m - 1) {
+            if (s % W != warp) continue;
+            const int j = __ffsll((long long)m) - 1;
+            const uint32_t y = c.todo_id[j];
+            const float vnorm = __ldg(reinterpret_cast<const float*>(V.hrec + 2 * (size_t)y));
+            float ab = warp_dot_t<NG>(frow(y), qv, ng, lane);
+            if (lane == 0) finish(j, y, ab, vnorm);
+        }
+        if (warp == W - 1) cp_async_commit_wait_all();
+        c.hop++;
+        __syncthreads();
+        return;
+    }
     const int lines = screen ? (V.ldh * 2 + 127) >> 7 : (V.ld * 4 + 127) >> 7;
     for (int j = warp + W; j < ntodo; j += W) {
         const char* rowp = screen ? reinterpret_cast<const char*>(hrow(c.todo_id[j])) : reinterpret_cast<const char*>(frow(c.todo_id[j]));
@@ -323,12 +442,12 @@
     else __syncthreads();
 }
 
-template <int NG, int W = HS_WARPS>
+template <int NG, int W = HS_WARPS, bool PF = false>
 __device__ inline void hs_layer_search(const VecDev& V, const GraphDev& G, SearchCtx& c, int layer, int ef) {
     int best = *c.s_best, len = *c.s_len;
     while (best < len) {
         uint64_t ckey = c.A[best];
-        hs_expand<false, NG, W, true>(V, G, c, key_id(ckey), layer, ef, 0.0f, best, len);
+        hs_expand<false, NG, W, true, PF>(V, G, c, key_id(ckey), layer, ef, 0.0f, best, len);
         hs_merge<false, true>(c, ef, best, c.last_hop().ntodo, &len, &best);
     }
 }
@@ -416,7 +535,7 @@
     if (threadIdx.x == 0) a.out_counts[q] = nacc;
 }
 
-template <int NG>
+template <int NG, bool PF>
 __global__ void __launch_bounds__(HS_THREADS, 4) hnsw_search_kernel(VecDev V, GraphDev G, SearchArgs a) {
     extern __shared__ __align__(16) unsigned char smem[];
     SearchCtx c;
@@ -432,7 +551,8 @@
         else { self = a.nodes[q]; qsrc = V.vecs + (size_t)self * V.ld; c.qnorm = V.sim != SIM_DOT ? V.norms[self] : 0.0f; }
         for (int i = threadIdx.x; i < ng; i += blockDim.x) reinterpret_cast<float4*>(c.qvec)[i] = reinterpret_cast<const float4*>(qsrc)[i];
         __syncthreads();
-        if (V.hvecs) c.qbound = hs_query_bound(c.qvec, V.ld);
+        if (PF || V.hvecs) c.qbound = hs_query_bound(c.qvec, V.ld);
+        if (PF) hs_query_prefix(V, c, reinterpret_cast<double*>(c.todo_key));
 
         if (threadIdx.x < 32) {
             uint32_t ep = G.entry_node;
@@ -451,7 +571,7 @@
             if (a.mode == 0) ef = layer == 0 ? a.ef0 : 1;
             else ef = layer <= top ? a.efC : 1;
             hs_reseed(c, c.vis);
-            hs_layer_search<NG>(V, G, c, layer, ef);
+            hs_layer_search<NG, HS_WARPS, PF>(V, G, c, layer, ef);
             __syncthreads();
             if (a.mode == 1 && layer <= top && layer < HS_MAX_LAYERS) {
                 int len = *c.s_len;
@@ -469,6 +589,7 @@
     }
     hs_flush_counters(c, a.counters);
     if (lane == 0 && c.n_dist) atomicAdd(&a.counters[6], c.n_dist - c.n_skip);
-}
-
-}
+    if (PF && lane == 0 && c.n_pref) atomicAdd(&a.counters[7], c.n_pref);
+}
+
+}
diff --git a/nucliadb_b200/segment.py b/nucliadb_b200/segment.py
--- a/nucliadb_b200/segment.py
+++ b/nucliadb_b200/segment.py
@@ -209,6 +209,11 @@
     def exact_rows(self) -> int:
         out = C.c_uint64()
         check(_lib.load().nidx_vec_exact_rows(self._h, C.byref(out)))
+        return out.value
+
+    def prefix_rows(self) -> int:
+        out = C.c_uint64()
+        check(_lib.load().nidx_vec_prefix_rows(self._h, C.byref(out)))
         return out.value
 
     def scan_counters(self):
```

New measurement: 580,200 (median of 6 runs). 1.29x the previous value.
